# cbalint13/opencv-dlco

Measured on AMD Instinct MI355X. Metric: pj-learn patch-pairs/sec, higher is better.
Workload: dtype f32; 1 GPU; pj-learn configs[1] Liberty-shaped, rank ~64: 500000 pair-rows x PR-dim 8192, batch 200+200 per GPU (global 200+200), mu=0.0025 gamma=0.5, fp32, rank 48 after 3893 steps; device= (gfx950:sramecc+:xnack-), burn_in_steps=300

## Files before the change

### include/dlco.h

```cpp
#ifndef DLCO_H
#define DLCO_H

#include <stddef.h>
#include <stdint.h>

#ifdef __cplusplus
extern "C" {
#endif

#define DLCO_OK            0
#define DLCO_ERR_INVALID  -2
#define DLCO_ERR_HIP      -3
#define DLCO_ERR_NODEVICE -4
#define DLCO_ERR_NOCONV   -5
#define DLCO_ERR_COMM     -6

typedef struct dlco_ctx dlco_ctx;

typedef struct dlco_cfg {
    int32_t  F;
    int32_t  N;
    int32_t  B;
    float    mu;
    float    gamma;
    uint64_t seed;
    int32_t  device;
    int32_t  rank;
    int32_t  world;
    float    eig_tol;
    int32_t  eig_guard;
    int32_t  eig_max_iter;
    int32_t  shard;
    int32_t  strict_conv;
    int32_t  grad_bf16;
    int32_t  reserved[5];
} dlco_cfg;

void dlco_cfg_default(dlco_cfg *cfg);

const char *dlco_version(void);
const char *dlco_last_error(const dlco_ctx *ctx);

int dlco_ctx_create(dlco_ctx **out, const dlco_cfg *cfg);
void dlco_ctx_destroy(dlco_ctx *ctx);
int dlco_device_name(const dlco_ctx *ctx, char *buf, size_t cap, int *cc_major, int *cc_minor);

int dlco_set_data(dlco_ctx *ctx, const float *dists_host, const uint8_t *labels_host);
int dlco_set_data_device(dlco_ctx *ctx, const float *dists_dev, const uint8_t *labels_host);
int dlco_device_width(const dlco_ctx *ctx);
int dlco_set_data_shared(dlco_ctx *ctx, dlco_ctx *src);
int dlco_set_pairs(dlco_ctx *ctx, const float *desc_host, int32_t P, const int32_t *pairs_host);
int dlco_set_pairs_device(dlco_ctx *ctx, const float *desc_dev, int32_t P, const int32_t *pairs_host);
int dlco_synth_data(dlco_ctx *ctx, const float *U_host, int32_t k, uint64_t seed,
                    float sigma_pos, float sigma_neg, float noise, float scale_jitter);
int dlco_get_rows(dlco_ctx *ctx, int32_t row0, int32_t n, float *out_host);

int dlco_get_index(const dlco_ctx *ctx, int32_t *pos, int32_t *n_pos, int32_t *n_pos_trn,
                   int32_t *neg, int32_t *n_neg, int32_t *n_neg_trn);

int dlco_step(dlco_ctx *ctx);
int dlco_steps(dlco_ctx *ctx, int32_t n);

int dlco_step_begin(dlco_ctx *ctx);
int dlco_step_grad(dlco_ctx *ctx);
int dlco_step_finish(dlco_ctx *ctx);

#define DLCO_BUF_DIST   1
#define DLCO_BUF_GRAD   2
#define DLCO_BUF_DFAVG  3
#define DLCO_BUF_W      4
#define DLCO_BUF_GATHER 5
#define DLCO_BUF_DATA   6
int dlco_dev_buffer(dlco_ctx *ctx, int32_t which, void **dev_ptr, size_t *bytes);
int dlco_bind_buffer(dlco_ctx *ctx, int32_t which, void *dev_ptr, size_t bytes);

typedef int (*dlco_allgather_fn)(void *user, int32_t which, size_t bytes_per_rank);
int dlco_set_allgather(dlco_ctx *ctx, dlco_allgather_fn fn, void *user);
int dlco_comm_unique_id(void *out_id, size_t cap, const char *rccl_path);
int dlco_comm_init(dlco_ctx *ctx, const void *id, size_t id_bytes, const char *rccl_path);
int dlco_comm_init_host(dlco_ctx *ctx, const char *shm_name);
int dlco_comm_destroy(dlco_ctx *ctx);
int dlco_stream(dlco_ctx *ctx, void **stream);
int dlco_sync(dlco_ctx *ctx);

int dlco_get_batch(const dlco_ctx *ctx, int32_t *pos_rows, int32_t *neg_rows,
                   float *pos_dist, float *neg_dist, int32_t *rho, int32_t *kappa);

int dlco_get_t(const dlco_ctx *ctx, uint32_t *t);
int dlco_get_W(dlco_ctx *ctx, float *W_host , int32_t *r);
int dlco_get_A(dlco_ctx *ctx, float *A_host );
int dlco_get_dfavg(dlco_ctx *ctx, float *dfavg_host );
int dlco_set_state(dlco_ctx *ctx, uint32_t t, const float *dfavg_host, const float *W_host, int32_t r);

int dlco_validate(dlco_ctx *ctx, float *loss_val, float *regul, int32_t *rank);

int dlco_stats(dlco_ctx *ctx, const float *W_host, int32_t r, int32_t *dim, float *fpr95, double *auc);

int dlco_project_sqdist(dlco_ctx *ctx, const int32_t *row_ids_host, int32_t n,
                        const float *W_host, int32_t r, float *out_host);
int dlco_viol_counts(dlco_ctx *ctx, const float *pd_host, const float *nd_host, int32_t B,
                     int32_t *rho_host, int32_t *kappa_host);
int dlco_grad_rda(dlco_ctx *ctx, const int32_t *pos_rows_host, const int32_t *neg_rows_host,
                  const int32_t *rho_host, const int32_t *kappa_host, int32_t B,
                  float alpha, float beta, const float *dfavg_in_host, float *dfavg_out_host);
int dlco_psd_project(dlco_ctx *ctx, const float *dfavg_host, uint32_t t,
                     float *W_host, int32_t *r, float *A_host );
int dlco_sym_product(dlco_ctx *ctx, const float *X_host, int32_t rows, const float *G_host, int32_t mode,
                     float *out_host);
int dlco_hinge_sum(dlco_ctx *ctx, const float *pos_host, int32_t n_pos,
                   const float *neg_host, int32_t n_neg, double *out);
int dlco_roc_stats(dlco_ctx *ctx, const float *dist_host, const uint8_t *labels_host, int32_t n,
                   float *fpr95, double *auc);

typedef struct dlco_log_entry {
    uint32_t t;
    int32_t  is_best;
    int32_t  saved;
    float    loss_val, regul, obj, obj_best;
    int32_t  rank, rank_best;
    int32_t  dim;
    double   auc, auc_best;
    float    fpr95, fpr95_best;
    double   vtime;
    int32_t  nonconv;
    int32_t  reserved;
} dlco_log_entry;
int dlco_log_step(dlco_ctx *ctx, dlco_log_entry *out);
int dlco_get_saved(dlco_ctx *ctx, float *W_host, int32_t *r, float *A_host);

int dlco_profile_enable(dlco_ctx *ctx, int32_t on);
int dlco_profile_read(dlco_ctx *ctx, const char *kernel, int64_t *launches, double *total_ms);
int dlco_counters(const dlco_ctx *ctx, int64_t out[8]);
int dlco_eig_stats(const dlco_ctx *ctx, int64_t *iters, int64_t *product_rows, int64_t *jacobi_sweeps,
                   int32_t *block_rows);

typedef struct dlco_pr_ctx dlco_pr_ctx;
const char *dlco_pr_last_error(const dlco_pr_ctx *ctx);
int dlco_pr_create(dlco_pr_ctx **out, int32_t F, int32_t N, float mu, float gamma, uint64_t seed, int32_t device);
void dlco_pr_destroy(dlco_pr_ctx *ctx);
int dlco_pr_device_name(const dlco_pr_ctx *ctx, char *buf, size_t cap, int *cc_major, int *cc_minor);
int dlco_pr_set_data(dlco_pr_ctx *ctx, const float *dists_host, const uint8_t *labels_host);
int dlco_pr_get_index(const dlco_pr_ctx *ctx, int32_t *n_pos, int32_t *n_pos_trn, int32_t *n_neg, int32_t *n_neg_trn);
int dlco_pr_steps(dlco_pr_ctx *ctx, uint32_t n);
int dlco_pr_get_state(dlco_pr_ctx *ctx, uint32_t *t, float *w_host , float *dfavg_host );
int dlco_pr_set_state(dlco_pr_ctx *ctx, uint32_t t, const float *w_host, const float *dfavg_host);
int dlco_pr_validate(dlco_pr_ctx *ctx, float *loss_val, float *regul, int32_t *nnz);
int dlco_pr_stats(dlco_pr_ctx *ctx, const float *w_host, const float *prparams_host, int32_t pr_rows, int32_t pr_cols,
                  int32_t nchannels, int32_t max_dim, int32_t *nPR, int32_t *dim, int32_t *nzdim, float *fpr95, double *auc);

typedef struct dlco_pr_grid dlco_pr_grid;
int  dlco_pr_grid_create(dlco_pr_grid **out, dlco_pr_ctx *src, int32_t G, const float *mu, const float *gamma, uint64_t seed);
void dlco_pr_grid_destroy(dlco_pr_grid *grid);
const char *dlco_pr_grid_last_error(const dlco_pr_grid *grid);
int  dlco_pr_grid_steps(dlco_pr_grid *grid, uint32_t n);
int  dlco_pr_grid_get_state(dlco_pr_grid *grid, uint32_t *t, float *w_host , float *dfavg_host );
int  dlco_pr_grid_validate(dlco_pr_grid *grid, float *loss_val, float *regul, int32_t *nnz);
int  dlco_pr_grid_stats(dlco_pr_grid *grid, const int32_t *configs, int32_t n, const float *w_host, const float *prparams_host,
                        int32_t pr_rows, int32_t pr_cols, int32_t nchannels, int32_t max_dim,
                        int32_t *nPR, int32_t *dim, int32_t *nzdim, float *fpr95, double *auc);
int  dlco_pr_grid_set_group(dlco_pr_grid *grid, int32_t per_group);
int32_t dlco_pr_grid_group(const dlco_pr_grid *grid);

typedef struct dlco_desc_ctx dlco_desc_ctx;

int  dlco_desc_create(dlco_desc_ctx **out, float init_sigma, int32_t n_angle_bins, int32_t norm, int32_t device);
void dlco_desc_destroy(dlco_desc_ctx *ctx);
const char *dlco_desc_last_error(const dlco_desc_ctx *ctx);
int  dlco_desc_select_filters(const float *pr_filters, int32_t rows, int32_t cols, const float *w, int32_t wcols,
                              float *out, int32_t *nsel_out);
int  dlco_desc_set_filters(dlco_desc_ctx *ctx, const float *filters_host, int32_t nsel);
int32_t dlco_desc_size(const dlco_desc_ctx *ctx);
int  dlco_desc_transform(dlco_desc_ctx *ctx, const uint8_t *patch_host, float *patch_trans_host);
int  dlco_desc_compute(dlco_desc_ctx *ctx, const uint8_t *patches_host, int64_t n, float *desc_host);
int  dlco_desc_compute_device(dlco_desc_ctx *ctx, const uint8_t *patches_host, int64_t n, float *desc_dev, int64_t ld);
int  dlco_desc_pair_dists(dlco_desc_ctx *ctx, const uint8_t *patches_host, int64_t n_patches, const int32_t *pairs_host,
                          int64_t n_pairs, float *dist_host, uint8_t *label_host);
int  dlco_desc_full_dists(dlco_desc_ctx *ctx, const uint8_t *patches_host, int64_t n_patches, const int32_t *pairs_host,
                          int64_t n_pairs, float *dist_host, uint8_t *label_host);
typedef int (*dlco_desc_sink_fn)(void *user, int64_t row0, int64_t rows, const float *dist, const uint8_t *label);
int  dlco_desc_pair_dists_stream(dlco_desc_ctx *ctx, const uint8_t *patches_host, int64_t n_patches, const int32_t *pairs_host,
                                 int64_t n_pairs, int64_t chunk_rows, dlco_desc_sink_fn sink, void *user);
int  dlco_desc_full_dists_stream(dlco_desc_ctx *ctx, const uint8_t *patches_host, int64_t n_patches, const int32_t *pairs_host,
                                 int64_t n_pairs, int64_t chunk_rows, dlco_desc_sink_fn sink, void *user);
int  dlco_desc_set_projection(dlco_desc_ctx *ctx, const float *W_host, int32_t r, int32_t F);
int32_t dlco_desc_projected_size(const dlco_desc_ctx *ctx);
int  dlco_desc_describe(dlco_desc_ctx *ctx, const uint8_t *patches_host, int64_t n, float *out_host);
int  dlco_desc_describe_device(dlco_desc_ctx *ctx, const uint8_t *patches_host, int64_t n, float *out_dev, int64_t ld);
int  dlco_desc_pair_sqdists(dlco_desc_ctx *ctx, const uint8_t *patches_host, int64_t n_patches, const int32_t *pairs_host,
                            int64_t n_pairs, float *dist_host, uint8_t *label_host);
int  dlco_desc_pair_stats(dlco_desc_ctx *ctx, const uint8_t *patches_host, int64_t n_patches, const int32_t *pairs_host,
                          int64_t n_pairs, int32_t *dim, float *fpr95, double *auc);
int dlco_desc_match(dlco_desc_ctx *ctx, const float *query_host, int64_t nq, const float *train_host, int64_t nt,
                    int32_t r, int32_t *idx_host, float *sqdist_host);
int dlco_desc_match_device(dlco_desc_ctx *ctx, const float *query_dev, int64_t ldq, int64_t nq,
                           const float *train_dev, int64_t ldt, int64_t nt, int32_t r,
                           int32_t *idx_dev, float *sqdist_dev);
int dlco_desc_cross_sqdists(dlco_desc_ctx *ctx, const float *query_host, int64_t nq, const float *train_host, int64_t nt,
                            int32_t r, float *out_host);
double dlco_desc_last_kernel_ms(const dlco_desc_ctx *ctx);

#ifdef __cplusplus
}
#endif
#endif
```

### opencv-dlco_amd/__init__.py

```python
import ctypes as C
import os
import subprocess

import numpy as np

_HERE = os.path.dirname(os.path.abspath(__file__))
LIB_PATH = os.path.join(_HERE, "libdlco.so")
HEADER_PATH = os.path.join(os.path.dirname(_HERE), "include", "dlco.h")

OK, ERR_INVALID, ERR_HIP, ERR_NODEVICE, ERR_NOCONV, ERR_COMM = 0, -2, -3, -4, -5, -6
BUF_DIST, BUF_GRAD, BUF_DFAVG, BUF_W, BUF_GATHER, BUF_DATA = 1, 2, 3, 4, 5, 6
ALLGATHER_FN = C.CFUNCTYPE(C.c_int, C.c_void_p, C.c_int32, C.c_size_t)


class DlcoError(RuntimeError):
    def __init__(self, code, msg):
        super().__init__("libdlco error %d: %s" % (code, msg))
        self.code = code


class Cfg(C.Structure):
    _fields_ = [
        ("F", C.c_int32), ("N", C.c_int32), ("B", C.c_int32),
        ("mu", C.c_float), ("gamma", C.c_float),
        ("seed", C.c_uint64),
        ("device", C.c_int32), ("rank", C.c_int32), ("world", C.c_int32),
        ("eig_tol", C.c_float), ("eig_guard", C.c_int32), ("eig_max_iter", C.c_int32),
        ("shard", C.c_int32), ("strict_conv", C.c_int32), ("grad_bf16", C.c_int32),
        ("reserved", C.c_int32 * 5),
    ]


class LogEntry(C.Structure):
    _fields_ = [
        ("t", C.c_uint32), ("is_best", C.c_int32), ("saved", C.c_int32),
        ("loss_val", C.c_float), ("regul", C.c_float), ("obj", C.c_float), ("obj_best", C.c_float),
        ("rank", C.c_int32), ("rank_best", C.c_int32), ("dim", C.c_int32),
        ("auc", C.c_double), ("auc_best", C.c_double),
        ("fpr95", C.c_float), ("fpr95_best", C.c_float),
        ("vtime", C.c_double),
        ("nonconv", C.c_int32), ("reserved", C.c_int32),
    ]


def build(verbose=False):
    cmd = ["make", "-C", os.path.join(_HERE, "csrc"), "-j8"]
    if not verbose:
        cmd.insert(1, "-s")
    subprocess.check_call(cmd)


_lib = None
f32p, i32p, u8p = C.POINTER(C.c_float), C.POINTER(C.c_int32), C.POINTER(C.c_uint8)


def load():
    global _lib
    if _lib is not None:
        return _lib
    if not os.path.exists(LIB_PATH):
        raise DlcoError(ERR_NODEVICE, "%s is missing: run __graft_entry__.build() (no CPU fallback exists)" % LIB_PATH)
    L = C.CDLL(LIB_PATH)
    vp = C.c_void_p
    L.dlco_version.restype = C.c_char_p
    L.dlco_last_error.restype = C.c_char_p
    L.dlco_last_error.argtypes = [vp]
    L.dlco_cfg_default.argtypes = [C.POINTER(Cfg)]
    L.dlco_cfg_default.restype = None
    L.dlco_ctx_create.argtypes = [C.POINTER(vp), C.POINTER(Cfg)]
    L.dlco_ctx_destroy.argtypes = [vp]
    L.dlco_ctx_destroy.restype = None
    L.dlco_device_name.argtypes = [vp, C.c_char_p, C.c_size_t, C.POINTER(C.c_int), C.POINTER(C.c_int)]
    L.dlco_set_data.argtypes = [vp, f32p, u8p]
    L.dlco_set_data_device.argtypes = [vp, vp, u8p]
    L.dlco_set_data_shared.argtypes = [vp, vp]
    L.dlco_device_width.argtypes = [vp]
    L.dlco_set_pairs.argtypes = [vp, f32p, C.c_int32, i32p]
    L.dlco_synth_data.argtypes = [vp, f32p, C.c_int32, C.c_uint64, C.c_float, C.c_float, C.c_float, C.c_float]
    L.dlco_get_rows.argtypes = [vp, C.c_int32, C.c_int32, f32p]
    L.dlco_get_index.argtypes = [vp, i32p, i32p, i32p, i32p, i32p, i32p]
    for name in ("dlco_step", "dlco_step_begin", "dlco_step_grad", "dlco_step_finish", "dlco_sync"):
        getattr(L, name).argtypes = [vp]
    L.dlco_steps.argtypes = [vp, C.c_int32]
    L.dlco_dev_buffer.argtypes = [vp, C.c_int32, C.POINTER(vp), C.POINTER(C.c_size_t)]
    L.dlco_bind_buffer.argtypes = [vp, C.c_int32, vp, C.c_size_t]
    L.dlco_stream.argtypes = [vp, C.POINTER(vp)]
    L.dlco_set_allgather.argtypes = [vp, ALLGATHER_FN, vp]
    L.dlco_comm_unique_id.argtypes = [vp, C.c_size_t, C.c_char_p]
    L.dlco_comm_init.argtypes = [vp, vp, C.c_size_t, C.c_char_p]
    L.dlco_comm_destroy.argtypes = [vp]
    L.dlco_get_batch.argtypes = [vp, i32p, i32p, f32p, f32p, i32p, i32p]
    L.dlco_get_t.argtypes = [vp, C.POINTER(C.c_uint32)]
    L.dlco_get_W.argtypes = [vp, f32p, i32p]
    L.dlco_get_A.argtypes = [vp, f32p]
    L.dlco_get_dfavg.argtypes = [vp, f32p]
    L.dlco_set_state.argtypes = [vp, C.c_uint32, f32p, f32p, C.c_int32]
    L.dlco_validate.argtypes = [vp, f32p, f32p, i32p]
    L.dlco_stats.argtypes = [vp, f32p, C.c_int32, i32p, f32p, C.POINTER(C.c_double)]
    L.dlco_project_sqdist.argtypes = [vp, i32p, C.c_int32, f32p, C.c_int32, f32p]
    L.dlco_viol_counts.argtypes = [vp, f32p, f32p, C.c_int32, i32p, i32p]
    L.dlco_grad_rda.argtypes = [vp, i32p, i32p, i32p, i32p, C.c_int32, C.c_float, C.c_float, f32p, f32p]
    L.dlco_psd_project.argtypes = [vp, f32p, C.c_uint32, f32p, i32p, f32p]
    L.dlco_hinge_sum.argtypes = [vp, f32p, C.c_int32, f32p, C.c_int32, C.POINTER(C.c_double)]
    L.dlco_sym_product.argtypes = [vp, f32p, C.c_int32, f32p, C.c_int32, f32p]
    L.dlco_roc_stats.argtypes = [vp, f32p, u8p, C.c_int32, f32p, C.POINTER(C.c_double)]
    L.dlco_log_step.argtypes = [vp, C.POINTER(LogEntry)]
    L.dlco_get_saved.argtypes = [vp, f32p, i32p, f32p]
    L.dlco_profile_enable.argtypes = [vp, C.c_int32]
    L.dlco_profile_read.argtypes = [vp, C.c_char_p, C.POINTER(C.c_int64), C.POINTER(C.c_double)]
    L.dlco_eig_stats.argtypes = [vp, C.POINTER(C.c_int64), C.POINTER(C.c_int64), C.POINTER(C.c_int64), i32p]
    L.dlco_counters.argtypes = [vp, C.POINTER(C.c_int64)]
    i64 = C.c_int64
    L.dlco_set_pairs_device.argtypes = [vp, vp, C.c_int32, i32p]
    L.dlco_desc_last_error.restype = C.c_char_p
    L.dlco_desc_last_error.argtypes = [vp]
    L.dlco_desc_create.argtypes = [C.POINTER(vp), C.c_float, C.c_int32, C.c_int32, C.c_int32]
    L.dlco_desc_destroy.argtypes = [vp]
    L.dlco_desc_destroy.restype = None
    L.dlco_desc_select_filters.argtypes = [f32p, C.c_int32, C.c_int32, f32p, C.c_int32, f32p, C.POINTER(C.c_int32)]
    L.dlco_desc_set_filters.argtypes = [vp, f32p, C.c_int32]
    L.dlco_desc_size.argtypes = [vp]
    L.dlco_desc_size.restype = C.c_int32
    L.dlco_desc_transform.argtypes = [vp, u8p, f32p]
    L.dlco_desc_compute.argtypes = [vp, u8p, i64, f32p]
    L.dlco_desc_compute_device.argtypes = [vp, u8p, i64, vp, i64]
    L.dlco_desc_pair_dists.argtypes = [vp, u8p, i64, i32p, i64, f32p, u8p]
    L.dlco_desc_full_dists.argtypes = [vp, u8p, i64, i32p, i64, f32p, u8p]
    L.dlco_desc_set_projection.argtypes = [vp, f32p, C.c_int32, C.c_int32]
    L.dlco_desc_projected_size.argtypes = [vp]
    L.dlco_desc_projected_size.restype = C.c_int32
    L.dlco_desc_describe.argtypes = [vp, u8p, i64, f32p]
    L.dlco_desc_describe_device.argtypes = [vp, u8p, i64, vp, i64]
    L.dlco_desc_pair_sqdists.argtypes = [vp, u8p, i64, i32p, i64, f32p, u8p]
    L.dlco_desc_pair_stats.argtypes = [vp, u8p, i64, i32p, i64, C.POINTER(C.c_int32), C.POINTER(C.c_float), C.POINTER(C.c_double)]
    L.dlco_desc_match.argtypes = [vp, f32p, i64, f32p, i64, C.c_int32, i32p, f32p]
    L.dlco_desc_match_device.argtypes = [vp, vp, i64, i64, vp, i64, i64, C.c_int32, vp, vp]
    L.dlco_desc_cross_sqdists.argtypes = [vp, f32p, i64, f32p, i64, C.c_int32, f32p]
    L.dlco_desc_last_kernel_ms.argtypes = [vp]
    L.dlco_desc_last_kernel_ms.restype = C.c_double
    L.dlco_pr_last_error.restype = C.c_char_p
    L.dlco_pr_last_error.argtypes = [vp]
    L.dlco_pr_create.argtypes = [C.POINTER(vp), C.c_int32, C.c_int32, C.c_float, C.c_float, C.c_uint64, C.c_int32]
    L.dlco_pr_destroy.argtypes = [vp]
    L.dlco_pr_destroy.restype = None
    L.dlco_pr_device_name.argtypes = [vp, C.c_char_p, C.c_size_t, C.POINTER(C.c_int), C.POINTER(C.c_int)]
    L.dlco_pr_set_data.argtypes = [vp, f32p, u8p]
    L.dlco_pr_get_index.argtypes = [vp, i32p, i32p, i32p, i32p]
    L.dlco_pr_steps.argtypes = [vp, C.c_uint32]
    L.dlco_pr_get_state.argtypes = [vp, C.POINTER(C.c_uint32), f32p, f32p]
    L.dlco_pr_set_state.argtypes = [vp, C.c_uint32, f32p, f32p]
    L.dlco_pr_validate.argtypes = [vp, f32p, f32p, i32p]
    L.dlco_pr_stats.argtypes = [vp, f32p, f32p, C.c_int32, C.c_int32, C.c_int32, C.c_int32, i32p, i32p, i32p, f32p, C.POINTER(C.c_double)]
    L.dlco_pr_grid_last_error.restype = C.c_char_p
    L.dlco_pr_grid_last_error.argtypes = [vp]
    L.dlco_pr_grid_create.argtypes = [C.POINTER(vp), vp, C.c_int32, f32p, f32p, C.c_uint64]
    L.dlco_pr_grid_destroy.argtypes = [vp]
    L.dlco_pr_grid_destroy.restype = None
    L.dlco_pr_grid_steps.argtypes = [vp, C.c_uint32]
    L.dlco_pr_grid_get_state.argtypes = [vp, C.POINTER(C.c_uint32), f32p, f32p]
    L.dlco_pr_grid_validate.argtypes = [vp, f32p, f32p, i32p]
    L.dlco_pr_grid_stats.argtypes = [vp, i32p, C.c_int32, f32p, f32p, C.c_int32, C.c_int32, C.c_int32, C.c_int32, i32p, i32p, i32p, f32p,
                                     C.POINTER(C.c_double)]
    L.dlco_pr_grid_set_group.argtypes = [vp, C.c_int32]
    L.dlco_pr_grid_group.argtypes = [vp]
    L.dlco_pr_grid_group.restype = C.c_int32
    _lib = L
    return L


def comm_unique_id(rccl_path=None):
    L = load()
    buf = C.create_string_buffer(128)
    rc = L.dlco_comm_unique_id(buf, 128, rccl_path.encode() if rccl_path else None)
    if rc != OK:
        raise DlcoError(rc, L.dlco_last_error(None).decode())
    return buf.raw


def exported_symbols():
    import re
    text = open(HEADER_PATH).read()
    return sorted(set(re.findall(r"\b(dlco_[a-z0-9_]+)\s*\(", text)))


def _p(a, t):
    return None if a is None else a.ctypes.data_as(t)


def _f32(a):
    return np.ascontiguousarray(a, dtype=np.float32)


def _i32(a):
    return np.ascontiguousarray(a, dtype=np.int32)


class Context:

    def __init__(self, F, N, B=200, mu=0.001, gamma=0.5, seed=2215, device=0, rank=0, world=1,
                 eig_tol=None, eig_guard=None, eig_max_iter=None, shard=0, strict_conv=0, grad_bf16=0):
        self.L = load()
        cfg = Cfg()
        self.L.dlco_cfg_default(C.byref(cfg))
        cfg.F, cfg.N, cfg.B, cfg.mu, cfg.gamma, cfg.seed = F, N, B, mu, gamma, seed
        cfg.device, cfg.rank, cfg.world, cfg.shard = device, rank, world, shard
        cfg.strict_conv = strict_conv
        cfg.grad_bf16 = grad_bf16
        if eig_tol is not None:
            cfg.eig_tol = eig_tol
        if eig_guard is not None:
            cfg.eig_guard = eig_guard
        if eig_max_iter is not None:
            cfg.eig_max_iter = eig_max_iter
        self.F, self.N, self.B, self.world, self.rank = F, N, B, world, rank
        h = C.c_void_p()
        rc = self.L.dlco_ctx_create(C.byref(h), C.byref(cfg))
        if rc != OK:
            raise DlcoError(rc, self.L.dlco_last_error(None).decode())
        self.h = h

    def close(self):
        if getattr(self, "h", None):
            self.L.dlco_ctx_destroy(self.h)
            self.h = None

    def __del__(self):
        try:
            self.close()
        except Exception:
            pass

    def _ck(self, rc):
        if rc != OK:
            raise DlcoError(rc, self.L.dlco_last_error(self.h).decode())

    def device_name(self):
        buf = C.create_string_buffer(256)
        a, b = C.c_int(), C.c_int()
        self._ck(self.L.dlco_device_name(self.h, buf, 256, C.byref(a), C.byref(b)))
        return buf.value.decode(), a.value, b.value

    def set_data(self, dists, labels):
        d, l = _f32(dists), np.ascontiguousarray(labels, np.uint8).ravel()
        assert d.shape == (self.N, self.F) and l.size == self.N
        self._ck(self.L.dlco_set_data(self.h, _p(d, f32p), _p(l, u8p)))

    def set_data_device(self, dev_ptr, labels):
        l = np.ascontiguousarray(labels, np.uint8).ravel()
        self._ck(self.L.dlco_set_data_device(self.h, C.c_void_p(dev_ptr), _p(l, u8p)))

    def set_data_shared(self, other):
        self._ck(self.L.dlco_set_data_shared(self.h, other.h))

    def device_width(self):
        return int(self.L.dlco_device_width(self.h))

    def set_pairs(self, desc, pairs):
# ... 14 lines not shown
    def get_rows(self, row0, n):
        out = np.empty((n, self.F), np.float32)
        self._ck(self.L.dlco_get_rows(self.h, row0, n, _p(out, f32p)))
        return out

    def index(self):
        a, b, c_, d = C.c_int32(), C.c_int32(), C.c_int32(), C.c_int32()
        self._ck(self.L.dlco_get_index(self.h, None, C.byref(a), C.byref(b), None, C.byref(c_), C.byref(d)))
        pos, neg = np.empty(max(a.value, 1), np.int32), np.empty(max(c_.value, 1), np.int32)
        self._ck(self.L.dlco_get_index(self.h, _p(pos, i32p), None, None, _p(neg, i32p), None, None))
        return dict(pos=pos[:a.value], n_pos_trn=b.value, neg=neg[:c_.value], n_neg_trn=d.value)

    def step(self):
        self._ck(self.L.dlco_step(self.h))

    def steps(self, n):
        self._ck(self.L.dlco_steps(self.h, n))

    def step_begin(self):
        self._ck(self.L.dlco_step_begin(self.h))

    def step_grad(self):
        self._ck(self.L.dlco_step_grad(self.h))

    def step_finish(self):
        self._ck(self.L.dlco_step_finish(self.h))

    def sync(self):
        self._ck(self.L.dlco_sync(self.h))

    def dev_buffer(self, which):
        p, n = C.c_void_p(), C.c_size_t()
        self._ck(self.L.dlco_dev_buffer(self.h, which, C.byref(p), C.byref(n)))
        return p.value, n.value

    def bind_buffer(self, which, dev_ptr, nbytes):
        self._ck(self.L.dlco_bind_buffer(self.h, which, C.c_void_p(dev_ptr), nbytes))

    def stream(self):
        p = C.c_void_p()
        self._ck(self.L.dlco_stream(self.h, C.byref(p)))
        return p.value

    def comm_init(self, id_bytes, rccl_path=None):
        buf = C.create_string_buffer(bytes(id_bytes), 128)
        self._ck(self.L.dlco_comm_init(self.h, buf, 128, rccl_path.encode() if rccl_path else None))

    def comm_destroy(self):
        self._ck(self.L.dlco_comm_destroy(self.h))

    def set_allgather(self, fn):
        def tramp(_user, which, nbytes):
            try:
                return int(fn(int(which), int(nbytes)) or 0)
            except Exception:
                import traceback
                traceback.print_exc()
                return -1
        self._ag = ALLGATHER_FN(tramp)
        self._ck(self.L.dlco_set_allgather(self.h, self._ag, None))

    def batch(self):
        B = self.B
        pr, nr = np.empty(B, np.int32), np.empty(B, np.int32)
        pd, nd = np.empty(B, np.float32), np.empty(B, np.float32)
        rho, kap = np.empty(B, np.int32), np.empty(B, np.int32)
        self._ck(self.L.dlco_get_batch(self.h, _p(pr, i32p), _p(nr, i32p), _p(pd, f32p), _p(nd, f32p), _p(rho, i32p), _p(kap, i32p)))
        return dict(pos_rows=pr, neg_rows=nr, pd=pd, nd=nd, rho=rho, kappa=kap)

    def t(self):
        v = C.c_uint32()
        self._ck(self.L.dlco_get_t(self.h, C.byref(v)))
        return v.value

    def W(self):
        W = np.empty((self.F, self.F), np.float32)
        r = C.c_int32()
        self._ck(self.L.dlco_get_W(self.h, _p(W, f32p), C.byref(r)))
        return W[:r.value].copy()

    def A(self):
        A = np.empty((self.F, self.F), np.float32)
        self._ck(self.L.dlco_get_A(self.h, _p(A, f32p)))
        return A

    def dfavg(self):
        A = np.empty((self.F, self.F), np.float32)
        self._ck(self.L.dlco_get_dfavg(self.h, _p(A, f32p)))
        return A

    def set_state(self, t, dfavg=None, W=None):
        d = None if dfavg is None else _f32(dfavg)
        w = None if W is None or len(W) == 0 else _f32(W)
        self._ck(self.L.dlco_set_state(self.h, t, _p(d, f32p), _p(w, f32p), 0 if w is None else w.shape[0]))

    def validate(self):
        lo, rg, rk = C.c_float(), C.c_float(), C.c_int32()
        self._ck(self.L.dlco_validate(self.h, C.byref(lo), C.byref(rg), C.byref(rk)))
        return lo.value, rg.value, rk.value

    def stats(self, W=None):
        dim, f, a = C.c_int32(), C.c_float(), C.c_double()
        w = None if W is None else _f32(W)
        self._ck(self.L.dlco_stats(self.h, _p(w, f32p), 0 if w is None else w.shape[0], C.byref(dim), C.byref(f), C.byref(a)))
        return dim.value, f.value, a.value

    def log_step(self):
        e = LogEntry()
        self._ck(self.L.dlco_log_step(self.h, C.byref(e)))
        return e

    def saved(self):
        r = C.c_int32()
        self._ck(self.L.dlco_get_saved(self.h, None, C.byref(r), None))
        if r.value == 0:
            return None, None
        W, A = np.empty((r.value, self.F), np.float32), np.empty((self.F, self.F), np.float32)
        self._ck(self.L.dlco_get_saved(self.h, _p(W, f32p), C.byref(r), _p(A, f32p)))
        return W, A

    def project_sqdist(self, row_ids, W):
        ids, w = _i32(row_ids), _f32(W)
        out = np.empty(ids.size, np.float32)
        self._ck(self.L.dlco_project_sqdist(self.h, _p(ids, i32p), ids.size, _p(w, f32p), w.shape[0] if w.size else 0, _p(out, f32p)))
        return out

    def viol_counts(self, pd, nd):
        pd, nd = _f32(pd), _f32(nd)
        rho, kap = np.empty(pd.size, np.int32), np.empty(pd.size, np.int32)
        self._ck(self.L.dlco_viol_counts(self.h, _p(pd, f32p), _p(nd, f32p), pd.size, _p(rho, i32p), _p(kap, i32p)))
        return rho, kap

    def grad_rda(self, pos_rows, neg_rows, rho, kappa, alpha, beta, dfavg_in=None):
        pr, nr, rho, kap = _i32(pos_rows), _i32(neg_rows), _i32(rho), _i32(kappa)
        d = None if dfavg_in is None else _f32(dfavg_in)
        out = np.empty((self.F, self.F), np.float32)
        self._ck(self.L.dlco_grad_rda(self.h, _p(pr, i32p), _p(nr, i32p), _p(rho, i32p), _p(kap, i32p), pr.size, alpha, beta, _p(d, f32p), _p(out, f32p)))
        return out

    def psd_project(self, dfavg, t, want_A=True):
        d = _f32(dfavg)
        W = np.empty((self.F, self.F), np.float32)
        A = np.empty((self.F, self.F), np.float32) if want_A else None
        r = C.c_int32()
        self._ck(self.L.dlco_psd_project(self.h, _p(d, f32p), t, _p(W, f32p), C.byref(r), _p(A, f32p)))
        return W[:r.value].copy(), A

    def sym_product(self, X, G, mode=0):
        x, g = _f32(X), _f32(G)
        out = np.empty_like(x)
        self._ck(self.L.dlco_sym_product(self.h, _p(x, f32p), x.shape[0], _p(g, f32p), mode, _p(out, f32p)))
        return out

    def hinge_sum(self, pos, neg):
        p, n = _f32(pos), _f32(neg)
        out = C.c_double()
        self._ck(self.L.dlco_hinge_sum(self.h, _p(p, f32p), p.size, _p(n, f32p), n.size, C.byref(out)))
        return out.value

    def roc_stats(self, dist, labels):
        d, l = _f32(dist), np.ascontiguousarray(labels, np.uint8).ravel()
        f, a = C.c_float(), C.c_double()
        self._ck(self.L.dlco_roc_stats(self.h, _p(d, f32p), _p(l, u8p), d.size, C.byref(f), C.byref(a)))
        return f.value, a.value

    def profile_enable(self, on=True):
        self._ck(self.L.dlco_profile_enable(self.h, int(on)))

    def profile_read(self, kernel="grad_syrk"):
        n, ms = C.c_int64(), C.c_double()
        self._ck(self.L.dlco_profile_read(self.h, kernel.encode(), C.byref(n), C.byref(ms)))
        return n.value, ms.value

    def counters(self):
        out = (C.c_int64 * 8)()
        self._ck(self.L.dlco_counters(self.h, out))
        return dict(steps=out[0], active_rows=out[1], nonconverged=out[2], jacobi_barrier_timeouts=out[3],
                    rank_update_passes=out[4], rank_update_check=out[5] * 1e-9, locked_passes=out[6], locked_rows=out[7])

    def eig_stats(self):
        a, b, c_, d = C.c_int64(), C.c_int64(), C.c_int64(), C.c_int32()
        self._ck(self.L.dlco_eig_stats(self.h, C.byref(a), C.byref(b), C.byref(c_), C.byref(d)))
        return dict(iters=a.value, product_rows=b.value, jacobi_sweeps=c_.value, block_rows=d.value)


class PrContext:

    def __init__(self, F, N, mu=0.025, gamma=0.10, seed=2215, device=0):
        self.L = load()
        self.F, self.N = F, N
        h = C.c_void_p()
        rc = self.L.dlco_pr_create(C.byref(h), F, N, mu, gamma, seed, device)
        if rc != OK:
            raise DlcoError(rc, self.L.dlco_pr_last_error(None).decode())
        self.h = h

    def close(self):
        if getattr(self, "h", None):
            self.L.dlco_pr_destroy(self.h)
            self.h = None

    def __del__(self):
        try:
            self.close()
        except Exception:
            pass

    def _ck(self, rc):
        if rc != OK:
            raise DlcoError(rc, self.L.dlco_pr_last_error(self.h).decode())

    def set_data(self, dists, labels):
        d, l = _f32(dists), np.ascontiguousarray(labels, np.uint8).ravel()
        assert d.shape == (self.N, self.F) and l.size == self.N
        self._ck(self.L.dlco_pr_set_data(self.h, _p(d, f32p), _p(l, u8p)))

    def index(self):
        a, b, c_, d = C.c_int32(), C.c_int32(), C.c_int32(), C.c_int32()
        self._ck(self.L.dlco_pr_get_index(self.h, C.byref(a), C.byref(b), C.byref(c_), C.byref(d)))
        return dict(n_pos=a.value, n_pos_trn=b.value, n_neg=c_.value, n_neg_trn=d.value)

    def steps(self, n):
        self._ck(self.L.dlco_pr_steps(self.h, n))

    def state(self):
        t = C.c_uint32()
        w, df = np.empty(self.F, np.float32), np.empty(self.F, np.float32)
        self._ck(self.L.dlco_pr_get_state(self.h, C.byref(t), _p(w, f32p), _p(df, f32p)))
        return dict(t=t.value, w=w, dfavg=df)

    def set_state(self, t, w=None, dfavg=None):
        w = None if w is None else _f32(w)
        d = None if dfavg is None else _f32(dfavg)
        self._ck(self.L.dlco_pr_set_state(self.h, t, _p(w, f32p), _p(d, f32p)))

    def validate(self):
        lo, rg, nz = C.c_float(), C.c_float(), C.c_int32()
        self._ck(self.L.dlco_pr_validate(self.h, C.byref(lo), C.byref(rg), C.byref(nz)))
        return lo.value, rg.value, nz.value

    def stats(self, prparams, w=None, nchannels=8, max_dim=-1):
        p = _f32(prparams)
        wv = None if w is None else _f32(w)
        npr, dim, nz, f, a = C.c_int32(), C.c_int32(), C.c_int32(), C.c_float(-1.0), C.c_double(0.0)
        self._ck(self.L.dlco_pr_stats(self.h, _p(wv, f32p), _p(p, f32p), p.shape[0], p.shape[1], nchannels, max_dim,
                                      C.byref(npr), C.byref(dim), C.byref(nz), C.byref(f), C.byref(a)))
        return dict(nPR=npr.value, dim=dim.value, nzdim=nz.value, fpr95=f.value, auc=a.value)


class PrGrid:

    def __init__(self, src, mus, gammas, seed=2215):
        self.L = load()
        mu, ga = _f32(mus).ravel(), _f32(gammas).ravel()
        assert mu.size == ga.size
        self.src, self.F, self.N, self.G = src, src.F, src.N, int(mu.size)
        self.mus, self.gammas = mu.copy(), ga.copy()
        h = C.c_void_p()
        rc = self.L.dlco_pr_grid_create(C.byref(h), src.h, self.G, _p(mu, f32p), _p(ga, f32p), seed)
        if rc != OK:
            raise DlcoError(rc, self.L.dlco_pr_grid_last_error(None).decode())
        self.h = h

    def close(self):
        if getattr(self, "h", None):
            self.L.dlco_pr_grid_destroy(self.h)
            self.h = None

    def __del__(self):
        try:
            self.close()
        except Exception:
            pass

    def _ck(self, rc):
        if rc != OK:
            raise DlcoError(rc, self.L.dlco_pr_grid_last_error(self.h).decode())

    def set_group(self, per_group):
        self._ck(self.L.dlco_pr_grid_set_group(self.h, per_group))

    def group(self):
        return int(self.L.dlco_pr_grid_group(self.h))

    def steps(self, n):
        self._ck(self.L.dlco_pr_grid_steps(self.h, n))

    def state(self):
        t = C.c_uint32()
        w, df = np.empty((self.G, self.F), np.float32), np.empty((self.G, self.F), np.float32)
        self._ck(self.L.dlco_pr_grid_get_state(self.h, C.byref(t), _p(w, f32p), _p(df, f32p)))
        return dict(t=t.value, w=w, dfavg=df)

    def validate(self):
        lo, rg, nz = np.empty(self.G, np.float32), np.empty(self.G, np.float32), np.empty(self.G, np.int32)
        self._ck(self.L.dlco_pr_grid_validate(self.h, _p(lo, f32p), _p(rg, f32p), _p(nz, i32p)))
        return dict(loss=lo, regul=rg, nnz=nz)

    def stats(self, prparams, configs=None, w=None, nchannels=8, max_dim=-1):
        p = _f32(prparams)
        cf = _i32(np.arange(self.G) if configs is None else configs).ravel()
        n = cf.size
        wv = None if w is None else _f32(w).reshape(n, self.F)
        npr, dim, nz = np.zeros(n, np.int32), np.zeros(n, np.int32), np.zeros(n, np.int32)
        f, a = np.full(n, -1.0, np.float32), np.zeros(n, np.float64)
        self._ck(self.L.dlco_pr_grid_stats(self.h, _p(cf, i32p), n, _p(wv, f32p), _p(p, f32p), p.shape[0], p.shape[1], nchannels, max_dim,
# ... 146 lines not shown
```

### opencv-dlco_amd/csrc/dlco_api.cpp

```cpp
#include "../../include/dlco.h"

#include "dlco_internal.hpp"
#include "eig_tracker.hpp"
#include "pair_index.hpp"
#include "rccl_comm.hpp"
#include "host_comm.hpp"

#include <algorithm>
#include <cfloat>
#include <chrono>
#include <cmath>
#include <cstring>

using namespace dlco;

static thread_local std::string g_last_error;

namespace {
struct EnvSwitch { const char *name, *purpose; };
const EnvSwitch kEnvSwitches[] = {
    {"DLCO_SYRK_FP32", "gradient SYRK as the k-ordered fp32 MFMA chain (syrk_rda_kernel8) instead of split-bf16 planes"},
    {"DLCO_NO_PACKED", "full F x F dual average where the packed upper-tile form would apply"},
    {"DLCO_FORCE_SHARD", "column-sharded layout (cfg.shard) on a single rank: the multi-GPU path on one GPU"},
    {"DLCO_NO_RANK_UPDATE", "first filter term from a product with the dual average, not from the step's rank update"},
// ... 989 lines not shown
        if (r) h2d_rows(c, Wd.p, W_host, (size_t)r, true);
        if (n <= 4096) project_few(c, ids.p, n, Wd.p, r, out.p);
        else project_many(c, ids.p, 0, n, Wd.p, r, out.p);
        d2h(c, out_host, out.p, (size_t)n * sizeof(float));
    });
}

int dlco_viol_counts(dlco_ctx *c, const float *pd_host, const float *nd_host, int32_t B, int32_t *rho_host,
                     int32_t *kappa_host)
{
    if (!c || !pd_host || !nd_host || !rho_host || !kappa_host || B < 0) return DLCO_ERR_INVALID;
    return guarded(c, [&] {
        DLCO_HIP(hipSetDevice(c->cfg.device));
        if (B == 0) return;
        DevBuf<float> pd, nd; DevBuf<int32_t> rho, kap;
        pd.alloc(B); nd.alloc(B); rho.alloc(B); kap.alloc(B);
        h2d(c, pd.p, pd_host, (size_t)B * sizeof(float));
        h2d(c, nd.p, nd_host, (size_t)B * sizeof(float));
        viol_counts(pd.p, nd.p, B, rho.p, kap.p, c->stream);
        d2h(c, rho_host, rho.p, (size_t)B * sizeof(int32_t));
        d2h(c, kappa_host, kap.p, (size_t)B * sizeof(int32_t));
    });
}

int dlco_grad_rda(dlco_ctx *c, const int32_t *pos_rows_host, const int32_t *neg_rows_host, const int32_t *rho_host,
                  const int32_t *kappa_host, int32_t B, float alpha, float beta, const float *dfavg_in_host,
                  float *dfavg_out_host)
{
    if (!c || !pos_rows_host || !neg_rows_host || !rho_host || !kappa_host || !dfavg_out_host || B < 1) return DLCO_ERR_INVALID;
    return guarded(c, [&] {
        DLCO_HIP(hipSetDevice(c->cfg.device));
        DLCO_CHECK(c->have_data && c->phase == 0, DLCO_ERR_INVALID, "dlco_grad_rda: no data / step in flight");
        for (int i = 0; i < B; i++)
            DLCO_CHECK(pos_rows_host[i] >= 0 && pos_rows_host[i] < c->N && neg_rows_host[i] >= 0 && neg_rows_host[i] < c->N,
                       DLCO_ERR_INVALID, "dlco_grad_rda: row id out of range");
        DevBuf<int32_t> pr, nr, rho, kap, ids; DevBuf<float> w; DevBuf<int> k;
        pr.alloc(B); nr.alloc(B); rho.alloc(B); kap.alloc(B); ids.alloc((2 * B + 31) & ~31); w.alloc((2 * B + 31) & ~31); k.alloc(1);
        h2d(c, pr.p, pos_rows_host, (size_t)B * sizeof(int32_t));
        h2d(c, nr.p, neg_rows_host, (size_t)B * sizeof(int32_t));
        h2d(c, rho.p, rho_host, (size_t)B * sizeof(int32_t));
        h2d(c, kap.p, kappa_host, (size_t)B * sizeof(int32_t));
        const size_t FF = (size_t)c->F * c->F;
        if (dfavg_in_host) {
            h2d_square(c, c->grad.p, dfavg_in_host);
            if (!c->shard) syrk_mirror_upper(c->grad.p, c->F, c->F, c->stream);
        } else fill_f32(c->grad.p, 0.f, FF, c->stream);
        build_active_rows(pr.p, nr.p, rho.p, kap.p, B, 0, B, ids.p, w.p, k.p, c->stream);
        if (c->packed) {
            DevBuf<float> pk;
            pk.alloc(syrk_packed_floats(c->F));
            syrk_pack_upper(c->grad.p, c->F, c->F, pk.p, c->stream);
            grad_syrk(c, ids.p, w.p, k.p, 2 * B, alpha, beta, pk.p, true);
            syrk_unpack_upper(pk.p, c->F, c->grad.p, c->F, c->stream);
            d2h_square(c, dfavg_out_host, c->grad.p);
            return;
        }
        grad_syrk(c, ids.p, w.p, k.p, 2 * B, alpha, beta, c->grad.p);
        d2h_square(c, dfavg_out_host, c->grad.p);
    });
}

int dlco_psd_project(dlco_ctx *c, const float *dfavg_host, uint32_t t, float *W_host, int32_t *r, float *A_host)
{
    if (!c || !dfavg_host || !r) return DLCO_ERR_INVALID;
    return guarded(c, [&] {
        DLCO_HIP(hipSetDevice(c->cfg.device));
        DLCO_CHECK(c->phase == 0, DLCO_ERR_INVALID, "dlco_psd_project: step in flight");
        const size_t FF = (size_t)c->F * c->F;
        DevBuf<float> G, Gp;
        G.alloc(FF);
        h2d_square(c, G.p, dfavg_host);
        if (c->packed) {
            Gp.alloc(syrk_packed_floats(c->F));
            syrk_mirror_upper(G.p, c->F, c->F, c->stream);
            syrk_pack_upper(G.p, c->F, c->F, Gp.p, c->stream);
        }
        c->eig->reset();
        const float cscale = (float)(std::sqrt((double)t + 1.0) / (double)c->cfg.gamma);
        double tr = 0.0;
        bool conv = true;
        DevBuf<float> Wd;
        Wd.alloc((size_t)c->w_cap * c->F);
        const int rr = c->eig->update(c->packed ? Gp.p : G.p, c->cfg.mu, cscale, Wd.p, &tr, &conv);
        c->eig->reset();
        if (rr > 0) {
            if (W_host) d2h_rows(c, W_host, Wd.p, (size_t)rr);
            *r = rr;
        } else {
            if (W_host) std::memset(W_host, 0, (size_t)c->Fu * c->Fu * sizeof(float));
            *r = c->Fu;
        }
        if (A_host) {
            build_A(c, Wd.p, rr);
            d2h_square(c, A_host, c->grad.p);
        }
        if (!conv) throw Error(DLCO_ERR_NOCONV, "dlco_psd_project: tracker did not reach its tolerance");
    });
}

int dlco_sym_product(dlco_ctx *c, const float *X_host, int32_t rows, const float *G_host, int32_t mode, float *out_host)
{
    if (!c || !X_host || !G_host || !out_host || rows < 1 || rows > ((mode == 1 || mode == 3) ? 160 : 128)) return DLCO_ERR_INVALID;
    return guarded(c, [&] {
        DLCO_HIP(hipSetDevice(c->cfg.device));
        const int F = c->F, pad = ((rows + 31) / 32) * 32;
        DevBuf<float> X, G, out;
        X.alloc((size_t)pad * F); G.alloc((size_t)F * F); out.alloc((size_t)pad * F);
        X.zero(c->stream);
        h2d_rows(c, X.p, X_host, (size_t)rows);
        h2d_square(c, G.p, G_host);
        bool ok;
        if (mode == 3 || mode == 4) {
            DevBuf<char> hi, lo, lo2;
            hi.alloc(bf16x2_plane_bytes(rows, F)); lo.alloc(bf16x2_plane_bytes(rows, F));
            if (mode == 4) lo2.alloc(bf16x2_plane_bytes(rows, F));
            DevBuf<float> slab, Gp;
            slab.alloc((size_t)4 * pad * F);
            Gp.alloc(syrk_packed_floats(F));
            syrk_mirror_upper(G.p, F, F, c->stream);
            syrk_pack_upper(G.p, F, F, Gp.p, c->stream);
            ok = skinny_product_sym(X.p, F, rows, Gp.p, F, 1.0f, out.p, F, nullptr, 0.f, nullptr, 0.f, hi.p, lo.p, slab.p, c->stream,
                                    mode == 4 ? lo2.p : nullptr);
            sync(c);
        } else if (mode == 1 || mode == 2) {
            DevBuf<char> hi, lo, lo2;
            hi.alloc(bf16x2_plane_bytes(rows, F)); lo.alloc(bf16x2_plane_bytes(rows, F));
            if (mode == 2) lo2.alloc(bf16x2_plane_bytes(rows, F));
            DevBuf<float> slab;
            slab.alloc(bf16x2_slab_floats(rows, F));
            ok = skinny_product_bf16x2(X.p, F, rows, G.p, F, F, F, 1.0f, out.p, F, nullptr, 0.f, nullptr, 0.f, hi.p, lo.p, slab.p,
                                       c->stream, 0, mode == 2 ? lo2.p : nullptr);
            sync(c);
        } else {
            GemmArgs g;
            g.M = rows; g.N = F; g.K = F;
            g.A.p = X.p; g.A.ld = F; g.A.kmajor = false;
            g.B.p = G.p; g.B.ld = F; g.B.kmajor = true;
            g.C = out.p; g.ldc = F;
            const int bm = rows <= 64 ? 64 : 128;
            const long tiles = (long)((rows + bm - 1) / bm) * ((F + 127) / 128);
            g.split_k = split_k_slices(tiles, 1024, F, 256);
            DevBuf<float> slab;
            slab.alloc(gemm_slab_floats(rows, F, g.split_k));
            g.slab = slab.p;
            gemm_f32(g, c->stream);
            sync(c);
            ok = true;
        }
        DLCO_CHECK(ok, DLCO_ERR_INVALID, "dlco_sym_product: shape not supported by this mode");
        d2h_rows(c, out_host, out.p, (size_t)rows);
    });
}

int dlco_hinge_sum(dlco_ctx *c, const float *pos_host, int32_t n_pos, const float *neg_host, int32_t n_neg, double *out)
{
    if (!c || !out || n_pos < 0 || n_neg < 0) return DLCO_ERR_INVALID;
    return guarded(c, [&] {
        DLCO_HIP(hipSetDevice(c->cfg.device));
        *out = 0.0;
        if (n_pos == 0) return;
        DevBuf<float> p, n, rows;
        p.alloc(n_pos); n.alloc(std::max(n_neg, 1)); rows.alloc(n_pos);
        h2d(c, p.p, pos_host, (size_t)n_pos * sizeof(float));
        if (n_neg) h2d(c, n.p, neg_host, (size_t)n_neg * sizeof(float));
        hinge_rows(p.p, n_pos, n.p, n_neg, rows.p, c->stream);
        sum_f32_to_f64(rows.p, n_pos, c->dscal.p, c->stream);
        d2h(c, out, c->dscal.p, sizeof(double));
    });
}

int dlco_roc_stats(dlco_ctx *c, const float *dist_host, const uint8_t *labels_host, int32_t n, float *fpr95, double *auc)
{
    if (!c || !dist_host || !labels_host || !fpr95 || !auc || n < 1) return DLCO_ERR_INVALID;
    return guarded(c, [&] {
        DLCO_HIP(hipSetDevice(c->cfg.device));
        DevBuf<float> d; DevBuf<uint8_t> l;
        d.alloc(n); l.alloc(n);
        h2d(c, d.p, dist_host, (size_t)n * sizeof(float));
        h2d(c, l.p, labels_host, (size_t)n);
        RocWork *w = roc_work_create(n);
        try { roc_stats(w, d.p, l.p, n, fpr95, auc, c->stream); } catch (...) { roc_work_destroy(w); throw; }
        roc_work_destroy(w);
    });
}

int dlco_log_step(dlco_ctx *c, dlco_log_entry *out)
{
    if (!c || !out) return DLCO_ERR_INVALID;
    return guarded(c, [&] {
        DLCO_HIP(hipSetDevice(c->cfg.device));
        DLCO_CHECK(c->phase == 0, DLCO_ERR_INVALID, "dlco_log_step: step in flight");
        const auto t0 = std::chrono::steady_clock::now();
        std::memset(out, 0, sizeof(*out));
        out->t = c->t - 1;
        float loss = 0.f, regul = 0.f;
        int32_t rank = 0;
        validate(c, &loss, &regul, &rank);
        const auto t1 = std::chrono::steady_clock::now();
        out->loss_val = loss; out->regul = regul; out->obj = loss + regul; out->rank = rank;
        if ((loss + regul) < c->obj_best) {
            c->obj_best = loss + regul;
            c->r_best = rank;
            out->is_best = 1;
            int32_t dim = 0; float f95 = 0.f; double auc = 0.0;
            stats(c, c->W.p, c->r, &dim, &f95, &auc);
            out->dim = dim; out->auc = auc; out->fpr95 = f95;
            if (c->auc_best <= auc && c->fpr95_best >= f95) {
                c->auc_best = auc; c->fpr95_best = f95;
                c->r_save_dev = c->r;
                c->r_save = c->r > 0 ? c->r : c->Fu;
                if (c->r > 0) {
                    c->W_save_dev.alloc((size_t)c->w_cap * c->F);
                    DLCO_HIP(hipMemcpyAsync(c->W_save_dev.p, c->W.p, (size_t)c->r * c->F * sizeof(float), hipMemcpyDeviceToDevice, c->stream));
                }
                out->saved = 1;
            }
        }
        out->obj_best = c->obj_best; out->rank_best = c->r_best;
        out->auc_best = c->auc_best; out->fpr95_best = c->fpr95_best;
        out->vtime = std::chrono::duration<double>(t1 - t0).count();
        out->nonconv = c->nonconv_window;
        c->nonconv_window = 0;
    });
}

int dlco_get_saved(dlco_ctx *c, float *W_host, int32_t *r, float *A_host)
{
    if (!c || !r) return DLCO_ERR_INVALID;
    *r = c->r_save;
    if (c->r_save <= 0 || (!W_host && !A_host)) return DLCO_OK;
    return guarded(c, [&] {
        DLCO_HIP(hipSetDevice(c->cfg.device));
        DLCO_CHECK(c->phase == 0, DLCO_ERR_INVALID, "dlco_get_saved: step in flight");
        if (W_host) {
            if (c->r_save_dev > 0) d2h_rows(c, W_host, c->W_save_dev.p, (size_t)c->r_save_dev);
            else std::memset(W_host, 0, (size_t)c->Fu * c->Fu * sizeof(float));
        }
        if (A_host) {
            build_A(c, c->W_save_dev.p, c->r_save_dev);
            d2h_square(c, A_host, c->grad.p);
        }
    });
}

int dlco_profile_enable(dlco_ctx *c, int32_t on)
{
    if (!c) return DLCO_ERR_INVALID;
    return guarded(c, [&] {
        c->prof.reset();
        c->prof.on = on != 0;
        c->prof.mask = on == 2 ? (1u << PROF_GRAD_SYRK) : ~0u;
    });
}

int dlco_profile_read(dlco_ctx *c, const char *kernel, int64_t *launches, double *total_ms)
{
    if (!c || !launches || !total_ms) return DLCO_ERR_INVALID;
    return guarded(c, [&] {
        int slot = PROF_GRAD_SYRK;
        if (kernel && std::strcmp(kernel, "eig_product") == 0) slot = PROF_EIG_PRODUCT;
        else if (kernel && std::strcmp(kernel, "jacobi") == 0) slot = PROF_JACOBI;
        else if (kernel && std::strcmp(kernel, "project") == 0) slot = PROF_PROJECT;
        else if (kernel && std::strcmp(kernel, "rank_update") == 0) slot = PROF_RANK_UPDATE;
        else if (kernel && std::strcmp(kernel, "grad_syrk") != 0) throw Error(DLCO_ERR_INVALID, "dlco_profile_read: unknown kernel group");
        c->prof.drain(slot);
        *launches = c->prof.rec[slot].n;
        *total_ms = c->prof.rec[slot].ms;
    });
}

int dlco_counters(const dlco_ctx *c, int64_t out[8])
{
    if (!c || !out) return DLCO_ERR_INVALID;
    for (int i = 0; i < 8; i++) out[i] = 0;
    out[0] = c->steps_run; out[1] = c->active_rows_sum; out[2] = c->nonconv_steps;
    out[3] = c->eig->stats().jacobi_barrier_timeouts;
    out[4] = c->eig->stats().rank_update_passes;
    out[5] = (int64_t)(c->eig->stats().rank_update_check * 1e9);
    out[6] = c->eig->stats().locked_passes;
    out[7] = c->eig->stats().locked_rows;
    return DLCO_OK;
}

int dlco_eig_stats(const dlco_ctx *c, int64_t *iters, int64_t *product_rows, int64_t *jacobi_sweeps, int32_t *block_rows)
{
    if (!c) return DLCO_ERR_INVALID;
    const EigStats &s = c->eig->stats();
    if (iters) *iters = s.iters;
    if (product_rows) *product_rows = s.product_rows;
    if (jacobi_sweeps) *jacobi_sweeps = s.jacobi_sweeps;
    if (block_rows) *block_rows = c->eig->block_rows();
    return DLCO_OK;
}

}
```

### opencv-dlco_amd/csrc/dlco_internal.hpp

```cpp
#pragma once

#include "../../include/dlco.h"

#include <hip/hip_runtime.h>

#include <algorithm>
#include <climits>
#include <cstdint>
#include <cstdio>
#include <cstdlib>
#include <cstring>
#include <functional>
#include <mutex>
#include <utility>
#include <stdexcept>
#include <string>
#include <type_traits>
#include <vector>

namespace dlco {

struct Error : std::runtime_error {
    int code;
    Error(int c, const std::string &m) : std::runtime_error(m), code(c) {}
};

#define DLCO_HIP(expr)                                                             \
    do {                                                                           \
        hipError_t e__ = (expr);                                                   \
        if (e__ != hipSuccess)                                                     \
            throw ::dlco::Error(-3, std::string(#expr) + ": " + hipGetErrorString(e__)); \
    } while (0)

#define DLCO_CHECK(cond, code, msg)                                                \
    do {                                                                           \
        if (!(cond)) throw ::dlco::Error((code), std::string(msg));                \
    } while (0)

template <typename Fn>
int guarded_call(std::string &thread_err, std::string *ctx_err, Fn &&fn)
{
    try {
        fn();
        return DLCO_OK;
    } catch (const Error &e) {
        thread_err = e.what();
        if (ctx_err) *ctx_err = e.what();
        return e.code;
    } catch (const std::exception &e) {
        thread_err = e.what();
        if (ctx_err) *ctx_err = e.what();
        return DLCO_ERR_INVALID;
    }
}

inline hipDeviceProp_t use_gfx950_device(int device)
{
    int ndev = 0;
    if (hipGetDeviceCount(&ndev) != hipSuccess || ndev <= 0 || device >= ndev)
        throw Error(DLCO_ERR_NODEVICE, "no usable HIP device (this library has no CPU fallback)");
    DLCO_HIP(hipSetDevice(device));
    hipDeviceProp_t prop;
    DLCO_HIP(hipGetDeviceProperties(&prop, device));
    if (std::strncmp(prop.gcnArchName, "gfx950", 6) != 0)
        throw Error(DLCO_ERR_NODEVICE, std::string("device is ") + prop.gcnArchName + ", this build targets gfx950 only");
    return prop;
}

template <int MAX, typename F>
void dispatch_mt(int mt, F &&f)
{
    if constexpr (MAX > 1) {
        if (mt < MAX) return dispatch_mt<MAX - 1>(mt, f);
    }
    f(std::integral_constant<int, MAX>{});
}

const char *env_switch(const char *name);

inline void ensure_dynamic_lds(const void *func, int bytes)
{
    static std::mutex mu;
    static std::vector<std::pair<const void *, int>> done;
    int dev = 0;
    DLCO_HIP(hipGetDevice(&dev));
    std::lock_guard<std::mutex> lock(mu);
    for (const auto &d : done)
        if (d.first == func && d.second == dev) return;
    DLCO_HIP(hipFuncSetAttribute(func, hipFuncAttributeMaxDynamicSharedMemorySize, bytes));
    done.emplace_back(func, dev);
}

template <typename T>
struct DevBuf {
    T *p = nullptr;
    size_t n = 0;
    DevBuf() = default;
    DevBuf(const DevBuf &) = delete;
    DevBuf &operator=(const DevBuf &) = delete;
    ~DevBuf() { release(); }
    void release() {
        if (p) (void)hipFree(p);
        p = nullptr;
        n = 0;
    }
    void alloc(size_t count) {
        if (count <= n && p) return;
        release();
        if (count == 0) count = 1;
        DLCO_HIP(hipMalloc((void **)&p, count * sizeof(T)));
        n = count;
    }
    void zero(hipStream_t s) { if (p) DLCO_HIP(hipMemsetAsync(p, 0, n * sizeof(T), s)); }
};

enum ProfSlot { PROF_GRAD_SYRK = 0, PROF_EIG_PRODUCT = 1, PROF_JACOBI = 2, PROF_PROJECT = 3, PROF_RANK_UPDATE = 4, PROF_SLOTS = 5 };

struct Profiler {
    bool on = false;
    unsigned mask = ~0u;
    hipStream_t s = nullptr;
    struct Rec { std::vector<hipEvent_t> ev; size_t used = 0; double ms = 0.0; int64_t n = 0; };
    Rec rec[PROF_SLOTS];
    ~Profiler() { for (auto &r : rec) for (hipEvent_t e : r.ev) (void)hipEventDestroy(e); }
    void mark(int slot) {
        if (!on || !((mask >> slot) & 1u)) return;
        Rec &r = rec[slot];
        if (r.used == r.ev.size()) { hipEvent_t e; DLCO_HIP(hipEventCreateWithFlags(&e, hipEventDisableSystemFence)); r.ev.push_back(e); }
        DLCO_HIP(hipEventRecord(r.ev[r.used++], s));
        if (r.used >= 8192 && (r.used % 2) == 0) drain(slot);
    }
    void begin(int slot) { mark(slot); }
    void end(int slot) { mark(slot); }
    void drain(int slot) {
        Rec &r = rec[slot];
        if (r.used == 0) return;
        DLCO_HIP(hipStreamSynchronize(s));
        for (size_t i = 0; i + 1 < r.used; i += 2) {
            float ms = 0.f;
            DLCO_HIP(hipEventElapsedTime(&ms, r.ev[i], r.ev[i + 1]));
            r.ms += ms; r.n++;
        }
        r.used = 0;
    }
    void drain_all() { for (int i = 0; i < PROF_SLOTS; i++) drain(i); }
    void reset() { drain_all(); for (auto &r : rec) { r.ms = 0.0; r.n = 0; } }
};

struct GemmOperand {
    const float *p = nullptr;
    long ld = 0;
    bool kmajor = false;
    const int32_t *row_ids = nullptr;
    const int32_t *row_ids2 = nullptr;
    const float *row_scale = nullptr;
};

struct GemmArgs {
    int M = 0, N = 0, K = 0;
    GemmOperand A, B;
    float *C = nullptr;
    long ldc = 0;
    float alpha = 1.0f, beta = 0.0f;
    const float *E1 = nullptr;
    float b1 = 0.0f;
    const float *E2 = nullptr;
    float b2 = 0.0f;
    const int *k_dev = nullptr;
    int split_k = 1;
    float *slab = nullptr;
    bool upper_only = false;
    const float *B2 = nullptr;
    float *C2 = nullptr;
    bool small_m_tiles = false;
    bool small_n_tiles = false;
};

void gemm_f32(const GemmArgs &a, hipStream_t s);
size_t bf16x2_plane_bytes(int M, int K);
size_t bf16x2_slab_floats(int M, int N, int ksplit = 0);
void split_planes_bf16(const float *X, long ldx, int M, int K, void *hi, void *lo, void *lo2, hipStream_t s);
bool skinny_product_bf16x2(const float *X, long ldx, int M, const float *G, long ldg, int N, int K, float alpha, float *C,
                           long ldc, const float *E1, float b1, const float *E2, float b2, void *plane_hi, void *plane_lo,
                           float *slab, hipStream_t s, int ksplit = 0, void *plane_lo2 = nullptr, bool g_tiled = false);
size_t project_rows_plane_bytes(int K);
bool project_rows_sqdist(const float *W, long ldw, int r, const float *D, long ldd, int F, const int32_t *ids, const int32_t *ids2,
                         long row0, int nrows, float *dist, void *plane_hi, void *plane_lo, void *plane_lo2, bool bf16, hipStream_t s);
bool project_rows_slab(const float *W, long ldw, int r, const float *D, long ldd, int F, const int32_t *ids, const int32_t *ids2,
                       int nrows, int ksplit, float *slab, long ldn, void *plane_hi, void *plane_lo, void *plane_lo2, bool bf16,
                       hipStream_t s);
struct RankCoeffJob {
    const float *proj = nullptr;
    long ldp = 0;
    int nw = 0, m = 0, MT = 0;
    const float *wscale = nullptr;
    const int32_t *slot = nullptr;
    void *frag = nullptr;
};
void syrk_mirror_upper(float *C, long ldc, int F, hipStream_t s);
size_t syrk_planes_bytes(int kmax, int F);
bool syrk_rda_f32(const float *D, long ldd, const int32_t *ids, const int32_t *ids2, const float *w, const int *k_dev,
                  int kmax, int F, float alpha, float beta, float *C, long ldc, hipStream_t s, int slab_col0 = 0,
                  int slab_cols = 0, bool bf16 = false, bool packed = false, void *planes_ws = nullptr,
                  const RankCoeffJob *coeff_job = nullptr);
int syrk_planes_mode(bool bf16);
size_t rank_coeff_bytes(int m, int kmax);
bool rank_first_term(const float *Y, const float *Q, long ld, int m, int F, float ay, float aq, float ac, float *out,
                     const float *proj, long ldp, int nw, const float *wscale, const int32_t *slot, const float *w,
                     const int *k_dev, int kmax, const void *planes, void *coeff_ws, void *plane_hi, void *plane_lo, hipStream_t s,
                     bool coeff_ready = false, int planes_mode = 3);
size_t syrk_packed_floats(int F);
void syrk_pack_upper(const float *C, long ldc, int F, float *packed, hipStream_t s);
void syrk_unpack_upper(const float *packed, int F, float *C, long ldc, hipStream_t s);
bool skinny_product_sym(const float *X, long ldx, int M, const float *Gpacked, int F, float alpha, float *C, long ldc,
                        const float *E1, float b1, const float *E2, float b2, void *plane_hi, void *plane_lo, float *slab,
                        hipStream_t s, void *plane_lo2 = nullptr, bool planes_ready = false, bool emit_planes = false);
size_t gemm_slab_floats(int M, int N, int split_k);
inline int split_k_slices(long tiles, long target, long K, long kmin, long slab_cap = LONG_MAX)
{
    const long split = std::min(std::min((target + tiles - 1) / tiles, K / kmin), slab_cap);
    return (int)std::max(1L, split);
}
void splitk_reduce_f32(const float *slab, int split, int M, int N, float *C, long ldc, float alpha, float beta,
                       const float *E1, float b1, const float *E2, float b2, hipStream_t s);

void sqdist_from_proj(const float *proj, int split, int r, int n, long ld, float *dist, hipStream_t s, int r_all = 0,
                      float *reduced = nullptr);
void viol_counts(const float *pd, const float *nd, int B, int32_t *rho, int32_t *kappa, hipStream_t s);
void viol_counts_active_rows(const float *pd, const float *nd, int B, int32_t *rho, int32_t *kappa, const int32_t *pos_rows,
                             const int32_t *neg_rows, int slot_lo, int slot_hi, int32_t *ids, float *w, int *k_active, hipStream_t s,
                             int32_t *slots = nullptr);
void build_active_rows(const int32_t *pos_rows, const int32_t *neg_rows, const int32_t *rho, const int32_t *kappa,
                       int B, int slot_lo, int slot_hi, int32_t *ids, float *w, int *k_active, hipStream_t s);
void hinge_rows(const float *pos, int n_pos, const float *neg, int n_neg, float *row_sums, hipStream_t s);
void sum_f32_to_f64(const float *x, int n, double *out, hipStream_t s);
void hinge_rows_batched(const float *pos, int n_pos, const float *neg, int n_neg, long ld_in, float *row_sums, long ld_out, int count,
                        hipStream_t s);
void sum_f32_to_f64_batched(const float *x, int n, long ldx, double *out, int count, hipStream_t s);
void axpby_inplace(float *y, const float *x, float a, float b, size_t n, hipStream_t s);
void scale_rows(float *dst, long ldd, const float *src, long lds, const float *scale, const int32_t *src_rows,
                int rows, int cols, hipStream_t s, const int32_t *src_rows2 = nullptr);
void emit_w_rows(float *W, long ldw, const float *Q, long ldq, const float *theta, int nw, float mu, float cscale, int F,
                 hipStream_t s, int m_ext = 0, float *wscale = nullptr);
void translate_ids(const int32_t *ids, int base, int n, const int32_t *pa, const int32_t *pb, int32_t *out_a, int32_t *out_b,
                   hipStream_t s);
void fill_f32(float *p, float v, size_t n, hipStream_t s);

struct ShardComm {
    int world = 1, rank = 0;
    int c0 = 0, cw = 0;
    float *gather = nullptr;
    size_t gather_floats = 0;
    std::function<void(size_t bytes_per_rank)> allgather;
};
void pack_cols(float *dst, const float *src, long ld, int c0, int cw, int rows, hipStream_t s);
void unpack_cols(float *dst, long ld, const float *src, int cw, int rows, int world, hipStream_t s);

void synth_rows(float *D, int N, int F, long ld, const float *U, int k, uint64_t seed, float sig_pos, float sig_neg,
                float noise, float jitter, hipStream_t s);

void jacobi_eigh(const float *T, long ldt, int n, float *evals, float *V, long ldv, float *work, int *sweeps_out,
                 hipStream_t s, float lam_cut = -3.0e38f, bool single_workgroup = false);
size_t jacobi_work_floats(int n);
constexpr int CHOL_INV_MAX_N = 160;
void chol_inverse128(const float *M, long ldm, int n, float rel_thresh, float *Linv, long ldl, int *dead, hipStream_t s);
struct ResidualEmit {
    float *W = nullptr;
    long ldw = 0;
    float mu = 0.f, cscale = 0.f;
    float *wscale = nullptr;
    bool guards = false;
};
void residual_norms_publish(const float *X, const float *Y, long ld, const float *theta, int m, int F, float *res, unsigned *ticket,
                            const float *src, float *dst_host, int n, unsigned *flag_host, unsigned seq, hipStream_t s,
                            const int *extra_dev = nullptr, int *extra_host = nullptr, const ResidualEmit *emit = nullptr,
                            bool *emitted = nullptr);
void residual_norms(const float *X, const float *Y, long ld, const float *theta, int m, int F, float *res,
                    hipStream_t s);
void row_normalize(float *X, long ld, int m, int F, hipStream_t s, float min_norm = 0.f);
void symv(const float *H, long ld, int F, const float *x, float *y, hipStream_t s);

struct RocWork;
RocWork *roc_work_create(int n_max);
void roc_work_destroy(RocWork *w);
void roc_stats(RocWork *w, const float *dist_dev, const uint8_t *labels_dev, int n, float *fpr95, double *auc,
               hipStream_t s);

bool pr_steps(const float *D, long ld, const int32_t *pos_rows, const int32_t *neg_rows, unsigned n, unsigned t0, float mu, float gamma,
              int F, float *w_io, float *df_io, float *last_f, hipStream_t s);
void pr_gemv(const float *D, long ld, const int32_t *ids, int n, const float *w, int F, float *out, bool in_double, hipStream_t s);
int pr_grid_group(int G, int F, int cus);
bool pr_grid_steps(const float *D, long ld, const int32_t *pos_rows, const int32_t *neg_rows, unsigned n, unsigned t0, const float *mu,
                   const float *gamma, int G, int group, int F, long ldw, float *w_io, float *df_io, hipStream_t s);
void pr_gemv_multi(const float *D, long ld, const int32_t *ids, int n, const float *W, long ldw, const int32_t *sel, int nsel, int F,
                   float *out, long ldo, bool in_double, hipStream_t s);

void desc_permute_filters(const float *src, int nsel, float *dst, hipStream_t s);
void desc_transform(const uint8_t *patches, int n_patches, const float *cf, int ks, float inv_step, bool norm, int qk, float qgamma,
                    float *PT, hipStream_t s);
void desc_pool(const float *PT, int n_patches, const float *Fl, int nsel, int nsel_pad, float *desc, long desc_ld, hipStream_t s);
void desc_pair_diff(const float *desc, long ld, int F, const int32_t *pairs, long n_pairs, float *dist, uint8_t *label, hipStream_t s);
void desc_full_dist(const float *desc, long ld, int n_groups, int n_pairs, float *dist, hipStream_t s);
void desc_project(const float *desc, long desc_ld, int n, const float *W, int r, int F, float *Y, long y_ld, hipStream_t s);
void desc_pair_sqdist(const float *Y, long ld, int r, const int32_t *pairs, long n_pairs, float *dist, uint8_t *label, hipStream_t s);
void match_norms(const float *x, long ld, long n, int r, double *norm, hipStream_t s);
int match_tiles_per_slice(long nq, long nt, int n_cu);
int match_slices(long nt, int tiles_per_slice);
void match_top2(const float *query, long ldq, int nq, const float *train, long ldt, int nt, int r, const double *qnorm, const double *tnorm,
                int tiles_per_slice, int32_t *idx, float *sqdist, void *part, float *out, hipStream_t s);

}
```

### opencv-dlco_amd/csrc/eig_tracker.cpp

```cpp
#include "eig_tracker.hpp"

#include <algorithm>
#include <chrono>
#include <cmath>
#include <cstring>
#include <initializer_list>

namespace dlco {

namespace {
inline int ceil_div(long a, long b) { return (int)((a + b - 1) / b); }
}

struct EigTracker::PlaneChain {
    const float *planes_of = nullptr;
    int rows = 0;
    bool next = false;
};

EigTracker::EigTracker(int F, int max_rows, int guard, float tol, int max_iter, hipStream_t stream, int live_cols)
    : F_(F), live_(live_cols > 0 ? std::min(live_cols, F) : F), guard_(guard), max_iter_(max_iter), tol_(tol), s_(stream)
{
    cap_ = std::min(live_, std::max(max_rows, 2 * guard + 32));
    if (guard_ > cap_ / 2) guard_ = std::max(1, cap_ / 2);
    for (int i = 0; i < 6; i++) { buf_[i].alloc((size_t)cap_ * F_); all_[i] = buf_[i].p; }
    Q_ = all_[0]; Y_ = all_[1];
    Tm_.alloc((size_t)cap_ * cap_);
    Vm_.alloc((size_t)cap_ * cap_);
    Cw_.alloc((size_t)cap_ * cap_);
    ritz_block_.alloc((size_t)2 * (cap_ + 8) + 8);
    evals_.p = ritz_block_.p;
    res_.p = ritz_block_.p + (cap_ + 8);
    sweeps_dev_ = reinterpret_cast<int *>(ritz_block_.p + 2 * (cap_ + 8));
    DLCO_HIP(hipMemsetAsync(sweeps_dev_, 0, 8 * sizeof(int), s_));
    scale_.alloc(cap_ + 8);
    wscale_.alloc(cap_ + 8);
    srcrow_.alloc(cap_ + 8);
    jwork_.alloc(jacobi_work_floats(cap_));
    dead_.alloc(CHOL_INV_MAX_N);
    {
        const int nt = F_ / 128;
        ks_ = 1;
        for (int d : {4, 2, 8, 7, 6, 5, 3})
            if (nt > 0 && nt % d == 0) { ks_ = d; break; }
    }
    plane_hi_.alloc(bf16x2_plane_bytes(std::min(cap_, 160), F_));
    plane_lo_.alloc(bf16x2_plane_bytes(std::min(cap_, 160), F_));
    plane_lo2_.alloc(bf16x2_plane_bytes(std::min(cap_, 128), F_));
    pv_.alloc(F_);
    pw_.alloc(F_);
    slab_floats_ = std::max((size_t)4 * cap_ * F_, (size_t)8 << 20);
    slab_floats_ = std::min(slab_floats_, (size_t)64 << 20);
    slab_floats_ = std::max(slab_floats_, (size_t)cap_ * F_);
    slab_.alloc(slab_floats_);
    pin_floats_ = (size_t)3 * cap_ + 64;
    DLCO_HIP(hipHostMalloc((void **)&pin_, pin_floats_ * sizeof(float), hipHostMallocCoherent));
    std::memset(pin_, 0, pin_floats_ * sizeof(float));
    h_theta_.assign(cap_, 0.f);
    h_res_.assign(cap_, 0.f);
}

EigTracker::~EigTracker()
{
    if (pin_) (void)hipHostFree(pin_);
}

float *EigTracker::pick(std::initializer_list<const float *> busy) const
{
    for (int i = 0; i < 6; i++) {
        bool used = false;
        for (const float *b : busy) used = used || (b == all_[i]);
        if (!used) return all_[i];
    }
    throw Error(-2, "eig tracker: no free work buffer");
}

void EigTracker::reset()
{
    m_ = 0;
    have_theta_ = false;
    have_lo_ = false;
    steps_since_lo_ = 0;
    cold_ = true;
    wext_rows_ = 0;
    ru_offered_ = false;
}

void EigTracker::seed_rows(const float *src, long ld, const int32_t *ids_dev, int n, const int32_t *ids2_dev)
{
    const int k = std::min(n, cap_);
    have_theta_ = false;
    wext_rows_ = 0;
    ru_offered_ = false;
    if (k <= 0) { m_ = 0; return; }
    scale_rows(Q_, F_, src, ld, nullptr, ids_dev, k, F_, s_, ids2_dev);
    m_ = k;
}

bool EigTracker::rank_coeff_job(RankCoeffJob *job, int kmax)
{
    if (wext_rows_ <= 0 || wext_rows_ != m_ || m_ > 160 || !packed_ || shard_ || kmax % 32 != 0) return false;
    coeff_.alloc(rank_coeff_bytes(cap_ < 160 ? cap_ : 160, kmax));
    job->nw = wext_nw_; job->m = m_; job->MT = (m_ + 31) / 32;
    job->wscale = wscale_.p; job->frag = coeff_.p;
    return true;
}

float EigTracker::next_uniform()
{
    rng_ ^= rng_ << 13; rng_ ^= rng_ >> 7; rng_ ^= rng_ << 17;
    return (float)((double)(rng_ >> 11) * (2.0 / 9007199254740992.0) - 1.0);
}

void EigTracker::append_random(float *Q, int have, int add)
{
    if (add <= 0) return;
    y_ok_ = false;
    h_tmp_.assign((size_t)add * F_, 0.f);
    for (int i = 0; i < add; i++)
        for (int j = 0; j < live_; j++) h_tmp_[(size_t)i * F_ + j] = next_uniform();
    DLCO_HIP(hipMemcpyAsync(Q + (size_t)have * F_, h_tmp_.data(), h_tmp_.size() * sizeof(float), hipMemcpyHostToDevice, s_));
    DLCO_HIP(hipStreamSynchronize(s_));
}

void EigTracker::product(const float *X, int rows, const float *G, float alpha, float *out, const float *E1, float b1,
                         const float *E2, float b2, bool approx, PlaneChain *chain)
{
    const int one_pass = (approx && !shard_) ? 160 : (packed_ ? 96 : 128);
    if (rows > one_pass && (packed_ || F_ >= 256)) {
        if (chain) chain->next = false;
        const int step = approx ? (rows <= 2 * one_pass ? (rows / 2 + 31) / 32 * 32 : one_pass) : 96;
        for (int r0 = 0; r0 < rows; r0 += step) {
            const int nr = std::min(step, rows - r0);
            const size_t o = (size_t)r0 * F_;
            product(X + o, nr, G, alpha, out + o, E1 ? E1 + o : nullptr, b1, E2 ? E2 + o : nullptr, b2, approx, chain);
        }
        return;
    }
    st_.product_rows += rows;
    if (packed_) {
        if (prof_) prof_->begin(PROF_EIG_PRODUCT);
        const bool ready = approx && chain && chain->planes_of == X && chain->rows == rows;
        const bool emit = approx && chain && chain->next;
        const bool ok = skinny_product_sym(X, F_, rows, G, F_, alpha, out, F_, E1, b1, E2, b2, plane_hi_.p, plane_lo_.p, slab_.p, s_,
                                           approx ? nullptr : plane_lo2_.p, ready, emit);
        if (chain) { chain->planes_of = emit ? out : nullptr; chain->rows = rows; }
        if (prof_) prof_->end(PROF_EIG_PRODUCT);
        DLCO_CHECK(ok, -2, "eig tracker: the symmetric product rejected a shape of the packed layout");
        return;
    }
    if (shard_) {
        const int c0 = shard_->c0, cw = shard_->cw, world = shard_->world;
        DLCO_CHECK((size_t)world * rows * cw <= shard_->gather_floats, -2, "eig tracker: exchange buffer too small");
        const float *E1s = E1 ? E1 + c0 : nullptr, *E2s = E2 ? E2 + c0 : nullptr;
        if (prof_) prof_->begin(PROF_EIG_PRODUCT);
        bool done = false;
        if (rows <= 128) {
            int ks = ks_;
            while (ks < 4 * world && F_ % (128 * ks * 2) == 0 && bf16x2_slab_floats(rows, cw, ks * 2) <= slab_floats_) ks *= 2;
            done = skinny_product_bf16x2(X, F_, rows, G + c0, F_, cw, F_, alpha, out + c0, F_, E1s, b1, E2s, b2, plane_hi_.p,
                                         plane_lo_.p, slab_.p, s_, ks, approx ? nullptr : plane_lo2_.p);
        }
        if (!done) {
            GemmArgs g;
            g.M = rows; g.N = cw; g.K = F_;
            g.A.p = X; g.A.ld = F_; g.A.kmajor = false;
            g.B.p = G + c0; g.B.ld = F_; g.B.kmajor = true;
            g.C = out + c0; g.ldc = F_;
            g.alpha = alpha; g.E1 = E1s; g.b1 = b1; g.E2 = E2s; g.b2 = b2;
            const long tiles = (long)ceil_div(rows, rows <= 64 ? 64 : 128) * ceil_div(cw, 128);
            g.split_k = split_k_slices(tiles, 512, F_, 256, (long)(slab_floats_ / ((size_t)rows * cw)));
            g.slab = slab_.p;
            gemm_f32(g, s_);
        }
        if (prof_) prof_->end(PROF_EIG_PRODUCT);
        pack_cols(shard_->gather + (size_t)shard_->rank * rows * cw, out, F_, c0, cw, rows, s_);
        shard_->allgather((size_t)rows * cw * sizeof(float));
        unpack_cols(out, F_, shard_->gather, cw, rows, world, s_);
        return;
    }
    if (rows <= one_pass && F_ >= 256) {
        if (prof_) prof_->begin(PROF_EIG_PRODUCT);
        const bool ok = skinny_product_bf16x2(X, F_, rows, G, F_, F_, F_, alpha, out, F_, E1, b1, E2, b2, plane_hi_.p,
                                              plane_lo_.p, slab_.p, s_, ks_, approx ? nullptr : plane_lo2_.p);
        if (prof_) prof_->end(PROF_EIG_PRODUCT);
        if (ok) return;
    }
    GemmArgs g;
    g.M = rows; g.N = F_; g.K = F_;
    g.A.p = X; g.A.ld = F_; g.A.kmajor = false;
    g.B.p = G; g.B.ld = F_; g.B.kmajor = true;
    g.C = out; g.ldc = F_;
    g.alpha = alpha; g.E1 = E1; g.b1 = b1; g.E2 = E2; g.b2 = b2;
    const int bm = rows <= 64 ? 64 : 128;
    const long tiles = (long)ceil_div(rows, bm) * ceil_div(F_, 128);
    g.split_k = split_k_slices(tiles, 1024, F_, 256, (long)(slab_floats_ / ((size_t)rows * F_)));
    g.slab = slab_.p;
    if (prof_) prof_->begin(PROF_EIG_PRODUCT);
    gemm_f32(g, s_);
    if (prof_) prof_->end(PROF_EIG_PRODUCT);
}

void EigTracker::rotate(const float *C, long ldc, int k_in, int k_out, const float *X, float *out, const float *X2, float *out2)
{
    GemmArgs g;
    g.M = k_out; g.N = F_; g.K = k_in;
    g.A.p = C; g.A.ld = ldc; g.A.kmajor = false;
    g.B.p = X; g.B.ld = F_; g.B.kmajor = true;
    g.C = out; g.ldc = F_;
    g.B2 = X2; g.C2 = out2;
    gemm_f32(g, s_);
}

void EigTracker::gram_rect(const float *X, int xrows, const float *Y, int yrows, float *T)
{
    GemmArgs g;
    g.M = xrows; g.N = yrows; g.K = F_;
    g.A.p = X; g.A.ld = F_; g.A.kmajor = false;
    g.B.p = Y; g.B.ld = F_; g.B.kmajor = false;
    g.C = T; g.ldc = cap_;
    const long tiles = (long)ceil_div(xrows, xrows <= 64 ? 64 : 128) * ceil_div(yrows, yrows <= 64 ? 64 : 128);
    const long kslice = std::max(64L, (long)F_ / 64 / 64 * 64);
    g.split_k = split_k_slices(tiles, 512, F_, kslice, (long)(slab_floats_ / ((size_t)xrows * yrows)));
    g.slab = slab_.p;
    gemm_f32(g, s_);
}

void EigTracker::project_out(float *Wp, int np, const float *Q, int kept)
{
    gram_rect(Wp, np, Q, kept, Cw_.p);
    GemmArgs g;
    g.M = np; g.N = F_; g.K = kept;
    g.A.p = Cw_.p; g.A.ld = cap_; g.A.kmajor = false;
    g.B.p = Q; g.B.ld = F_; g.B.kmajor = true;
    g.C = Wp; g.ldc = F_;
    g.alpha = -1.0f; g.beta = 1.0f;
    gemm_f32(g, s_);
}

int EigTracker::orthonormalize(float *Z, int rows, float *scratch, const std::vector<int> &panel_ends, int skip)
{
    const bool one_panel = skip == 0 && rows <= CHOL_INV_MAX_N && (panel_ends.empty() || panel_ends[0] >= rows);
    if (!one_panel) row_normalize(Z + (size_t)skip * F_, F_, rows - skip, F_, s_);
    size_t pi = 0;
    for (int p0 = skip; p0 < rows;) {
        while (pi < panel_ends.size() && panel_ends[pi] <= p0) pi++;
        int pend = pi < panel_ends.size() ? std::min(rows, panel_ends[pi]) : rows;
        if (pend - p0 > CHOL_INV_MAX_N) pend = p0 + CHOL_INV_MAX_N;
        const int np = pend - p0;
        float *Wp = Z + (size_t)p0 * F_, *Sp = scratch + (size_t)p0 * F_;
        if (p0 > 0) {
            for (int pass = 0; pass < 2; pass++) {
                project_out(Wp, np, Z, p0);
                row_normalize(Wp, F_, np, F_, s_, pass == 0 ? 2e-5f : 0.f);
            }
        }
        for (int pass = 0; pass < 2; pass++) {
            const float *src = pass == 0 ? Wp : Sp;
            float *dst = pass == 0 ? Sp : Wp;
            gram_rect(src, np, src, np, Tm_.p);
            chol_inverse128(Tm_.p, cap_, np, 1e-5f, Vm_.p, cap_, dead_.p, s_);
            GemmArgs g;
            g.M = np; g.N = F_; g.K = np;
            g.A.p = Vm_.p; g.A.ld = cap_; g.A.kmajor = false;
            g.B.p = src; g.B.ld = F_; g.B.kmajor = true;
            g.C = dst; g.ldc = F_;
            gemm_f32(g, s_);
        }
        p0 = pend;
    }
    return rows;
}

int EigTracker::drop_dead_rows()
{
    std::vector<int32_t> live;
    for (int i = 0; i < m_; i++)
        if (!(h_theta_[i] == 0.f && h_res_[i] == 0.f)) live.push_back(i);
    const int k = (int)live.size();
    if (k == m_ || k == 0) return m_;
    DLCO_HIP(hipMemcpyAsync(srcrow_.p, live.data(), (size_t)k * sizeof(int32_t), hipMemcpyHostToDevice, s_));
    DLCO_HIP(hipStreamSynchronize(s_));
    float *Qn = pick({Q_, Y_});
    scale_rows(Qn, F_, Q_, F_, nullptr, srcrow_.p, k, F_, s_);
    float *Yn = pick({Q_, Y_, Qn});
    scale_rows(Yn, F_, Y_, F_, nullptr, srcrow_.p, k, F_, s_);
    Q_ = Qn; Y_ = Yn;
    for (int j = 0; j < k; j++) { h_theta_[j] = h_theta_[live[j]]; h_res_[j] = h_res_[live[j]]; }
    m_ = k;
    return k;
}

void EigTracker::refresh_lower_bound(const float *G, int iters, float theta_top)
{
    static const float kZero = 0.f;
    const bool cold = !have_lo_;
    if (cold) {
        std::vector<float> v(F_, 0.f);
        for (int i = 0; i < live_; i++) v[i] = next_uniform();
        DLCO_HIP(hipMemcpyAsync(pv_.p, v.data(), F_ * sizeof(float), hipMemcpyHostToDevice, s_));
        DLCO_HIP(hipStreamSynchronize(s_));
        row_normalize(pv_.p, F_, 1, F_, s_);
    }
    DLCO_HIP(hipMemcpyAsync(scale_.p, &kZero, sizeof(float), hipMemcpyHostToDevice, s_));
    auto run = [&](float shift, int n) -> float {
        float *v = pv_.p, *w = pw_.p;
        for (int i = 0; i < n; i++) {
            if (shard_ || packed_) product(v, 1, G, 1.0f, w, nullptr, 0.f, nullptr, 0.f, false);
            else symv(G, F_, F_, v, w, s_);
            if (shift != 0.f) axpby_inplace(w, v, 1.0f, shift, F_, s_);
            if (i == n - 1) residual_norms(v, w, F_, scale_.p, 1, F_, res_.p, s_);
            row_normalize(w, F_, 1, F_, s_);
            std::swap(v, w);
        }
        if (v != pv_.p) DLCO_HIP(hipMemcpyAsync(pv_.p, v, F_ * sizeof(float), hipMemcpyDeviceToDevice, s_));
        DLCO_HIP(hipMemcpyAsync(pin_, res_.p, sizeof(float), hipMemcpyDeviceToHost, s_));
        DLCO_HIP(hipStreamSynchronize(s_));
        return pin_[0];
    };
    const float rho = run(0.f, cold ? 12 : 2);
    const float shift = std::max(cold ? 2.0f * rho : 1.05f * rho, 1.1f * std::max(theta_top, 0.f)) + 1e-30f;
    const float top = run(shift, iters) - shift;
    const float lam_max = std::max(top, 0.f);
    lo_bound_ = -(1.3f * lam_max + 0.05f * std::max(rho, theta_top)) - 1e-12f;
    have_lo_ = true;
    steps_since_lo_ = 0;
}

struct EigTracker::UpdateState {
    const float *G = nullptr;
    float mu = 0.f, cscale = 0.f;
    float *W = nullptr;
    float tol = 0.f;
    bool ru_ok = false;
    int ru_nw = 0;
    int it = 0;
    int nw = 0;
    int n_ritz = 0;
    float theta_top = 0.f, block_min = 0.f;
    bool conv = false, cheap_done = false;
    bool w_emitted = false;
    eig_rules::FilterPlan plan;
    std::vector<int> panel_ends;
};

eig_rules::Block EigTracker::block_of(const UpdateState &u) const
{
    eig_rules::Block b;
    b.theta = h_theta_.data(); b.res = h_res_.data();
    b.m = m_; b.live = live_; b.guard = guard_;
    b.mu = u.mu; b.cscale = u.cscale; b.tol = u.tol;
    return b;
}

int EigTracker::update(const float *G, float mu, float cscale, float *W, double *trace, bool *converged)
{
    st_.updates++;
    UpdateState u;
    u.G = G; u.mu = mu; u.cscale = cscale; u.W = W;
    open_update(u);
    for (; u.it < max_iter_; u.it++) {
        u.plan = eig_rules::plan_filter(block_of(u), u.n_ritz, u.nw, u.it, deg0_, lo_bound_, u.block_min, u.theta_top, lock_,
                                        !u.cheap_done && y_ok_, last_crit_);
        float *Z = Q_;
        if (u.plan.cheap) { u.cheap_done = true; Z = filter_cheap(u); }
        else if (u.plan.n_lock > 0) Z = filter_locked(u);
        else if (u.plan.filtered) Z = filter_plain(u);
        if (u.plan.filtered) last_deg_ = u.plan.d;
        eig_rules::cut_panels(block_of(u), u.n_ritz, u.plan, CHOL_INV_MAX_N, u.panel_ends);
        orthonormalize(Z, m_, pick({Z}), u.panel_ends, u.plan.n_lock);
        rayleigh_ritz(u, Z);
        judge(u);
        const bool crowded = m_ < live_ && eig_rules::reaches_guards(u.nw, m_, guard_);
        if (crowded) u.conv = false;
        if (crowded && m_ < cap_) { grow(u); continue; }
        if (crowded || u.conv) { u.it++; break; }
    }
    const double tr = trim_and_emit(u);
    if (converged) *converged = u.conv;
    if (trace) *trace = tr;
    return u.nw;
}

void EigTracker::open_update(UpdateState &u)
{
    u.ru_ok = ru_offered_ && y_ok_ && have_theta_ && packed_ && !shard_ && wext_rows_ == m_ &&
              ru_.rows == m_ && m_ >= 1 && m_ <= 160 && m_ < live_ && ru_.proj && ru_.planes;
    ru_offered_ = false;
    u.ru_nw = wext_nw_;
    wext_rows_ = 0;
    y_ok_ = false;
    if (m_ == 0) {
        m_ = std::min(cap_, 2 * guard_ + 32);
        append_random(Q_, 0, m_);
        have_theta_ = false;
    }
    u.theta_top = have_theta_ ? h_theta_[0] : 0.f;
    u.block_min = have_theta_ ? std::min(h_theta_[m_ - 1], u.mu) : u.mu;
    u.n_ritz = have_theta_ ? m_ : 0;
    steps_since_lo_++;
    if (!have_lo_) refresh_lower_bound(u.G, 30, u.theta_top);
    else if (steps_since_lo_ >= eig_rules::lower_bound_period(st_.updates)) refresh_lower_bound(u.G, 6, u.theta_top);

    u.tol = cold_ ? 0.25f * tol_ : tol_;
    cold_ = false;
}

float *EigTracker::filter_cheap(const UpdateState &u)
{
    const float c0 = u.plan.c0, e0 = u.plan.e0;
    axpby_inplace(Y_, Q_, 1.0f / e0, -c0 / e0, (size_t)m_ * F_, s_);
    y_ok_ = false;
    st_.cheap_passes++;
    return Y_;
}

float *EigTracker::filter_locked(const UpdateState &u)
{
    const float c0 = u.plan.c0, e0 = u.plan.e0;
    const int n_lock = u.plan.n_lock, na = m_ - n_lock;
    const size_t off = (size_t)n_lock * F_;
    y_ok_ = false;
    const float *prev = Q_;
    float *cur = pick({Q_, Y_});
    product(Q_ + off, na, u.G, -1.0f / e0, cur + off, Q_ + off, -c0 / e0, nullptr, 0.f, true);
    project_out(cur + off, na, Q_, n_lock);
    for (int k = 2; k <= u.plan.d; k++) {
        float *nxt = pick({Q_, prev, cur});
        product(cur + off, na, u.G, -2.0f / e0, nxt + off, cur + off, -2.0f * c0 / e0, prev + off, -1.0f, true);
        project_out(nxt + off, na, Q_, n_lock);
        prev = cur; cur = nxt;
    }
    DLCO_HIP(hipMemcpyAsync(cur, Q_, off * sizeof(float), hipMemcpyDeviceToDevice, s_));
    st_.locked_passes++;
    st_.locked_rows += n_lock;
    return cur;
}

float *EigTracker::filter_plain(const UpdateState &u)
{
    const float c0 = u.plan.c0, e0 = u.plan.e0;
    const int d = u.plan.d;
    const float *prev = Q_;
    float *cur = pick({Q_, Y_});
    PlaneChain chain;
    chain.next = d >= 2;
    bool first_done = false;
    if (u.it == 0 && u.ru_ok && u.n_ritz == m_) {
        coeff_.alloc(rank_coeff_bytes(cap_ < 160 ? cap_ : 160, ru_.kmax));
        if (prof_) prof_->begin(PROF_RANK_UPDATE);
        first_done = rank_first_term(Y_, Q_, F_, m_, F_, ru_.beta / e0, -c0 / e0, -ru_.alpha / e0, cur, ru_.proj, ru_.ldp,
                                     u.ru_nw, wscale_.p, ru_.slot, ru_.w, ru_.k_dev, ru_.kmax, ru_.planes, coeff_.p,
                                     chain.next ? plane_hi_.p : nullptr, plane_lo_.p, s_, ru_.coeff_ready, ru_.planes_mode);
        if (prof_) prof_->end(PROF_RANK_UPDATE);
        if (first_done) {
            st_.rank_update_passes++;
            chain.planes_of = chain.next ? cur : nullptr;
            chain.rows = m_;
            if (ru_check_) check_first_term(u, cur);
        }
    }
    if (!first_done) product(Q_, m_, u.G, -1.0f / e0, cur, Q_, -c0 / e0, nullptr, 0.f, true, &chain);
    for (int k = 2; k <= d; k++) {
        float *nxt = pick({prev, cur});
        chain.next = k < d;
        product(cur, m_, u.G, -2.0f / e0, nxt, cur, -2.0f * c0 / e0, prev, -1.0f, true, &chain);
        prev = cur; cur = nxt;
    }
    return cur;
}

void EigTracker::check_first_term(const UpdateState &u, const float *cur)
{
    const float c0 = u.plan.c0, e0 = u.plan.e0;
    float *ref = pick({Q_, Y_, cur});
    std::vector<char> ph(bf16x2_plane_bytes(m_, F_)), pl(ph.size());
    DLCO_HIP(hipMemcpyAsync(ph.data(), plane_hi_.p, ph.size(), hipMemcpyDeviceToHost, s_));
    DLCO_HIP(hipMemcpyAsync(pl.data(), plane_lo_.p, pl.size(), hipMemcpyDeviceToHost, s_));
    product(Q_, m_, u.G, -1.0f / e0, ref, Q_, -c0 / e0, nullptr, 0.f, true);
    std::vector<float> a((size_t)m_ * F_), b(a.size());
    DLCO_HIP(hipMemcpyAsync(a.data(), cur, a.size() * sizeof(float), hipMemcpyDeviceToHost, s_));
    DLCO_HIP(hipMemcpyAsync(b.data(), ref, b.size() * sizeof(float), hipMemcpyDeviceToHost, s_));
    DLCO_HIP(hipMemcpyAsync(plane_hi_.p, ph.data(), ph.size(), hipMemcpyHostToDevice, s_));
    DLCO_HIP(hipMemcpyAsync(plane_lo_.p, pl.data(), pl.size(), hipMemcpyHostToDevice, s_));
    DLCO_HIP(hipStreamSynchronize(s_));
    double dmax = 0.0, rmax = 0.0;
    for (size_t e = 0; e < a.size(); e++) { dmax = std::max(dmax, (double)std::fabs(a[e] - b[e])); rmax = std::max(rmax, (double)std::fabs(b[e])); }
    st_.rank_update_check = std::max(st_.rank_update_check, rmax > 0.0 ? dmax / rmax : 0.0);
    st_.product_rows -= m_;
}

void EigTracker::rayleigh_ritz(UpdateState &u, float *Qo)
{
    float *Yb = pick({Qo});
    product(Qo, m_, u.G, -1.0f, Yb, nullptr, 0.f, nullptr, 0.f, false);
    gram_rect(Yb, m_, Qo, m_, Tm_.p);
    if (prof_) prof_->begin(PROF_JACOBI);
    const float lam_cut = eig_rules::jacobi_lam_cut(block_of(u), have_theta_ && u.n_ritz == m_);
    float *Qn = pick({Qo, Yb});
    float *Yn = pick({Qo, Yb, Qn});
    u.w_emitted = false;
    const size_t blk = (size_t)2 * (cap_ + 8) + 1;
    for (int attempt = 0;; attempt++) {
        jacobi_eigh(Tm_.p, cap_, m_, evals_.p, Vm_.p, cap_, jwork_.p, sweeps_dev_, s_, lam_cut, attempt > 0);
        if (prof_) prof_->end(PROF_JACOBI);
        rotate(Vm_.p, cap_, m_, m_, Qo, Qn, Yb, Yn);
        Q_ = Qn; Y_ = Yn;
        y_ok_ = true;
        unsigned *flag = reinterpret_cast<unsigned *>(pin_ + pin_floats_ - 16);
        const unsigned seq = ++publish_seq_;
        int *extra_host = reinterpret_cast<int *>(pin_ + pin_floats_ - 32);
        ResidualEmit em;
        em.W = u.W; em.ldw = F_; em.mu = u.mu; em.cscale = u.cscale; em.wscale = wscale_.p; em.guards = emit_guards_;
        residual_norms_publish(Q_, Y_, F_, evals_.p, m_, F_, res_.p, reinterpret_cast<unsigned *>(sweeps_dev_ + 4), ritz_block_.p, pin_,
                               (int)blk, flag, seq, s_, extra_dev_, extra_host, &em, &u.w_emitted);
        const auto t0 = std::chrono::steady_clock::now();
        bool seen = false;
        for (long spins = 0;; spins++) {
            if (__atomic_load_n(flag, __ATOMIC_ACQUIRE) == seq) { seen = true; break; }
            if ((spins & 1023) == 1023 && std::chrono::steady_clock::now() - t0 > std::chrono::milliseconds(200)) break;
        }
        if (!seen) {
            DLCO_HIP(hipStreamSynchronize(s_));
            DLCO_CHECK(__atomic_load_n(flag, __ATOMIC_ACQUIRE) == seq, -3, "eig tracker: read-back did not arrive");
        }
        if (extra_dev_) extra_val_ = *reinterpret_cast<int *>(pin_ + pin_floats_ - 32);
        const int sweeps = *reinterpret_cast<int *>(pin_ + 2 * (cap_ + 8));
        if (sweeps >= 0) { st_.jacobi_sweeps += sweeps; break; }
        st_.jacobi_barrier_timeouts++;
        DLCO_CHECK(attempt == 0, -3, "eig tracker: the Jacobi kernel reported a failure twice (grid barrier of jacobi_mw_kernel, then the single-workgroup kernel)");
        if (prof_) prof_->begin(PROF_JACOBI);
    }
    std::memcpy(h_theta_.data(), pin_, (size_t)m_ * sizeof(float));
    std::memcpy(h_res_.data(), pin_ + (cap_ + 8), (size_t)m_ * sizeof(float));
    have_theta_ = true;
    const int before = m_;
    theta_dev_valid_ = (drop_dead_rows() == before);
    u.theta_top = h_theta_[0];
    u.block_min = std::min(h_theta_[m_ - 1], u.mu);
    u.n_ritz = m_;
}

void EigTracker::judge(UpdateState &u)
{
    const eig_rules::Verdict v = eig_rules::judge(block_of(u), u.it);
    u.nw = v.nw;
    u.conv = v.conv;
    last_crit_ = v.crit;
    if (debug_)
        std::fprintf(stderr, "[eig] upd %ld it %d deg %d lock %d m %d nw %d theta[%.5g .. %.5g] mu %.5g lo %.5g crit/emax %.3g guards_ok %d conv %d\n",
                     (long)st_.updates, u.it, last_deg_, u.plan.n_lock, m_, u.nw, h_theta_[0], h_theta_[m_ - 1], u.mu, lo_bound_, last_crit_,
                     (int)v.guards_ok, (int)u.conv);
    lo_bound_ = eig_rules::lowered_bound(lo_bound_, h_theta_[m_ - 1]);
}

void EigTracker::grow(UpdateState &u)
{
    const int add = eig_rules::growth_rows(m_, cap_, guard_, u.nw);
    int got = 0;
    if (grow_cb_) got = std::max(0, std::min(add / 2, grow_cb_(Q_ + (size_t)m_ * F_, add / 2)));
    append_random(Q_, m_ + got, add - got);
    for (int i = m_; i < m_ + add; i++) { h_theta_[i] = u.block_min; h_res_[i] = 0.f; }
    m_ += add;
}

double EigTracker::trim_and_emit(UpdateState &u)
{
    st_.iters += u.it;
    deg0_ = eig_rules::next_deg0(deg0_, u.it, u.conv, last_crit_, tol_);
    if (!u.conv) st_.nonconverged++;
    m_ = eig_rules::trimmed_rows(m_, u.nw, guard_);
    const int nw = u.nw;
    double tr = 0.0;
    if (nw > 0) {
        for (int i = 0; i < nw; i++) tr += (double)(u.cscale * (h_theta_[i] - u.mu));
        if (theta_dev_valid_) {
            const bool ext = emit_guards_ && y_ok_ && m_ > nw;
            if (!u.w_emitted) emit_w_rows(u.W, F_, Q_, F_, evals_.p, nw, u.mu, u.cscale, F_, s_, ext ? m_ : 0, ext ? wscale_.p : nullptr);
            if (ext) { wext_rows_ = m_; wext_nw_ = nw; }
        } else {
            h_sc_.resize(nw);
            h_sr_.resize(nw);
            for (int j = 0; j < nw; j++) {
                const int i = nw - 1 - j;
                h_sc_[j] = std::sqrt(u.cscale * (h_theta_[i] - u.mu));
                h_sr_[j] = i;
            }
            DLCO_HIP(hipMemcpyAsync(scale_.p, h_sc_.data(), nw * sizeof(float), hipMemcpyHostToDevice, s_));
            DLCO_HIP(hipMemcpyAsync(srcrow_.p, h_sr_.data(), nw * sizeof(int32_t), hipMemcpyHostToDevice, s_));
            DLCO_HIP(hipStreamSynchronize(s_));
            scale_rows(u.W, F_, Q_, F_, scale_.p, srcrow_.p, nw, F_, s_);
        }
    }
    return tr;
}

}
```

### opencv-dlco_amd/csrc/eig_tracker.hpp

```cpp
#pragma once

#include "dlco_internal.hpp"
#include "eig_rules.hpp"

#include <functional>
#include <initializer_list>

namespace dlco {

struct EigStats {
    int64_t iters = 0, product_rows = 0, jacobi_sweeps = 0, updates = 0, nonconverged = 0, cheap_passes = 0;
    int64_t jacobi_barrier_timeouts = 0;
    int64_t locked_passes = 0, locked_rows = 0;
    int64_t rank_update_passes = 0;
    double rank_update_check = 0.0;
};

struct RankUpdate {
    const float *proj = nullptr;
    long ldp = 0;
    int rows = 0;
    const int32_t *slot = nullptr;
    const float *w = nullptr;
    const int *k_dev = nullptr;
    int kmax = 0;
    const void *planes = nullptr;
    float alpha = 0.f, beta = 1.f;
    int planes_mode = 3;
    bool coeff_ready = false;
};

class EigTracker {
public:
    EigTracker(int F, int max_rows, int guard, float tol, int max_iter, hipStream_t stream, int live_cols = 0);
    ~EigTracker();

    void reset();
    void seed_rows(const float *src, long ld, const int32_t *ids_dev, int n, const int32_t *ids2_dev = nullptr);

    int update(const float *G, float mu, float cscale, float *W, double *trace, bool *converged);

    int block_rows() const { return m_; }
    void set_profiler(Profiler *p) { prof_ = p; }
    void set_shard(const ShardComm *sc) { shard_ = sc; }
    void set_readback_extra(const int *dev) { extra_dev_ = dev; }
    void set_growth_rows(std::function<int(float *dst, int want)> cb) { grow_cb_ = std::move(cb); }
    int readback_extra() const { return extra_val_; }
    void set_emit_guards(bool on) { emit_guards_ = on; }
    int ext_rows() const { return wext_rows_; }
    void offer_rank_update(const RankUpdate &ru) { ru_ = ru; ru_offered_ = true; }
    bool rank_coeff_job(RankCoeffJob *job, int kmax);
    void set_packed(bool on) { packed_ = on; }
    bool packed() const { return packed_; }
    static bool packed_supported(int F) { return F % 128 == 0 && F / 128 <= 64 && env_switch("DLCO_NO_PACKED") == nullptr; }
    const EigStats &stats() const { return st_; }
    float last_crit() const { return last_crit_; }

private:
    struct UpdateState;
    struct PlaneChain;
    void open_update(UpdateState &u);
    eig_rules::Block block_of(const UpdateState &u) const;
    float *filter_cheap(const UpdateState &u);
    float *filter_locked(const UpdateState &u);
    float *filter_plain(const UpdateState &u);
    void check_first_term(const UpdateState &u, const float *cur);
    void rayleigh_ritz(UpdateState &u, float *Qo);
    void judge(UpdateState &u);
    void grow(UpdateState &u);
    double trim_and_emit(UpdateState &u);

    void product(const float *X, int rows, const float *G, float alpha, float *out, const float *E1, float b1,
                 const float *E2, float b2, bool approx, PlaneChain *chain = nullptr);
    void gram_rect(const float *X, int xrows, const float *Y, int yrows, float *T);
    void project_out(float *Wp, int np, const float *Q, int kept);
    void rotate(const float *C, long ldc, int k_in, int k_out, const float *X, float *out, const float *X2 = nullptr, float *out2 = nullptr);
    int orthonormalize(float *Z, int rows, float *scratch, const std::vector<int> &panel_ends, int skip = 0);
    int drop_dead_rows();
    void refresh_lower_bound(const float *G, int iters, float theta_top);
    void append_random(float *Q, int have, int add);
    float next_uniform();
    float *pick(std::initializer_list<const float *> busy) const;

    int F_, live_, cap_, guard_, max_iter_;
    float tol_;
    std::function<int(float *, int)> grow_cb_;
    const int *extra_dev_ = nullptr;
    int extra_val_ = 0;
    bool packed_ = false;
    bool emit_guards_ = false;
    int wext_rows_ = 0, wext_nw_ = 0;
    RankUpdate ru_;
    bool ru_offered_ = false;
    bool ru_check_ = env_switch("DLCO_RANK_UPDATE_CHECK") != nullptr;
    DevBuf<float> wscale_;
    DevBuf<char> coeff_;
    bool cold_ = true;
    hipStream_t s_;
    int m_ = 0;
    bool have_theta_ = false;
    bool theta_dev_valid_ = false;
    float lo_bound_ = 0.f;
    bool have_lo_ = false;
    int steps_since_lo_ = 0;
    uint64_t rng_ = 0x243F6A8885A308D3ULL;
    float last_crit_ = 0.f;
    int deg0_ = 4;
    int last_deg_ = 0;
    bool y_ok_ = false;
    bool lock_ = env_switch("DLCO_NO_LOCKING") == nullptr;
    bool debug_ = env_switch("DLCO_EIG_DEBUG") != nullptr;

    DevBuf<float> buf_[6];
    float *all_[6] = {nullptr, nullptr, nullptr, nullptr, nullptr, nullptr};
    float *Q_ = nullptr, *Y_ = nullptr;
    DevBuf<float> Tm_, Vm_, Cw_, jwork_, slab_, pv_, pw_, scale_;
    struct FView { float *p = nullptr; };
    DevBuf<float> ritz_block_;
    FView evals_, res_;
    int *sweeps_dev_ = nullptr;
    DevBuf<int32_t> srcrow_;
    int ks_ = 4;
    DevBuf<char> plane_hi_, plane_lo_, plane_lo2_;
    DevBuf<int> dead_;
    size_t slab_floats_ = 0;
    std::vector<float> h_theta_, h_res_, h_tmp_, h_sc_;
    std::vector<int32_t> h_sr_;
    float *pin_ = nullptr;
    unsigned publish_seq_ = 0;
    size_t pin_floats_ = 0;
    EigStats st_;
    Profiler *prof_ = nullptr;
    const ShardComm *shard_ = nullptr;
};

}
```

### opencv-dlco_amd/csrc/kernels_bf16x2.hip

```cpp
#include "dlco_internal.hpp"
#include "split_bf16_dev.hpp"

#include <algorithm>

namespace dlco {

namespace {

constexpr int W8 = 8;
constexpr int T8 = 64 * W8;
constexpr int KS = 4;

__global__ __launch_bounds__(256) void split_x_kernel(const float *X, long ldx, int M, int MT, int K, bf16x8 *hi, bf16x8 *lo,
                                                      bf16x8 *lo2)
{
    const long t = (long)blockIdx.x * blockDim.x + threadIdx.x;
    const long total = (long)(K / 16) * MT * 64;
    if (t >= total) return;
    const int lane = (int)(t & 63);
    const long q = t >> 6;
    const int tile = (int)(q % MT);
    const int k16 = (int)(q / MT);
    const int row = tile * 32 + (lane & 31), k = k16 * 16 + 8 * (lane >> 5);
    bf16x8 h, l, l2;
// ... 323 lines not shown
        struct Stage { f32x4 gq[8]; bf16x8 aq[NA]; };
        Stage s0, s1;
        auto gload = [&](int cc, Stage &st) {
            const int J = __builtin_amdgcn_readfirstlane(partner(cc)), half = cc & 1;
            const bool direct = I <= J;
            const int voff = direct ? voff_d : voff_t;
            const int soff = tile_bytes(J) + (direct ? half * 64 : half * 64 * 128) * (int)sizeof(float);
            const int ustep = (direct ? 16 : 8) * 128 * (int)sizeof(float);
            const int a0 = slice_bytes<MT>(J * 8 + half * 4);
            __builtin_amdgcn_sched_barrier(0);
#pragma unroll
            for (int u = 0; u < 8; u++) {
                st.gq[u] = __builtin_bit_cast(f32x4, __builtin_amdgcn_raw_buffer_load_b128(rsrc, voff, soff + u * ustep, 0));
                __builtin_amdgcn_sched_barrier(0);
            }
#pragma unroll
            for (int v = 0; v < NA; v++) {
                st.aq[v] = load_slice_entry<MT>(rs, a0, lt, v);
                __builtin_amdgcn_sched_barrier(0);
            }
        };
        auto gstore = [&](int cc, const Stage &st) {
            float *gb = (cc & 1) ? gb1 : gb0;
            bf16x8 *ab = (cc & 1) ? ab1 : ab0;
            const bool direct = I <= partner(cc);
            const int loff = direct ? loff_d : loff_t, lstep = direct ? 16 * SB_RS : 8 * SYM_TS;
#pragma unroll
            for (int u = 0; u < 8; u++) *reinterpret_cast<f32x4 *>(gb + loff + u * lstep) = st.gq[u];
#pragma unroll
            for (int v = 0; v < NA; v++) ab[lt + 256 * v] = st.aq[v];
        };
        gload(0, s0);
        gload(1, s1);
        gstore(0, s0);
        gload(min(2, nchunks - 1), s0);
        __syncthreads();
        int cc = 0;
        for (; cc + 4 < nchunks; cc += 2) {
            gstore(cc + 1, s1); gload(cc + 3, s1); __syncthreads();
            gstore(cc + 2, s0); gload(cc + 4, s0); __syncthreads();
        }
        for (; cc < nchunks; cc += 2) {
            if (cc + 1 < nchunks) gstore(cc + 1, s1);
            if (cc + 3 < nchunks) gload(cc + 3, s1);
            __syncthreads();
            if (cc + 2 < nchunks) gstore(cc + 2, s0);
            if (cc + 4 < nchunks) gload(cc + 4, s0);
            __syncthreads();
        }
        __syncthreads();
        return;
    }

    const int lc = lane & 31, lh = lane >> 5;
    const int nt = wave & 3, kh = wave >> 2;
    f32x16 acc[MT];
#pragma unroll
    for (int a = 0; a < MT; a++)
#pragma unroll
        for (int r = 0; r < 16; r++) acc[a][r] = 0.f;

    auto fetch = [&](const float *gb, const bf16x8 *ab, bool direct, int q, Frag<MT, NS> &f) {
        if (direct) {
            const float *pp = gb + (nt * 32 + lc) * SB_RS + 16 * q + 8 * lh;
            f.g0 = *reinterpret_cast<const f32x4 *>(pp);
            f.g1 = *reinterpret_cast<const f32x4 *>(pp + 4);
        } else {
            const float *pp = gb + (16 * q + 8 * lh) * SYM_TS + nt * 32 + lc;
#pragma unroll
            for (int j = 0; j < 4; j++) { f.g0[j] = pp[j * SYM_TS]; f.g1[j] = pp[(4 + j) * SYM_TS]; }
        }
#pragma unroll
        for (int n = 0; n < NS; n++)
#pragma unroll
            for (int t = 0; t < MT; t++) f.a[n][t] = ab[n * APLANE + plane_entry(q, MT, t, lane)];
    };
    auto multiply = [&](const Frag<MT, NS> &f) {
        bf16x8 bh, bl, bl2;
        split_frag<NS>(f.g0, f.g1, bh, bl, bl2);
        mfma_split_terms<MT, NS>(f.a[0], f.a[NS >= 2 ? 1 : 0], f.a[NS - 1], bh, bl, bl2, acc);
    };
    Frag<MT, NS> fa;
    __syncthreads();
    for (int cc = 0; cc < nchunks; cc++) {
        const float *gb = (cc & 1) ? gb1 : gb0;
        const bf16x8 *ab = (cc & 1) ? ab1 : ab0;
        const bool direct = I <= partner(cc);
        fetch(gb, ab, direct, 2 * kh, fa);
        multiply(fa);
        fetch(gb, ab, direct, 2 * kh + 1, fa);
        multiply(fa);
        __syncthreads();
    }

    float *red = reinterpret_cast<float *>(lds_raw);
    if (kh == 1) {
#pragma unroll
        for (int a = 0; a < MT; a++)
#pragma unroll
            for (int r = 0; r < 16; r++) red[((nt * MT + a) * 16 + r) * 64 + lane] = acc[a][r];
    }
    __syncthreads();
    if (kh == 0) {
        float *slab = g.slab + (long)p * g.M * g.K;
        const int col = I * 128 + nt * 32 + lc;
#pragma unroll
        for (int a = 0; a < MT; a++)
#pragma unroll
            for (int r = 0; r < 16; r++) {
                const float sum = acc[a][r] + red[((nt * MT + a) * 16 + r) * 64 + lane];
                const int i = a * 32 + (r & 3) + 8 * (r >> 2) + 4 * lh;
                if (i < g.M) slab[(long)i * g.K + col] = sum;
            }
    }
}

template <int MT, int NS>
void launch_sym(const SymDev &g, hipStream_t s)
{
    const size_t lds = sb_lds_bytes(MT, NS);
    if (g.nt == (1 << g.lb)) {
        ensure_dynamic_lds(reinterpret_cast<const void *>(skinny_sym_kernel<MT, NS, true>), (int)lds);
        hipLaunchKernelGGL((skinny_sym_kernel<MT, NS, true>), dim3(4u << g.lb), dim3(SB_T), lds, s, g);
    } else {
        ensure_dynamic_lds(reinterpret_cast<const void *>(skinny_sym_kernel<MT, NS, false>), (int)lds);
        hipLaunchKernelGGL((skinny_sym_kernel<MT, NS, false>), dim3(4u << g.lb), dim3(SB_T), lds, s, g);
    }
}

template <int MT, int NS>
void launch_rows(const Bf2Dev &g, dim3 grid, hipStream_t s)
{
    const size_t lds = sb_lds_bytes(MT, NS);
    ensure_dynamic_lds(reinterpret_cast<const void *>(skinny_rows_kernel<MT, NS>), (int)lds);
    hipLaunchKernelGGL((skinny_rows_kernel<MT, NS>), grid, dim3(SB_T), lds, s, g);
}

}

void split_planes_bf16(const float *X, long ldx, int M, int K, void *hi, void *lo, void *lo2, hipStream_t s)
{
    const int mt = (M + 31) / 32;
    const long total = (long)(K / 16) * mt * 64;
    hipLaunchKernelGGL(split_x_kernel, dim3((unsigned)((total + 255) / 256)), dim3(256), 0, s, X, ldx, M, mt, K,
                       static_cast<bf16x8 *>(hi), static_cast<bf16x8 *>(lo), static_cast<bf16x8 *>(lo2));
    DLCO_HIP(hipGetLastError());
}

size_t bf16x2_plane_bytes(int M, int K) { return (size_t)((M + 31) / 32) * 32 * K * sizeof(__bf16); }
size_t bf16x2_slab_floats(int M, int N, int ksplit) { return (size_t)(ksplit > 0 ? ksplit : KS) * M * N; }

bool skinny_product_bf16x2(const float *X, long ldx, int M, const float *G, long ldg, int N, int K, float alpha, float *C,
                           long ldc, const float *E1, float b1, const float *E2, float b2, void *plane_hi, void *plane_lo,
                           float *slab, hipStream_t s, int ksplit, void *plane_lo2, bool g_tiled)
{
    const int mt = (M + 31) / 32;
    const int ks = ksplit > 0 ? ksplit : KS;
    if (M < 1 || mt > 5 || N % 128 != 0 || K % (16 * ks * 2 * 4) != 0) return false;
    if (ldx % 4 != 0 || (reinterpret_cast<uintptr_t>(X) & 15) != 0) return false;
    split_planes_bf16(X, ldx, M, K, plane_hi, plane_lo, plane_lo2, s);
    Bf2Dev g;
    g.M = M; g.N = N; g.K = K;
    g.xhi = static_cast<const bf16x8 *>(plane_hi); g.xlo = static_cast<const bf16x8 *>(plane_lo);
    g.xlo2 = static_cast<const bf16x8 *>(plane_lo2);
    g.G = G; g.ldg = ldg; g.slab = slab; g.tiled = g_tiled ? 1 : 0;
    const dim3 grid(N / 128, ks), block(T8);
    if (N == K && K % (128 * ks) == 0 && ldg % 4 == 0 && (reinterpret_cast<uintptr_t>(G) & 15) == 0 &&
        (long)K * ldg * 4 < (1L << 31) && !(mt >= 4 && plane_lo2)) {
        if (plane_lo2) dispatch_mt<4>(mt, [&](auto MT) { launch_rows<MT(), 3>(g, grid, s); });
        else dispatch_mt<5>(mt, [&](auto MT) { launch_rows<MT(), 2>(g, grid, s); });
        DLCO_HIP(hipGetLastError());
        splitk_reduce_f32(slab, ks, M, N, C, ldc, alpha, 0.f, E1, b1, E2, b2, s);
        return true;
    }
    if (g_tiled || mt > 4) return false;
    if (plane_lo2) dispatch_mt<4>(mt, [&](auto MT) { hipLaunchKernelGGL((skinny_bf16x2_kernel<MT(), 3>), grid, block, 0, s, g); });
    else dispatch_mt<4>(mt, [&](auto MT) { hipLaunchKernelGGL((skinny_bf16x2_kernel<MT(), 2>), grid, block, 0, s, g); });
    DLCO_HIP(hipGetLastError());
    splitk_reduce_f32(slab, ks, M, N, C, ldc, alpha, 0.f, E1, b1, E2, b2, s);
    return true;
}

bool skinny_product_sym(const float *X, long ldx, int M, const float *Gpacked, int F, float alpha, float *C, long ldc,
                        const float *E1, float b1, const float *E2, float b2, void *plane_hi, void *plane_lo, float *slab,
                        hipStream_t s, void *plane_lo2, bool planes_ready, bool emit_planes)
{
    const int mt = (M + 31) / 32;
    const int nt = F / 128;
    if (F % 128 != 0 || nt < 1 || nt > 64 || M < 1 || mt > 5 || (mt >= 4 && plane_lo2)) return false;
    if (ldx % 4 != 0 || (reinterpret_cast<uintptr_t>(X) & 15) != 0 || (reinterpret_cast<uintptr_t>(Gpacked) & 15) != 0) return false;
    if ((planes_ready || emit_planes) && plane_lo2) return false;
    if (!planes_ready) split_planes_bf16(X, ldx, M, F, plane_hi, plane_lo, plane_lo2, s);
    SymDev g;
    g.M = M; g.K = F;
    g.nt = nt; g.lb = 2;
    while ((1 << g.lb) < nt) g.lb++;
    g.xhi = static_cast<const bf16x8 *>(plane_hi); g.xlo = static_cast<const bf16x8 *>(plane_lo); g.xlo2 = static_cast<const bf16x8 *>(plane_lo2);
    g.G = Gpacked; g.slab = slab;
    if (plane_lo2) dispatch_mt<3>(mt, [&](auto MT) { launch_sym<MT(), 3>(g, s); });
    else dispatch_mt<5>(mt, [&](auto MT) { launch_sym<MT(), 2>(g, s); });
    DLCO_HIP(hipGetLastError());
    if (emit_planes && ldc % 4 == 0 && (reinterpret_cast<uintptr_t>(C) & 15) == 0) {
        const long work = (long)M * (F / 8);
        hipLaunchKernelGGL(reduce_split_kernel, dim3((unsigned)std::min<long>((work + 255) / 256, 4096)), dim3(256), 0, s, slab, 4, M, mt, F, C, ldc,
                           alpha, E1, b1, E2, b2, static_cast<bf16x8 *>(plane_hi), static_cast<bf16x8 *>(plane_lo));
        DLCO_HIP(hipGetLastError());
    } else {
        splitk_reduce_f32(slab, 4, M, F, C, ldc, alpha, 0.f, E1, b1, E2, b2, s);
    }
    return true;
}

}
```

### opencv-dlco_amd/csrc/kernels_eig.hip

```cpp
#include "dlco_internal.hpp"

#include <type_traits>

namespace dlco {

namespace {

typedef float f32x4 __attribute__((ext_vector_type(4)));

__device__ __forceinline__ float wsum(float v)
{
#pragma unroll
    for (int o = 32; o > 0; o >>= 1) v += __shfl_xor(v, o, 64);
    return v;
}

__global__ __launch_bounds__(256) void residual_kernel(const float *X, const float *Y, long ld, const float *theta,
                                                       int m, int F, float *res)
{
    __shared__ float part[4];
    const int i = blockIdx.x;
    if (i >= m) return;
    const float th = theta[i];
    float s = 0.f;
    if ((F & 3) == 0 && (ld & 3) == 0) {
        const f32x4 *y4 = reinterpret_cast<const f32x4 *>(Y + (long)i * ld), *x4 = reinterpret_cast<const f32x4 *>(X + (long)i * ld);
        for (int f = threadIdx.x; f < F / 4; f += blockDim.x) {
            const f32x4 d = y4[f] - th * x4[f];
            s += d[0] * d[0] + d[1] * d[1] + d[2] * d[2] + d[3] * d[3];
        }
    } else {
        for (int f = threadIdx.x; f < F; f += blockDim.x) {
            const float d = Y[(long)i * ld + f] - th * X[(long)i * ld + f];
            s += d * d;
        }
    }
    s = wsum(s);
    if ((threadIdx.x & 63) == 0) part[threadIdx.x >> 6] = s;
    __syncthreads();
    if (threadIdx.x == 0) res[i] = sqrtf(part[0] + part[1] + part[2] + part[3]);
}

__global__ __launch_bounds__(256) void row_normalize_kernel(float *X, long ld, int m, int F, float min_norm)
{
    __shared__ float part[4];
    __shared__ float inv;
    const int i = blockIdx.x;
    if (i >= m) return;
    float s = 0.f;
    const bool vec = (F & 3) == 0 && (ld & 3) == 0;
    f32x4 *x4 = reinterpret_cast<f32x4 *>(X + (long)i * ld);
    if (vec) {
        for (int f = threadIdx.x; f < F / 4; f += blockDim.x) { const f32x4 v = x4[f]; s += v[0] * v[0] + v[1] * v[1] + v[2] * v[2] + v[3] * v[3]; }
    } else {
        for (int f = threadIdx.x; f < F; f += blockDim.x) { const float v = X[(long)i * ld + f]; s += v * v; }
    }
    s = wsum(s);
    if ((threadIdx.x & 63) == 0) part[threadIdx.x >> 6] = s;
    __syncthreads();
    if (threadIdx.x == 0) { const float n2 = part[0] + part[1] + part[2] + part[3]; inv = (n2 > 0.f && n2 >= min_norm * min_norm) ? 1.f / sqrtf(n2) : 0.f; }
    __syncthreads();
    const float sc = inv;
    if (vec) {
        for (int f = threadIdx.x; f < F / 4; f += blockDim.x) x4[f] = x4[f] * sc;
    } else {
        for (int f = threadIdx.x; f < F; f += blockDim.x) X[(long)i * ld + f] *= sc;
    }
}

__global__ __launch_bounds__(256) void symv_kernel(const float *H, long ld, int F, const float *x, float *y)
{
    const int row = blockIdx.x * 4 + (threadIdx.x >> 6), lane = threadIdx.x & 63;
    if (row >= F) return;
    float s = 0.f;
    for (int f = lane; f < F; f += 64) s += H[(long)row * ld + f] * x[f];
    s = wsum(s);
    if (lane == 0) y[row] = s;
}

constexpr int C2_T = 1024;
__host__ __device__ constexpr int c2_pld(int nbm) { return 64 * nbm + 4; }
__host__ __device__ constexpr size_t c2_lds_floats(int nbm)
{
    return (size_t)2 * 32 * 33 + 2 * 32 * c2_pld(nbm) + 2 * 32 * nbm * 33 + 32 * nbm * 3 + 64 + 2 * nbm * nbm * 64;
}

__device__ __forceinline__ float readlane_f(float v, int l) { return __int_as_float(__builtin_amdgcn_readlane(__float_as_int(v), l)); }

template <int NBM>
__global__ __launch_bounds__(C2_T) void chol_inv2_kernel(const float *M, long ldm, int n, float rel_thresh, float *Linv, long ldl,
                                                         int *dead)
{
    extern __shared__ __attribute__((aligned(16))) float c2[];
    float (*Dblk)[33] = reinterpret_cast<float (*)[33]>(c2);
    float (*Tblk)[33] = reinterpret_cast<float (*)[33]>(c2 + 32 * 33);
    constexpr int C2_PLD = c2_pld(NBM), NR = 32 * NBM;
    float (*Praw)[C2_PLD] = reinterpret_cast<float (*)[C2_PLD]>(c2 + 2 * 32 * 33);
    float (*Pbuf)[C2_PLD] = reinterpret_cast<float (*)[C2_PLD]>(c2 + 2 * 32 * 33 + 32 * C2_PLD);
    float (*Acol)[33] = reinterpret_cast<float (*)[33]>(c2 + 2 * 32 * 33 + 2 * 32 * C2_PLD);
    float (*Fbuf)[33] = reinterpret_cast<float (*)[33]>(c2 + 2 * 32 * 33 + 2 * 32 * C2_PLD + NR * 33);
    float *diag0 = c2 + 2 * 32 * 33 + 2 * 32 * C2_PLD + 2 * NR * 33;
    float *dpiv = diag0 + NR;
    int *deadf = reinterpret_cast<int *>(dpiv + NR);
    float *dinv = dpiv + 2 * NR;
    float *stash = dinv + 64;
    const int t = threadIdx.x, tx = t & 31, ty = t >> 5;
    const int nb = (n + 31) >> 5;

    float reg[NBM][2 * NBM];
#pragma unroll
    for (int r = 0; r < NBM; r++)
#pragma unroll
        for (int c = 0; c < NBM; c++) {
            const int i = 32 * r + ty, k = 32 * c + tx;
            reg[r][c] = (i < n && k < n) ? M[(long)max(i, k) * ldm + min(i, k)] : ((i == k) ? 1.f : 0.f);
            reg[r][NBM + c] = (i == k) ? 1.f : 0.f;
        }
    if (t < NR) { diag0[t] = t < n ? M[(long)t * ldm + t] : 1.f; deadf[t] = 0; dpiv[t] = 1.f; }
    {
        float e2 = 0.f;
#pragma unroll
        for (int r = 0; r < NBM; r++)
#pragma unroll
            for (int c = 0; c < NBM; c++) { const float e = reg[r][c] - ((32 * r + ty == 32 * c + tx) ? 1.f : 0.f); e2 += e * e; }
        e2 = wsum(e2);
        if ((t & 63) == 0) dinv[32 + (t >> 6)] = e2;
    }
    __syncthreads();
    {
        float tot = 0.f;
        for (int w = 0; w < C2_T / 64; w++) tot += dinv[32 + w];
        if (tot <= 1e-6f) {
#pragma unroll
            for (int r = 0; r < NBM; r++)
#pragma unroll
                for (int c = 0; c < NBM; c++) {
                    const int i = 32 * r + ty, k = 32 * c + tx;
                    if (i < n && k < n) Linv[(long)i * ldl + k] = ((i == k) ? 1.5f : 0.f) - 0.5f * reg[r][c];
                }
            if (t < n) dead[t] = 0;
            return;
        }
    }

    auto block = [&](auto KBc) {
        constexpr int kb = decltype(KBc)::value;
        if (kb < nb) {
            Dblk[ty][tx] = reg[kb][kb];
            __syncthreads();
            if (t < 64) {
#pragma unroll
                for (int r = 0; r < NBM; r++)
#pragma unroll
                    for (int c = 0; c < 2 * NBM; c++) stash[(r * 2 * NBM + c) * 64 + t] = reg[r][c];
                const int i = t & 31;
                float a[32], x[32];
#pragma unroll
                for (int k = 0; k < 32; k++) { a[k] = Dblk[i][k]; x[k] = (i == k) ? 1.f : 0.f; }
                const float d0_mine = diag0[32 * kb + i];
#pragma unroll
                for (int j = 0; j < 32; j++) {
                    const float piv = readlane_f(a[j], j);
                    const float d0 = readlane_f(d0_mine, j);
                    const bool dd = !(piv > rel_thresh * d0) || !(d0 > 0.f);
                    const float rinv = dd ? 0.f : __builtin_amdgcn_rcpf(piv);
                    if (t == 0) { dpiv[32 * kb + j] = piv; deadf[32 * kb + j] = dd ? 1 : 0; dinv[j] = rinv; }
                    const float f = (i > j) ? a[j] * rinv : 0.f;
#pragma unroll
                    for (int k = j + 1; k < 32; k++) a[k] -= f * readlane_f(a[k], j);
#pragma unroll
                    for (int k = 0; k <= j; k++) x[k] -= f * readlane_f(x[k], j);
                }
                if (t < 32) {
#pragma unroll
                    for (int k = 0; k < 32; k++) Tblk[i][k] = x[k];
                }
#pragma unroll
                for (int r = 0; r < NBM; r++)
#pragma unroll
                    for (int c = 0; c < 2 * NBM; c++) reg[r][c] = stash[(r * 2 * NBM + c) * 64 + t];
            }
#pragma unroll
            for (int c = 0; c < NBM; c++) {
                if (c > kb && c < nb) Praw[ty][32 * c + tx] = reg[kb][c];
                if (c <= kb) Praw[ty][NR + 32 * c + tx] = reg[kb][NBM + c];
            }
#pragma unroll
            for (int r = 0; r < NBM; r++)
                if (r > kb && r < nb) Acol[32 * r + ty][tx] = reg[r][kb];
            __syncthreads();
            {
                float pacc[2 * NBM];
#pragma unroll
                for (int c = 0; c < 2 * NBM; c++) pacc[c] = 0.f;
#pragma unroll 2
                for (int j = 0; j < 32; j++) {
                    const float tj = Tblk[ty][j];
#pragma unroll
                    for (int c = 0; c < NBM; c++) {
                        if (c > kb && c < nb) pacc[c] += tj * Praw[j][32 * c + tx];
                        if (c <= kb) pacc[NBM + c] += tj * Praw[j][NR + 32 * c + tx];
                    }
                }
#pragma unroll
                for (int c = 0; c < NBM; c++) {
                    if (c > kb && c < nb) { reg[kb][c] = pacc[c]; Pbuf[ty][32 * c + tx] = pacc[c]; }
                    if (c <= kb) { reg[kb][NBM + c] = pacc[NBM + c]; Pbuf[ty][NR + 32 * c + tx] = pacc[NBM + c]; }
                }
                const float di = dinv[tx];
#pragma unroll
                for (int r = 0; r < NBM; r++) {
                    if (r > kb && r < nb) {
                        float facc = 0.f;
#pragma unroll 4
                        for (int l = 0; l < 32; l++) facc += Tblk[tx][l] * Acol[32 * r + ty][l];
                        Fbuf[32 * r + ty][tx] = facc * di;
                    }
                }
            }
            __syncthreads();
            if (kb + 1 < nb) {
#pragma unroll 2
                for (int j = 0; j < 32; j++) {
                    float fr[NBM], pc[2 * NBM];
#pragma unroll
                    for (int r = 0; r < NBM; r++) fr[r] = (r > kb && r < nb) ? Fbuf[32 * r + ty][j] : 0.f;
#pragma unroll
                    for (int c = 0; c < NBM; c++) {
                        pc[c] = (c > kb && c < nb) ? Pbuf[j][32 * c + tx] : 0.f;
                        pc[NBM + c] = (c <= kb) ? Pbuf[j][NR + 32 * c + tx] : 0.f;
                    }
#pragma unroll
                    for (int r = 0; r < NBM; r++) {
                        if (r > kb) {
#pragma unroll
                            for (int c = 0; c < NBM; c++) {
                                if (c > kb) reg[r][c] -= fr[r] * pc[c];
                                if (c <= kb) reg[r][NBM + c] -= fr[r] * pc[NBM + c];
                            }
                        }
                    }
                }
            }
        }
    };
    block(std::integral_constant<int, 0>{});
    block(std::integral_constant<int, 1>{});
    block(std::integral_constant<int, 2>{});
    if constexpr (NBM > 3) block(std::integral_constant<int, 3>{});
    if constexpr (NBM > 4) block(std::integral_constant<int, NBM - 1>{});
    __syncthreads();
#pragma unroll
    for (int r = 0; r < NBM; r++) {
        const int i = 32 * r + ty;
        if (i < n) {
            const float sc = deadf[i] ? 0.f : rsqrtf(dpiv[i]);
#pragma unroll
            for (int c = 0; c < NBM; c++) {
                const int k = 32 * c + tx;
                if (k < n) Linv[(long)i * ldl + k] = (k <= i) ? reg[r][NBM + c] * sc : 0.f;
            }
        }
    }
    if (t < n) dead[t] = deadf[t];
}

}

template <int NBM>
static void launch_chol_inv2(const float *M, long ldm, int n, float rel_thresh, float *Linv, long ldl, int *dead, hipStream_t s)
{
    ensure_dynamic_lds(reinterpret_cast<const void *>(chol_inv2_kernel<NBM>), (int)(c2_lds_floats(NBM) * sizeof(float)));
    hipLaunchKernelGGL(chol_inv2_kernel<NBM>, dim3(1), dim3(C2_T), c2_lds_floats(NBM) * sizeof(float), s, M, ldm, n, rel_thresh, Linv, ldl, dead);
}

void chol_inverse128(const float *M, long ldm, int n, float rel_thresh, float *Linv, long ldl, int *dead, hipStream_t s)
{
    DLCO_CHECK(n >= 1 && n <= CHOL_INV_MAX_N, -2, "chol_inverse128: n out of range");
    if (n <= 96) launch_chol_inv2<3>(M, ldm, n, rel_thresh, Linv, ldl, dead, s);
    else if (n <= 128) launch_chol_inv2<4>(M, ldm, n, rel_thresh, Linv, ldl, dead, s);
    else launch_chol_inv2<5>(M, ldm, n, rel_thresh, Linv, ldl, dead, s);
    DLCO_HIP(hipGetLastError());
}

__global__ __launch_bounds__(256) void residual_publish_kernel(const float *X, const float *Y, long ld, const float *theta, int m, int F,
                                                               float *res, unsigned *ticket, const float *src, float *dst_host, int n,
                                                               unsigned *flag_host, unsigned seq, const int *extra_dev, int *extra_host,
                                                               ResidualEmit em)
{
    __shared__ float part[4];
    __shared__ int last;
    __shared__ int cnt[4];
    const int i = blockIdx.x;
    const float th = theta[i];
    float s = 0.f;
    if (em.W && (F & 3) == 0 && (ld & 3) == 0 && (em.ldw & 3) == 0) {
        int c = 0;
        for (int k = threadIdx.x; k < m; k += blockDim.x) c += theta[k] > em.mu ? 1 : 0;
        c = (int)wsum((float)c);
        if ((threadIdx.x & 63) == 0) cnt[threadIdx.x >> 6] = c;
        __syncthreads();
        const int nw = cnt[0] + cnt[1] + cnt[2] + cnt[3];
        const bool mine = i < nw || em.guards;
        const float sc = i < nw ? sqrtf(em.cscale * (th - em.mu)) : 1.0f;
        f32x4 *w4 = reinterpret_cast<f32x4 *>(em.W + (long)(i < nw ? nw - 1 - i : i) * em.ldw);
        if (em.wscale && threadIdx.x == 0) em.wscale[i] = sc;
        const f32x4 *y4 = reinterpret_cast<const f32x4 *>(Y + (long)i * ld), *x4 = reinterpret_cast<const f32x4 *>(X + (long)i * ld);
        for (int f = threadIdx.x; f < F / 4; f += blockDim.x) {
            const f32x4 x = x4[f];
            const f32x4 d = y4[f] - th * x;
            s += d[0] * d[0] + d[1] * d[1] + d[2] * d[2] + d[3] * d[3];
            if (mine) { f32x4 v = x; v[0] *= sc; v[1] *= sc; v[2] *= sc; v[3] *= sc; w4[f] = v; }
        }
    } else if ((F & 3) == 0 && (ld & 3) == 0) {
        const f32x4 *y4 = reinterpret_cast<const f32x4 *>(Y + (long)i * ld), *x4 = reinterpret_cast<const f32x4 *>(X + (long)i * ld);
        for (int f = threadIdx.x; f < F / 4; f += blockDim.x) {
            const f32x4 d = y4[f] - th * x4[f];
            s += d[0] * d[0] + d[1] * d[1] + d[2] * d[2] + d[3] * d[3];
        }
    } else {
        for (int f = threadIdx.x; f < F; f += blockDim.x) {
            const float d = Y[(long)i * ld + f] - th * X[(long)i * ld + f];
            s += d * d;
        }
    }
    s = wsum(s);
    if ((threadIdx.x & 63) == 0) part[threadIdx.x >> 6] = s;
    __syncthreads();
    if (threadIdx.x == 0) {
        __hip_atomic_store(res + i, sqrtf(part[0] + part[1] + part[2] + part[3]), __ATOMIC_RELAXED, __HIP_MEMORY_SCOPE_AGENT);
        const unsigned t = __hip_atomic_fetch_add(ticket, 1u, __ATOMIC_ACQ_REL, __HIP_MEMORY_SCOPE_AGENT);
        last = t == gridDim.x - 1 ? 1 : 0;
        if (last) __hip_atomic_store(ticket, 0u, __ATOMIC_RELAXED, __HIP_MEMORY_SCOPE_AGENT);
    }
    __syncthreads();
    if (!last) return;
    __builtin_amdgcn_fence(__ATOMIC_ACQUIRE, "agent");
    for (int k = threadIdx.x; k < n; k += 256) dst_host[k] = __hip_atomic_load(src + k, __ATOMIC_RELAXED, __HIP_MEMORY_SCOPE_AGENT);
    if (extra_dev && threadIdx.x == 0) *extra_host = __hip_atomic_load(extra_dev, __ATOMIC_RELAXED, __HIP_MEMORY_SCOPE_AGENT);
    __threadfence_system();
    __syncthreads();
    if (threadIdx.x == 0) __hip_atomic_store(flag_host, seq, __ATOMIC_RELEASE, __HIP_MEMORY_SCOPE_SYSTEM);
}

void residual_norms_publish(const float *X, const float *Y, long ld, const float *theta, int m, int F, float *res, unsigned *ticket,
                            const float *src, float *dst_host, int n, unsigned *flag_host, unsigned seq, hipStream_t s,
                            const int *extra_dev, int *extra_host, const ResidualEmit *emit, bool *emitted)
{
    DLCO_CHECK(m > 0, -2, "residual_norms_publish: empty block");
    ResidualEmit em;
    if (emit && emit->W && (F & 3) == 0 && (ld & 3) == 0 && (emit->ldw & 3) == 0 && (reinterpret_cast<uintptr_t>(emit->W) & 15) == 0) em = *emit;
    if (emitted) *emitted = em.W != nullptr;
    hipLaunchKernelGGL(residual_publish_kernel, dim3(m), dim3(256), 0, s, X, Y, ld, theta, m, F, res, ticket, src, dst_host, n, flag_host,
                       seq, extra_dev, extra_host, em);
    DLCO_HIP(hipGetLastError());
}

void residual_norms(const float *X, const float *Y, long ld, const float *theta, int m, int F, float *res,
                    hipStream_t s)
{
    if (m <= 0) return;
    hipLaunchKernelGGL(residual_kernel, dim3(m), dim3(256), 0, s, X, Y, ld, theta, m, F, res);
    DLCO_HIP(hipGetLastError());
}

void row_normalize(float *X, long ld, int m, int F, hipStream_t s, float min_norm)
{
    if (m <= 0) return;
    hipLaunchKernelGGL(row_normalize_kernel, dim3(m), dim3(256), 0, s, X, ld, m, F, min_norm);
    DLCO_HIP(hipGetLastError());
}

void symv(const float *H, long ld, int F, const float *x, float *y, hipStream_t s)
{
    hipLaunchKernelGGL(symv_kernel, dim3((F + 3) / 4), dim3(256), 0, s, H, ld, F, x, y);
    DLCO_HIP(hipGetLastError());
}

}
```

### opencv-dlco_amd/csrc/kernels_gemm.hip

```cpp
#include "dlco_internal.hpp"

namespace dlco {

typedef float f32x16 __attribute__((ext_vector_type(16)));
typedef float f32x4 __attribute__((ext_vector_type(4)));

namespace {

constexpr int BK = 16;
constexpr int PAD = 4;
constexpr int NT = 256;

struct OperandDev {
    const float *p;
    long ld;
    const int32_t *row_ids;
    const float *row_scale;
    int vec_ok;
    const int32_t *row_ids2;
};

__device__ __forceinline__ f32x4 load4(const float *src, int pos, int limit, int vec_ok)
{
    f32x4 v = {0.f, 0.f, 0.f, 0.f};
    if (vec_ok && pos + 3 < limit) {
        v = *reinterpret_cast<const f32x4 *>(src);
    } else {
        v[0] = src[0];
        if (pos + 1 < limit) v[1] = src[1];
        if (pos + 2 < limit) v[2] = src[2];
        if (pos + 3 < limit) v[3] = src[3];
    }
    return v;
}

struct GemmDev {
    int M, N, K;
    OperandDev A, B;
    float *C;
    long ldc;
    float alpha, beta, b1, b2;
    const float *E1, *E2;
    const int *k_dev;
    int k_chunk;
    float *slab;
    int upper_only;
    const float *B2;
    float *C2;
};

template <int BT, bool KM>
__device__ __forceinline__ void load_tile(const OperandDev &op, int t0, int tmax, int k0, int kend,
                                          f32x4 (&regs)[BT / 64])
{
    const int tid = threadIdx.x;
#pragma unroll
    for (int u = 0; u < BT / 64; u++) {
        const int f = tid + NT * u;
        f32x4 v = {0.f, 0.f, 0.f, 0.f};
        if (KM) {
            const int row = f / (BT / 4), c4 = f % (BT / 4);
            const int k = k0 + row, col = t0 + c4 * 4;
            if (k < kend && col < tmax) {
                const long mr = op.row_ids ? (long)op.row_ids[k] : (long)k;
                v = load4(op.p + mr * op.ld + col, col, tmax, op.vec_ok);
                if (op.row_ids2) v -= load4(op.p + (long)op.row_ids2[k] * op.ld + col, col, tmax, op.vec_ok);
                if (op.row_scale) {
                    const float sc = op.row_scale[k];
                    v *= sc;
                }
            }
        } else {
            const int row = f / (BK / 4), kq = f % (BK / 4);
            const int t = t0 + row, k = k0 + kq * 4;
            if (t < tmax && k < kend) {
                const long mr = op.row_ids ? (long)op.row_ids[t] : (long)t;
                v = load4(op.p + mr * op.ld + k, k, kend, op.vec_ok);
                if (op.row_ids2) v -= load4(op.p + (long)op.row_ids2[t] * op.ld + k, k, kend, op.vec_ok);
            }
        }
        regs[u] = v;
    }
}

template <int BT, bool KM>
__device__ __forceinline__ void store_tile(float (*lds)[BT + PAD], const f32x4 (&regs)[BT / 64])
{
    const int tid = threadIdx.x;
#pragma unroll
    for (int u = 0; u < BT / 64; u++) {
        const int f = tid + NT * u;
        if (KM) {
            const int row = f / (BT / 4), c4 = f % (BT / 4);
            *reinterpret_cast<f32x4 *>(&lds[row][c4 * 4]) = regs[u];
        } else {
            const int row = f / (BK / 4), kq = f % (BK / 4);
            lds[kq * 4 + 0][row] = regs[u][0];
            lds[kq * 4 + 1][row] = regs[u][1];
            lds[kq * 4 + 2][row] = regs[u][2];
            lds[kq * 4 + 3][row] = regs[u][3];
        }
    }
}

template <int WM, int WN, bool A_KM, bool B_KM>
__global__ __launch_bounds__(NT) void gemm_kernel(GemmDev g)
{
    constexpr int BM = 64 * WM, BN = 64 * WN;
    __shared__ __attribute__((aligned(16))) float As[2][BK][BM + PAD];
    __shared__ __attribute__((aligned(16))) float Bs[2][BK][BN + PAD];

    const int bi = blockIdx.y, bj = blockIdx.x;
    if (g.upper_only && bj * BN + BN <= bi * BM) return;
    const int i0 = bi * BM, j0 = bj * BN;
    const int lane = threadIdx.x & 63, wave = threadIdx.x >> 6;
    const int wm = wave >> 1, wn = wave & 1;

    int kz = blockIdx.z;
    if (g.B2) {
        if (kz == 1) { g.B.p = g.B2; g.C = g.C2; }
        kz = 0;
    }
    int kbeg = kz * g.k_chunk;
    int kend = min(g.K, kbeg + g.k_chunk);
    if (g.k_dev) kend = min(kend, *g.k_dev);

    f32x16 acc[WM][WN];
#pragma unroll
    for (int a = 0; a < WM; a++)
#pragma unroll
        for (int b = 0; b < WN; b++)
#pragma unroll
            for (int r = 0; r < 16; r++) acc[a][b][r] = 0.f;

    const int nk = kend > kbeg ? (kend - kbeg + BK - 1) / BK : 0;
    f32x4 ra[BM / 64], rb[BN / 64];
    if (nk > 0) {
        load_tile<BM, A_KM>(g.A, i0, g.M, kbeg, kend, ra);
        load_tile<BN, B_KM>(g.B, j0, g.N, kbeg, kend, rb);
        store_tile<BM, A_KM>(As[0], ra);
        store_tile<BN, B_KM>(Bs[0], rb);
    }
    __syncthreads();
    for (int kt = 0; kt < nk; kt++) {
        const int buf = kt & 1;
        if (kt + 1 < nk) {
            load_tile<BM, A_KM>(g.A, i0, g.M, kbeg + (kt + 1) * BK, kend, ra);
            load_tile<BN, B_KM>(g.B, j0, g.N, kbeg + (kt + 1) * BK, kend, rb);
        }
        const int lr = lane & 31, lk = lane >> 5;
#pragma unroll
        for (int kk = 0; kk < BK / 2; kk++) {
            float af[WM], bf[WN];
#pragma unroll
            for (int a = 0; a < WM; a++) af[a] = As[buf][2 * kk + lk][wm * 32 * WM + a * 32 + lr];
#pragma unroll
            for (int b = 0; b < WN; b++) bf[b] = Bs[buf][2 * kk + lk][wn * 32 * WN + b * 32 + lr];
#pragma unroll
            for (int a = 0; a < WM; a++)
#pragma unroll
                for (int b = 0; b < WN; b++)
                    acc[a][b] = __builtin_amdgcn_mfma_f32_32x32x2f32(af[a], bf[b], acc[a][b], 0, 0, 0);
        }
        if (kt + 1 < nk) {
            store_tile<BM, A_KM>(As[buf ^ 1], ra);
            store_tile<BN, B_KM>(Bs[buf ^ 1], rb);
        }
        __syncthreads();
    }

    const int lc = lane & 31, lh = lane >> 5;
#pragma unroll
    for (int a = 0; a < WM; a++)
#pragma unroll
        for (int b = 0; b < WN; b++)
#pragma unroll
            for (int r = 0; r < 16; r++) {
                const int i = i0 + wm * 32 * WM + a * 32 + (r & 3) + 8 * (r >> 2) + 4 * lh;
                const int j = j0 + wn * 32 * WN + b * 32 + lc;
                if (i >= g.M || j >= g.N) continue;
                if (g.slab) {
                    g.slab[((long)blockIdx.z * g.M + i) * g.N + j] = acc[a][b][r];
                    continue;
                }
                if (g.upper_only && j < i) continue;
                const long idx = (long)i * g.ldc + j;
                float o = g.alpha * acc[a][b][r];
                if (g.beta != 0.f) o += g.beta * g.C[idx];
                if (g.E1) o += g.b1 * g.E1[idx];
                if (g.E2) o += g.b2 * g.E2[idx];
                g.C[idx] = o;
                if (g.upper_only && j > i) g.C[(long)j * g.ldc + i] = o;
            }
}

__global__ void splitk_reduce_kernel(const float *slab, int split, int M, int N, float *C, long ldc, float alpha,
                                     float beta, const float *E1, float b1, const float *E2, float b2)
{
    const long total = (long)M * N;
    const int zl = threadIdx.x & 15;
    for (long e = ((long)blockIdx.x * blockDim.x + threadIdx.x) >> 4; e < total; e += ((long)gridDim.x * blockDim.x) >> 4) {
        const int i = (int)(e / N), j = (int)(e % N);
        float s = 0.f;
        for (int z = zl; z < split; z += 16) s += slab[(long)z * total + e];
        s += __int_as_float(__builtin_amdgcn_update_dpp(0, __float_as_int(s), 0xB1, 0xF, 0xF, true));
        s += __int_as_float(__builtin_amdgcn_update_dpp(0, __float_as_int(s), 0x4E, 0xF, 0xF, true));
        s += __int_as_float(__builtin_amdgcn_update_dpp(0, __float_as_int(s), 0x141, 0xF, 0xF, true));
        s += __int_as_float(__builtin_amdgcn_update_dpp(0, __float_as_int(s), 0x140, 0xF, 0xF, true));
        if (zl != 0) continue;
        const long idx = (long)i * ldc + j;
        float o = alpha * s;
        if (beta != 0.f) o += beta * C[idx];
        if (E1) o += b1 * E1[idx];
        if (E2) o += b2 * E2[idx];
        C[idx] = o;
    }
}

__global__ __launch_bounds__(256) void splitk_reduce_wide_kernel(const float *slab, int split, int M, int N, float *C,
                                                                 long ldc, float alpha, float beta, const float *E1,
                                                                 float b1, const float *E2, float b2)
{
    const long total = (long)M * N, q = N >> 2;
    for (long e = (long)blockIdx.x * blockDim.x + threadIdx.x; e < (long)M * q; e += (long)gridDim.x * blockDim.x) {
        const int i = (int)(e / q), j = (int)(e % q) * 4;
        const float *p = slab + (long)i * N + j;
        f32x4 s = *reinterpret_cast<const f32x4 *>(p);
        for (int z = 1; z < split; z++) s += *reinterpret_cast<const f32x4 *>(p + (long)z * total);
        const long idx = (long)i * ldc + j;
        f32x4 o = alpha * s;
        if (beta != 0.f) o += beta * *reinterpret_cast<const f32x4 *>(C + idx);
        if (E1) o += b1 * *reinterpret_cast<const f32x4 *>(E1 + idx);
        if (E2) o += b2 * *reinterpret_cast<const f32x4 *>(E2 + idx);
        *reinterpret_cast<f32x4 *>(C + idx) = o;
    }
}

template <int WM, int WN>
void launch(const GemmDev &g, bool akm, bool bkm, dim3 grid, hipStream_t s)
{
    if (akm && bkm) hipLaunchKernelGGL((gemm_kernel<WM, WN, true, true>), grid, dim3(NT), 0, s, g);
    else if (akm && !bkm) hipLaunchKernelGGL((gemm_kernel<WM, WN, true, false>), grid, dim3(NT), 0, s, g);
    else if (!akm && bkm) hipLaunchKernelGGL((gemm_kernel<WM, WN, false, true>), grid, dim3(NT), 0, s, g);
    else hipLaunchKernelGGL((gemm_kernel<WM, WN, false, false>), grid, dim3(NT), 0, s, g);
}

inline int vec_ok(const GemmOperand &o) { return (o.ld % 4 == 0) && ((reinterpret_cast<uintptr_t>(o.p) & 15) == 0); }

}

size_t gemm_slab_floats(int M, int N, int split_k) { return split_k > 1 ? (size_t)split_k * M * N : 0; }

void splitk_reduce_f32(const float *slab, int split, int M, int N, float *C, long ldc, float alpha, float beta,
                       const float *E1, float b1, const float *E2, float b2, hipStream_t s)
{
    const long total = (long)M * N;
    auto al16 = [](const void *p) { return (reinterpret_cast<uintptr_t>(p) & 15) == 0; };
    if (split <= 32 && total >= 65536 && N % 4 == 0 && ldc % 4 == 0 && al16(slab) && al16(C) && (!E1 || al16(E1)) &&
        (!E2 || al16(E2))) {
        long blocks = (total / 4 + 255) / 256;
        if (blocks > 4096) blocks = 4096;
        hipLaunchKernelGGL(splitk_reduce_wide_kernel, dim3((unsigned)blocks), dim3(256), 0, s, slab, split, M, N, C, ldc, alpha,
                           beta, E1, b1, E2, b2);
        DLCO_HIP(hipGetLastError());
        return;
    }
    long blocks = (total * 16 + 255) / 256;
    if (blocks > 8192) blocks = 8192;
    hipLaunchKernelGGL(splitk_reduce_kernel, dim3((unsigned)blocks), dim3(256), 0, s, slab, split, M, N, C, ldc, alpha, beta,
                       E1, b1, E2, b2);
    DLCO_HIP(hipGetLastError());
}

void gemm_f32(const GemmArgs &a, hipStream_t s)
{
    if (a.M <= 0 || a.N <= 0) return;
    DLCO_CHECK(a.A.p && a.B.p && a.C, -2, "gemm_f32: null operand");
    DLCO_CHECK(!(a.upper_only && (a.M != a.N || a.split_k > 1)), -2, "gemm_f32: upper_only needs M==N, split_k==1");
    GemmDev g;
    g.M = a.M; g.N = a.N; g.K = a.K;
    g.A = {a.A.p, a.A.ld, a.A.row_ids, a.A.kmajor ? a.A.row_scale : nullptr, vec_ok(a.A), a.A.row_ids2};
    g.B = {a.B.p, a.B.ld, a.B.row_ids, a.B.kmajor ? a.B.row_scale : nullptr, vec_ok(a.B), a.B.row_ids2};
    g.C = a.C; g.ldc = a.ldc;
    g.alpha = a.alpha; g.beta = a.beta; g.E1 = a.E1; g.b1 = a.b1; g.E2 = a.E2; g.b2 = a.b2;
    g.k_dev = a.k_dev;
    g.upper_only = a.upper_only ? 1 : 0;
    int split = a.split_k < 1 ? 1 : a.split_k;
    int chunk = (a.K + split - 1) / split;
    chunk = ((chunk + BK - 1) / BK) * BK;
    if (chunk < BK) chunk = BK;
    split = a.K > 0 ? (a.K + chunk - 1) / chunk : 1;
    g.k_chunk = chunk;
    g.slab = nullptr;
    if (split > 1) {
        DLCO_CHECK(a.slab != nullptr, -2, "gemm_f32: split_k > 1 needs a slab workspace");
        g.slab = a.slab;
    }
    g.B2 = a.B2; g.C2 = a.C2;
    if (a.B2) {
        DLCO_CHECK(a.C2 && split == 1 && !a.upper_only, -2, "gemm_f32: a twin product needs C2 and no K split");
        split = 2;
    }
    bool small_m = a.M <= 64 || a.small_m_tiles, small_n = a.N <= 64 || a.small_n_tiles;
    auto n_wg = [&](bool sm, bool sn) {
        return (long)((a.M + (sm ? 63 : 127)) / (sm ? 64 : 128)) * ((a.N + (sn ? 63 : 127)) / (sn ? 64 : 128)) * split;
    };
    if (!a.upper_only) {
        if (!small_m && n_wg(small_m, small_n) < 256) small_m = true;
        if (!small_n && n_wg(small_m, small_n) < 256) small_n = true;
    }
    if (small_m && small_n) {
        dim3 grid((a.N + 63) / 64, (a.M + 63) / 64, split);
        launch<1, 1>(g, a.A.kmajor, a.B.kmajor, grid, s);
    } else if (small_m) {
        dim3 grid((a.N + 127) / 128, (a.M + 63) / 64, split);
        launch<1, 2>(g, a.A.kmajor, a.B.kmajor, grid, s);
    } else if (small_n) {
        dim3 grid((a.N + 63) / 64, (a.M + 127) / 128, split);
        launch<2, 1>(g, a.A.kmajor, a.B.kmajor, grid, s);
    } else {
        dim3 grid((a.N + 127) / 128, (a.M + 127) / 128, split);
        launch<2, 2>(g, a.A.kmajor, a.B.kmajor, grid, s);
    }
    DLCO_HIP(hipGetLastError());
    if (split > 1 && !a.B2)
        splitk_reduce_f32(a.slab, split, a.M, a.N, a.C, a.ldc, a.alpha, a.beta, a.E1, a.b1, a.E2, a.b2, s);
}

}
```

Baseline: 710,500 pair-rows/s.

## Fold Cholesky orthonormalization into Rayleigh-Ritz and emit bf16 planes from GEMM epilogue

For single-panel blocks, orthonormalization now uses a Gram matrix, an inverse Cholesky factor and a GEMM instead of row normalization plus panel passes. The GEMM epilogue writes the split bf16 hi/lo/lo2 planes directly, so the next product can skip re-splitting. Rayleigh-Ritz computes both Gram products in one twin-A split-K GEMM, and a fused single-block kernel does the Cholesky inverse plus the small projected-matrix products. This is meant to cut kernel launches and redundant passes over the F-wide block in the eigen-tracker. The cost is more code paths, and the Cholesky-based orthonormalization may be less numerically robust.

Result: slower. 693,200 pair-rows/s (-2.4%).

```diff
diff --git a/include/dlco.h b/include/dlco.h
--- a/include/dlco.h
+++ b/include/dlco.h
@@ -107,6 +107,11 @@
                      float *W_host, int32_t *r, float *A_host );
 int dlco_sym_product(dlco_ctx *ctx, const float *X_host, int32_t rows, const float *G_host, int32_t mode,
                      float *out_host);
+int dlco_ritz_prepare(dlco_ctx *ctx, const float *Z1_host, const float *Y1_host, int32_t rows, int32_t mode,
+                      float *S_host, float *T_host, int32_t *dead_host);
+int dlco_apply_planes(dlco_ctx *ctx, const float *L_host, const float *Z_host, int32_t rows, int32_t mode,
+                      float *out_host, uint16_t *hi_host, uint16_t *lo_host, uint16_t *lo2_host);
+int dlco_eig_block(dlco_ctx *ctx, float *Q_host, float *Y_host, int32_t *rows);
 int dlco_hinge_sum(dlco_ctx *ctx, const float *pos_host, int32_t n_pos,
                    const float *neg_host, int32_t n_neg, double *out);
 int dlco_roc_stats(dlco_ctx *ctx, const float *dist_host, const uint8_t *labels_host, int32_t n,
diff --git a/opencv-dlco_amd/__init__.py b/opencv-dlco_amd/__init__.py
--- a/opencv-dlco_amd/__init__.py
+++ b/opencv-dlco_amd/__init__.py
@@ -103,6 +103,10 @@
     L.dlco_psd_project.argtypes = [vp, f32p, C.c_uint32, f32p, i32p, f32p]
     L.dlco_hinge_sum.argtypes = [vp, f32p, C.c_int32, f32p, C.c_int32, C.POINTER(C.c_double)]
     L.dlco_sym_product.argtypes = [vp, f32p, C.c_int32, f32p, C.c_int32, f32p]
+    L.dlco_ritz_prepare.argtypes = [vp, f32p, f32p, C.c_int32, C.c_int32, f32p, f32p, i32p]
+    L.dlco_apply_planes.argtypes = [vp, f32p, f32p, C.c_int32, C.c_int32, f32p, C.POINTER(C.c_uint16), C.POINTER(C.c_uint16),
+                                    C.POINTER(C.c_uint16)]
+    L.dlco_eig_block.argtypes = [vp, f32p, f32p, i32p]
     L.dlco_roc_stats.argtypes = [vp, f32p, u8p, C.c_int32, f32p, C.POINTER(C.c_double)]
     L.dlco_log_step.argtypes = [vp, C.POINTER(LogEntry)]
     L.dlco_get_saved.argtypes = [vp, f32p, i32p, f32p]
@@ -423,6 +427,29 @@
         self._ck(self.L.dlco_sym_product(self.h, _p(x, f32p), x.shape[0], _p(g, f32p), mode, _p(out, f32p)))
         return out
 
+    def ritz_prepare(self, Z1, Y1, mode=0):
+        z, y = _f32(Z1), _f32(Y1)
+        n = z.shape[0]
+        S, T, dead = np.empty((n, n), np.float32), np.empty((n, n), np.float32), np.empty(n, np.int32)
+        self._ck(self.L.dlco_ritz_prepare(self.h, _p(z, f32p), _p(y, f32p), n, mode, _p(S, f32p), _p(T, f32p), _p(dead, i32p)))
+        return S, T, dead
+
+    def apply_planes(self, Lm, Z, mode=0):
+        l, z = _f32(Lm), _f32(Z)
+        n, F = z.shape
+        out = np.empty_like(z)
+        u16p = C.POINTER(C.c_uint16)
+        planes = [np.empty(((n + 31) // 32) * 32 * F, np.uint16) for _ in range(3)]
+        self._ck(self.L.dlco_apply_planes(self.h, _p(l, f32p), _p(z, f32p), n, mode, _p(out, f32p), *[_p(p, u16p) for p in planes]))
+        return out, planes
+
+    def eig_block(self):
+        rows = C.c_int32()
+        self._ck(self.L.dlco_eig_block(self.h, None, None, C.byref(rows)))
+        Q, Y = np.empty((rows.value, self.F), np.float32), np.empty((rows.value, self.F), np.float32)
+        self._ck(self.L.dlco_eig_block(self.h, _p(Q, f32p), _p(Y, f32p), C.byref(rows)))
+        return Q, Y
+
     def hinge_sum(self, pos, neg):
         p, n = _f32(pos), _f32(neg)
         out = C.c_double()
diff --git a/opencv-dlco_amd/csrc/dlco_api.cpp b/opencv-dlco_amd/csrc/dlco_api.cpp
--- a/opencv-dlco_amd/csrc/dlco_api.cpp
+++ b/opencv-dlco_amd/csrc/dlco_api.cpp
@@ -1165,6 +1165,102 @@
     });
 }
 
+int dlco_ritz_prepare(dlco_ctx *c, const float *Z1_host, const float *Y1_host, int32_t rows, int32_t mode, float *S_host, float *T_host,
+                      int32_t *dead_host)
+{
+    if (!c || !Z1_host || !Y1_host || !S_host || !T_host || !dead_host || rows < 1 || rows > CHOL_INV_MAX_N || mode < 0 || mode > 1)
+        return DLCO_ERR_INVALID;
+    return guarded(c, [&] {
+        DLCO_HIP(hipSetDevice(c->cfg.device));
+        DLCO_CHECK(c->Fu == c->F, DLCO_ERR_INVALID, "dlco_ritz_prepare: the context's width must need no padding");
+        const int F = c->F, n = rows;
+        DevBuf<float> Z, Y, Q2, Y2, MT, S, T, U, slab;
+        DevBuf<int> dead;
+        Z.alloc((size_t)n * F); Y.alloc((size_t)n * F); MT.alloc((size_t)2 * n * n); S.alloc((size_t)n * n); T.alloc((size_t)n * n);
+        U.alloc((size_t)n * n); dead.alloc(n);
+        h2d(c, Z.p, Z1_host, (size_t)n * F * sizeof(float));
+        h2d(c, Y.p, Y1_host, (size_t)n * F * sizeof(float));
+        const long kslice = std::max(64L, (long)F / 64 / 64 * 64);
+        const int split = split_k_slices(n <= 64 ? 1 : 4, 512, F, kslice);
+        slab.alloc((size_t)2 * split * n * n);
+        auto gram = [&](const float *A, const float *A2, const float *B, float *C) {
+            GemmArgs g;
+            g.M = n; g.N = n; g.K = F;
+            g.A.p = A; g.A.ld = F; g.A2 = A2;
+            g.B.p = B; g.B.ld = F;
+            g.C = C; g.ldc = n;
+            g.split_k = split; g.slab = slab.p;
+            gemm_f32(g, c->stream);
+        };
+        if (mode == 0) {
+            gram(Z.p, Y.p, Z.p, MT.p);
+            ritz_prepare(MT.p, n, n, 1e-5f, S.p, n, T.p, n, U.p, n, dead.p, c->stream);
+        } else {
+            Q2.alloc((size_t)n * F); Y2.alloc((size_t)n * F);
+            gram(Z.p, nullptr, Z.p, MT.p);
+            chol_inverse128(MT.p, n, n, 1e-5f, S.p, n, dead.p, c->stream);
+            GemmArgs g;
+            g.M = n; g.N = F; g.K = n;
+            g.A.p = S.p; g.A.ld = n;
+            g.B.p = Z.p; g.B.ld = F; g.B.kmajor = true;
+            g.C = Q2.p; g.ldc = F;
+            g.B2 = Y.p; g.C2 = Y2.p;
+            gemm_f32(g, c->stream);
+            gram(Y2.p, nullptr, Q2.p, T.p);
+        }
+        d2h(c, S_host, S.p, (size_t)n * n * sizeof(float));
+        d2h(c, T_host, T.p, (size_t)n * n * sizeof(float));
+        d2h(c, dead_host, dead.p, (size_t)n * sizeof(int));
+    });
+}
+
+int dlco_apply_planes(dlco_ctx *c, const float *L_host, const float *Z_host, int32_t rows, int32_t mode, float *out_host, uint16_t *hi_host,
+                      uint16_t *lo_host, uint16_t *lo2_host)
+{
+    if (!c || !L_host || !Z_host || !out_host || !hi_host || !lo_host || !lo2_host || rows < 1 || rows > 160 || mode < 0 || mode > 1)
+        return DLCO_ERR_INVALID;
+    return guarded(c, [&] {
+        DLCO_HIP(hipSetDevice(c->cfg.device));
+        DLCO_CHECK(c->Fu == c->F && c->F % 64 == 0, DLCO_ERR_INVALID, "dlco_apply_planes: the width must be whole 64-column tiles");
+        const int F = c->F, n = rows;
+        const size_t pb = bf16x2_plane_bytes(n, F);
+        DevBuf<float> L, Z, out;
+        DevBuf<char> hi, lo, lo2;
+        L.alloc((size_t)n * n); Z.alloc((size_t)n * F); out.alloc((size_t)n * F);
+        hi.alloc(pb); lo.alloc(pb); lo2.alloc(pb);
+        h2d(c, L.p, L_host, (size_t)n * n * sizeof(float));
+        h2d(c, Z.p, Z_host, (size_t)n * F * sizeof(float));
+        DLCO_HIP(hipMemsetAsync(hi.p, 0xFF, pb, c->stream));
+        DLCO_HIP(hipMemsetAsync(lo.p, 0xFF, pb, c->stream));
+        DLCO_HIP(hipMemsetAsync(lo2.p, 0xFF, pb, c->stream));
+        GemmArgs g;
+        g.M = n; g.N = F; g.K = n;
+        g.A.p = L.p; g.A.ld = n;
+        g.B.p = Z.p; g.B.ld = F; g.B.kmajor = true;
+        g.C = out.p; g.ldc = F;
+        if (mode == 0) { g.plane_hi = hi.p; g.plane_lo = lo.p; g.plane_lo2 = lo2.p; }
+        gemm_f32(g, c->stream);
+        if (mode == 1) split_planes_bf16(out.p, F, n, F, hi.p, lo.p, lo2.p, c->stream);
+        d2h(c, out_host, out.p, (size_t)n * F * sizeof(float));
+        d2h(c, hi_host, hi.p, pb);
+        d2h(c, lo_host, lo.p, pb);
+        d2h(c, lo2_host, lo2.p, pb);
+    });
+}
+
+int dlco_eig_block(dlco_ctx *c, float *Q_host, float *Y_host, int32_t *rows)
+{
+    if (!c || !rows) return DLCO_ERR_INVALID;
+    return guarded(c, [&] {
+        DLCO_HIP(hipSetDevice(c->cfg.device));
+        DLCO_CHECK(c->phase == 0, DLCO_ERR_INVALID, "dlco_eig_block: step in flight");
+        sync(c);
+        *rows = c->eig->block_rows();
+        if (Q_host) d2h_rows(c, Q_host, c->eig->block_q(), (size_t)*rows);
+        if (Y_host) d2h_rows(c, Y_host, c->eig->block_y(), (size_t)*rows);
+    });
+}
+
 int dlco_hinge_sum(dlco_ctx *c, const float *pos_host, int32_t n_pos, const float *neg_host, int32_t n_neg, double *out)
 {
     if (!c || !out || n_pos < 0 || n_neg < 0) return DLCO_ERR_INVALID;
diff --git a/opencv-dlco_amd/csrc/dlco_internal.hpp b/opencv-dlco_amd/csrc/dlco_internal.hpp
--- a/opencv-dlco_amd/csrc/dlco_internal.hpp
+++ b/opencv-dlco_amd/csrc/dlco_internal.hpp
@@ -172,6 +172,10 @@
     bool upper_only = false;
     const float *B2 = nullptr;
     float *C2 = nullptr;
+    const float *A2 = nullptr;
+    void *plane_hi = nullptr;
+    void *plane_lo = nullptr;
+    void *plane_lo2 = nullptr;
     bool small_m_tiles = false;
     bool small_n_tiles = false;
 };
@@ -182,7 +186,8 @@
 void split_planes_bf16(const float *X, long ldx, int M, int K, void *hi, void *lo, void *lo2, hipStream_t s);
 bool skinny_product_bf16x2(const float *X, long ldx, int M, const float *G, long ldg, int N, int K, float alpha, float *C,
                            long ldc, const float *E1, float b1, const float *E2, float b2, void *plane_hi, void *plane_lo,
-                           float *slab, hipStream_t s, int ksplit = 0, void *plane_lo2 = nullptr, bool g_tiled = false);
+                           float *slab, hipStream_t s, int ksplit = 0, void *plane_lo2 = nullptr, bool g_tiled = false,
+                           bool planes_ready = false);
 size_t project_rows_plane_bytes(int K);
 bool project_rows_sqdist(const float *W, long ldw, int r, const float *D, long ldd, int F, const int32_t *ids, const int32_t *ids2,
                          long row0, int nrows, float *dist, void *plane_hi, void *plane_lo, void *plane_lo2, bool bf16, hipStream_t s);
@@ -264,6 +269,9 @@
 size_t jacobi_work_floats(int n);
 constexpr int CHOL_INV_MAX_N = 160;
 void chol_inverse128(const float *M, long ldm, int n, float rel_thresh, float *Linv, long ldl, int *dead, hipStream_t s);
+void ritz_prepare(const float *MT, long ldm, int n, float rel_thresh, float *S, long lds, float *T, long ldt, float *U, long ldu, int *dead,
+                  hipStream_t s);
+void ritz_compose(const float *V, long ldv, const float *S, long lds, int n, float *C, long ldc, hipStream_t s);
 struct ResidualEmit {
     float *W = nullptr;
     long ldw = 0;
diff --git a/opencv-dlco_amd/csrc/eig_tracker.cpp b/opencv-dlco_amd/csrc/eig_tracker.cpp
--- a/opencv-dlco_amd/csrc/eig_tracker.cpp
+++ b/opencv-dlco_amd/csrc/eig_tracker.cpp
@@ -28,6 +28,8 @@
     Tm_.alloc((size_t)cap_ * cap_);
     Vm_.alloc((size_t)cap_ * cap_);
     Cw_.alloc((size_t)cap_ * cap_);
+    Mt_.alloc((size_t)2 * cap_ * cap_);
+    Sm_.alloc((size_t)cap_ * cap_);
     ritz_block_.alloc((size_t)2 * (cap_ + 8) + 8);
     evals_.p = ritz_block_.p;
     res_.p = ritz_block_.p + (cap_ + 8);
@@ -138,9 +140,11 @@
         return;
     }
     st_.product_rows += rows;
+    const bool x3_ready = !approx && x3_of_ == X && x3_rows_ == rows;
+    x3_of_ = nullptr;
     if (packed_) {
         if (prof_) prof_->begin(PROF_EIG_PRODUCT);
-        const bool ready = approx && chain && chain->planes_of == X && chain->rows == rows;
+        const bool ready = approx ? (chain && chain->planes_of == X && chain->rows == rows) : x3_ready;
         const bool emit = approx && chain && chain->next;
         const bool ok = skinny_product_sym(X, F_, rows, G, F_, alpha, out, F_, E1, b1, E2, b2, plane_hi_.p, plane_lo_.p, slab_.p, s_,
                                            approx ? nullptr : plane_lo2_.p, ready, emit);
@@ -159,7 +163,7 @@
             int ks = ks_;
             while (ks < 4 * world && F_ % (128 * ks * 2) == 0 && bf16x2_slab_floats(rows, cw, ks * 2) <= slab_floats_) ks *= 2;
             done = skinny_product_bf16x2(X, F_, rows, G + c0, F_, cw, F_, alpha, out + c0, F_, E1s, b1, E2s, b2, plane_hi_.p,
-                                         plane_lo_.p, slab_.p, s_, ks, approx ? nullptr : plane_lo2_.p);
+                                         plane_lo_.p, slab_.p, s_, ks, approx ? nullptr : plane_lo2_.p, false, x3_ready);
         }
         if (!done) {
             GemmArgs g;
@@ -182,7 +186,7 @@
     if (rows <= one_pass && F_ >= 256) {
         if (prof_) prof_->begin(PROF_EIG_PRODUCT);
         const bool ok = skinny_product_bf16x2(X, F_, rows, G, F_, F_, F_, alpha, out, F_, E1, b1, E2, b2, plane_hi_.p,
-                                              plane_lo_.p, slab_.p, s_, ks_, approx ? nullptr : plane_lo2_.p);
+                                              plane_lo_.p, slab_.p, s_, ks_, approx ? nullptr : plane_lo2_.p, false, x3_ready);
         if (prof_) prof_->end(PROF_EIG_PRODUCT);
         if (ok) return;
     }
@@ -212,6 +216,13 @@
     gemm_f32(g, s_);
 }
 
+int EigTracker::gram_slices(int xrows, int yrows, int products) const
+{
+    const long tiles = (long)ceil_div(xrows, xrows <= 64 ? 64 : 128) * ceil_div(yrows, yrows <= 64 ? 64 : 128);
+    const long kslice = std::max(64L, (long)F_ / 64 / 64 * 64);
+    return split_k_slices(tiles, 512, F_, kslice, (long)(slab_floats_ / ((size_t)products * xrows * yrows)));
+}
+
 void EigTracker::gram_rect(const float *X, int xrows, const float *Y, int yrows, float *T)
 {
     GemmArgs g;
@@ -219,9 +230,20 @@
     g.A.p = X; g.A.ld = F_; g.A.kmajor = false;
     g.B.p = Y; g.B.ld = F_; g.B.kmajor = false;
     g.C = T; g.ldc = cap_;
-    const long tiles = (long)ceil_div(xrows, xrows <= 64 ? 64 : 128) * ceil_div(yrows, yrows <= 64 ? 64 : 128);
-    const long kslice = std::max(64L, (long)F_ / 64 / 64 * 64);
-    g.split_k = split_k_slices(tiles, 512, F_, kslice, (long)(slab_floats_ / ((size_t)xrows * yrows)));
+    g.split_k = gram_slices(xrows, yrows, 1);
+    g.slab = slab_.p;
+    gemm_f32(g, s_);
+}
+
+void EigTracker::gram_pair(const float *X, const float *Y, int rows, float *MT)
+{
+    GemmArgs g;
+    g.M = rows; g.N = rows; g.K = F_;
+    g.A.p = X; g.A.ld = F_; g.A.kmajor = false;
+    g.A2 = Y;
+    g.B.p = X; g.B.ld = F_; g.B.kmajor = false;
+    g.C = MT; g.ldc = cap_;
+    g.split_k = gram_slices(rows, rows, 2);
     g.slab = slab_.p;
     gemm_f32(g, s_);
 }
@@ -238,10 +260,27 @@
     gemm_f32(g, s_);
 }
 
-int EigTracker::orthonormalize(float *Z, int rows, float *scratch, const std::vector<int> &panel_ends, int skip)
+float *EigTracker::orthonormalize(float *Z, int rows, float *scratch, const std::vector<int> &panel_ends, int skip, bool *fold)
 {
     const bool one_panel = skip == 0 && rows <= CHOL_INV_MAX_N && (panel_ends.empty() || panel_ends[0] >= rows);
-    if (!one_panel) row_normalize(Z + (size_t)skip * F_, F_, rows - skip, F_, s_);
+    *fold = one_panel;
+    x3_of_ = nullptr;
+    if (one_panel) {
+        gram_rect(Z, rows, Z, rows, Tm_.p);
+        chol_inverse128(Tm_.p, cap_, rows, 1e-5f, Vm_.p, cap_, dead_.p, s_);
+        GemmArgs g;
+        g.M = rows; g.N = F_; g.K = rows;
+        g.A.p = Vm_.p; g.A.ld = cap_; g.A.kmajor = false;
+        g.B.p = Z; g.B.ld = F_; g.B.kmajor = true;
+        g.C = scratch; g.ldc = F_;
+        if (exact_planes_fit(rows)) {
+            g.plane_hi = plane_hi_.p; g.plane_lo = plane_lo_.p; g.plane_lo2 = plane_lo2_.p;
+            x3_of_ = scratch; x3_rows_ = rows;
+        }
+        gemm_f32(g, s_);
+        return scratch;
+    }
+    row_normalize(Z + (size_t)skip * F_, F_, rows - skip, F_, s_);
     size_t pi = 0;
     for (int p0 = skip; p0 < rows;) {
         while (pi < panel_ends.size() && panel_ends[pi] <= p0) pi++;
@@ -269,7 +308,13 @@
         }
         p0 = pend;
     }
-    return rows;
+    return Z;
+}
+
+bool EigTracker::exact_planes_fit(int rows) const
+{
+    if (F_ % 128 != 0) return false;
+    return packed_ ? rows <= 96 : (F_ >= 256 && rows <= 128);
 }
 
 int EigTracker::drop_dead_rows()
@@ -368,8 +413,9 @@
         else if (u.plan.filtered) Z = filter_plain(u);
         if (u.plan.filtered) last_deg_ = u.plan.d;
         eig_rules::cut_panels(block_of(u), u.n_ritz, u.plan, CHOL_INV_MAX_N, u.panel_ends);
-        orthonormalize(Z, m_, pick({Z}), u.panel_ends, u.plan.n_lock);
-        rayleigh_ritz(u, Z);
+        bool fold = false;
+        float *Zo = orthonormalize(Z, m_, pick({Z}), u.panel_ends, u.plan.n_lock, &fold);
+        rayleigh_ritz(u, Zo, fold);
         judge(u);
         const bool crowded = m_ < live_ && eig_rules::reaches_guards(u.nw, m_, guard_);
         if (crowded) u.conv = false;
@@ -490,11 +536,16 @@
     st_.product_rows -= m_;
 }
 
-void EigTracker::rayleigh_ritz(UpdateState &u, float *Qo)
+void EigTracker::rayleigh_ritz(UpdateState &u, float *Qo, bool fold)
 {
     float *Yb = pick({Qo});
     product(Qo, m_, u.G, -1.0f, Yb, nullptr, 0.f, nullptr, 0.f, false);
-    gram_rect(Yb, m_, Qo, m_, Tm_.p);
+    if (fold) {
+        gram_pair(Qo, Yb, m_, Mt_.p);
+        ritz_prepare(Mt_.p, cap_, m_, 1e-5f, Sm_.p, cap_, Tm_.p, cap_, Cw_.p, cap_, dead_.p, s_);
+    } else {
+        gram_rect(Yb, m_, Qo, m_, Tm_.p);
+    }
     if (prof_) prof_->begin(PROF_JACOBI);
     const float lam_cut = eig_rules::jacobi_lam_cut(block_of(u), have_theta_ && u.n_ritz == m_);
     float *Qn = pick({Qo, Yb});
@@ -504,7 +555,8 @@
     for (int attempt = 0;; attempt++) {
         jacobi_eigh(Tm_.p, cap_, m_, evals_.p, Vm_.p, cap_, jwork_.p, sweeps_dev_, s_, lam_cut, attempt > 0);
         if (prof_) prof_->end(PROF_JACOBI);
-        rotate(Vm_.p, cap_, m_, m_, Qo, Qn, Yb, Yn);
+        if (fold) ritz_compose(Vm_.p, cap_, Sm_.p, cap_, m_, Cw_.p, cap_, s_);
+        rotate(fold ? Cw_.p : Vm_.p, cap_, m_, m_, Qo, Qn, Yb, Yn);
         Q_ = Qn; Y_ = Yn;
         y_ok_ = true;
         unsigned *flag = reinterpret_cast<unsigned *>(pin_ + pin_floats_ - 16);
diff --git a/opencv-dlco_amd/csrc/eig_tracker.hpp b/opencv-dlco_amd/csrc/eig_tracker.hpp
--- a/opencv-dlco_amd/csrc/eig_tracker.hpp
+++ b/opencv-dlco_amd/csrc/eig_tracker.hpp
@@ -41,6 +41,8 @@
     int update(const float *G, float mu, float cscale, float *W, double *trace, bool *converged);
 
     int block_rows() const { return m_; }
+    const float *block_q() const { return Q_; }
+    const float *block_y() const { return Y_; }
     void set_profiler(Profiler *p) { prof_ = p; }
     void set_shard(const ShardComm *sc) { shard_ = sc; }
     void set_readback_extra(const int *dev) { extra_dev_ = dev; }
@@ -65,17 +67,20 @@
     float *filter_locked(const UpdateState &u);
     float *filter_plain(const UpdateState &u);
     void check_first_term(const UpdateState &u, const float *cur);
-    void rayleigh_ritz(UpdateState &u, float *Qo);
+    void rayleigh_ritz(UpdateState &u, float *Qo, bool fold);
     void judge(UpdateState &u);
     void grow(UpdateState &u);
     double trim_and_emit(UpdateState &u);
 
     void product(const float *X, int rows, const float *G, float alpha, float *out, const float *E1, float b1,
                  const float *E2, float b2, bool approx, PlaneChain *chain = nullptr);
+    int gram_slices(int xrows, int yrows, int products) const;
     void gram_rect(const float *X, int xrows, const float *Y, int yrows, float *T);
+    void gram_pair(const float *X, const float *Y, int rows, float *MT);
+    bool exact_planes_fit(int rows) const;
     void project_out(float *Wp, int np, const float *Q, int kept);
     void rotate(const float *C, long ldc, int k_in, int k_out, const float *X, float *out, const float *X2 = nullptr, float *out2 = nullptr);
-    int orthonormalize(float *Z, int rows, float *scratch, const std::vector<int> &panel_ends, int skip = 0);
+    float *orthonormalize(float *Z, int rows, float *scratch, const std::vector<int> &panel_ends, int skip, bool *fold);
     int drop_dead_rows();
     void refresh_lower_bound(const float *G, int iters, float theta_top);
     void append_random(float *Q, int have, int add);
@@ -115,6 +120,9 @@
     float *all_[6] = {nullptr, nullptr, nullptr, nullptr, nullptr, nullptr};
     float *Q_ = nullptr, *Y_ = nullptr;
     DevBuf<float> Tm_, Vm_, Cw_, jwork_, slab_, pv_, pw_, scale_;
+    DevBuf<float> Mt_, Sm_;
+    const float *x3_of_ = nullptr;
+    int x3_rows_ = 0;
     struct FView { float *p = nullptr; };
     DevBuf<float> ritz_block_;
     FView evals_, res_;
diff --git a/opencv-dlco_amd/csrc/kernels_bf16x2.hip b/opencv-dlco_amd/csrc/kernels_bf16x2.hip
--- a/opencv-dlco_amd/csrc/kernels_bf16x2.hip
+++ b/opencv-dlco_amd/csrc/kernels_bf16x2.hip
@@ -499,13 +499,13 @@
 
 bool skinny_product_bf16x2(const float *X, long ldx, int M, const float *G, long ldg, int N, int K, float alpha, float *C,
                            long ldc, const float *E1, float b1, const float *E2, float b2, void *plane_hi, void *plane_lo,
-                           float *slab, hipStream_t s, int ksplit, void *plane_lo2, bool g_tiled)
+                           float *slab, hipStream_t s, int ksplit, void *plane_lo2, bool g_tiled, bool planes_ready)
 {
     const int mt = (M + 31) / 32;
     const int ks = ksplit > 0 ? ksplit : KS;
     if (M < 1 || mt > 5 || N % 128 != 0 || K % (16 * ks * 2 * 4) != 0) return false;
     if (ldx % 4 != 0 || (reinterpret_cast<uintptr_t>(X) & 15) != 0) return false;
-    split_planes_bf16(X, ldx, M, K, plane_hi, plane_lo, plane_lo2, s);
+    if (!planes_ready) split_planes_bf16(X, ldx, M, K, plane_hi, plane_lo, plane_lo2, s);
     Bf2Dev g;
     g.M = M; g.N = N; g.K = K;
     g.xhi = static_cast<const bf16x8 *>(plane_hi); g.xlo = static_cast<const bf16x8 *>(plane_lo);
@@ -536,7 +536,7 @@
     const int nt = F / 128;
     if (F % 128 != 0 || nt < 1 || nt > 64 || M < 1 || mt > 5 || (mt >= 4 && plane_lo2)) return false;
     if (ldx % 4 != 0 || (reinterpret_cast<uintptr_t>(X) & 15) != 0 || (reinterpret_cast<uintptr_t>(Gpacked) & 15) != 0) return false;
-    if ((planes_ready || emit_planes) && plane_lo2) return false;
+    if (emit_planes && plane_lo2) return false;
     if (!planes_ready) split_planes_bf16(X, ldx, M, F, plane_hi, plane_lo, plane_lo2, s);
     SymDev g;
     g.M = M; g.K = F;
diff --git a/opencv-dlco_amd/csrc/kernels_eig.hip b/opencv-dlco_amd/csrc/kernels_eig.hip
--- a/opencv-dlco_amd/csrc/kernels_eig.hip
+++ b/opencv-dlco_amd/csrc/kernels_eig.hip
@@ -7,6 +7,7 @@
 namespace {
 
 typedef float f32x4 __attribute__((ext_vector_type(4)));
+typedef float f32x16 __attribute__((ext_vector_type(16)));
 
 __device__ __forceinline__ float wsum(float v)
 {
@@ -88,10 +89,8 @@
 __device__ __forceinline__ float readlane_f(float v, int l) { return __int_as_float(__builtin_amdgcn_readlane(__float_as_int(v), l)); }
 
 template <int NBM>
-__global__ __launch_bounds__(C2_T) void chol_inv2_kernel(const float *M, long ldm, int n, float rel_thresh, float *Linv, long ldl,
-                                                         int *dead)
-{
-    extern __shared__ __attribute__((aligned(16))) float c2[];
+__device__ __forceinline__ void chol_inv2_body(const float *M, long ldm, int n, float rel_thresh, float *Linv, long ldl, int *dead, float *c2)
+{
     float (*Dblk)[33] = reinterpret_cast<float (*)[33]>(c2);
     float (*Tblk)[33] = reinterpret_cast<float (*)[33]>(c2 + 32 * 33);
     constexpr int C2_PLD = c2_pld(NBM), NR = 32 * NBM;
@@ -265,6 +264,119 @@
     if (t < n) dead[t] = deadf[t];
 }
 
+template <int NBM>
+__global__ __launch_bounds__(C2_T) void chol_inv2_kernel(const float *M, long ldm, int n, float rel_thresh, float *Linv, long ldl,
+                                                         int *dead)
+{
+    extern __shared__ __attribute__((aligned(16))) float c2[];
+    chol_inv2_body<NBM>(M, ldm, n, rel_thresh, Linv, ldl, dead, c2);
+}
+
+
+__host__ __device__ constexpr int sm_tpw(int nbm) { return (nbm * nbm + 15) / 16; }
+
+template <int NBM, bool BT>
+__device__ __forceinline__ void small_mm(const float *A, long lda, const float *B, long ldb, int n, f32x16 (&acc)[sm_tpw(NBM)], float *lds)
+{
+    constexpr int NR = 32 * NBM, TPW = sm_tpw(NBM);
+    float (*As)[33] = reinterpret_cast<float (*)[33]>(lds);
+    float (*Bs)[NR + 1] = reinterpret_cast<float (*)[NR + 1]>(lds + NR * 33);
+    const int t = threadIdx.x, lane = t & 63, wave = t >> 6, nb = (n + 31) >> 5;
+    const int lr = lane & 31, lk = lane >> 5;
+#pragma unroll
+    for (int u = 0; u < TPW; u++)
+#pragma unroll
+        for (int r = 0; r < 16; r++) acc[u][r] = 0.f;
+    for (int kb = 0; kb < nb; kb++) {
+        __syncthreads();
+        for (int idx = t; idx < NR * 32; idx += C2_T) {
+            const int i = idx >> 5, kk = idx & 31, k = 32 * kb + kk;
+            const bool in = i < n && k < n;
+            const float id = (i == k) ? 1.f : 0.f;
+            if (BT) {
+                As[i][kk] = in ? A[(long)i * lda + k] : 0.f;
+                Bs[kk][i] = in ? B[(long)i * ldb + k] - id : 0.f;
+            } else {
+                As[i][kk] = in ? A[(long)i * lda + k] - id : 0.f;
+                const int k2 = idx / NR, j = idx % NR;
+                Bs[k2][j] = (j < n && 32 * kb + k2 < n) ? B[(long)(32 * kb + k2) * ldb + j] : 0.f;
+            }
+        }
+        __syncthreads();
+#pragma unroll
+        for (int u = 0; u < TPW; u++) {
+            const int tile = wave + 16 * u;
+            if (tile < NBM * NBM) {
+                const int tr = tile / NBM, tc = tile % NBM;
+#pragma unroll
+                for (int kk = 0; kk < 16; kk++)
+                    acc[u] = __builtin_amdgcn_mfma_f32_32x32x2f32(As[32 * tr + lr][2 * kk + lk], Bs[2 * kk + lk][32 * tc + lr], acc[u], 0, 0, 0);
+            }
+        }
+    }
+    const float *X = BT ? A : B;
+    const long ldx = BT ? lda : ldb;
+#pragma unroll
+    for (int u = 0; u < TPW; u++) {
+        const int tile = wave + 16 * u;
+        if (tile < NBM * NBM) {
+#pragma unroll
+            for (int r = 0; r < 16; r++) {
+                const int i = 32 * (tile / NBM) + (r & 3) + 8 * (r >> 2) + 4 * lk, j = 32 * (tile % NBM) + lr;
+                if (i < n && j < n) acc[u][r] += X[(long)i * ldx + j];
+            }
+        }
+    }
+}
+
+template <int NBM>
+__device__ __forceinline__ void small_store(const f32x16 (&acc)[sm_tpw(NBM)], float *C, long ldc, int n)
+{
+    const int lane = threadIdx.x & 63, wave = threadIdx.x >> 6;
+#pragma unroll
+    for (int u = 0; u < sm_tpw(NBM); u++) {
+        const int tile = wave + 16 * u;
+        if (tile < NBM * NBM) {
+#pragma unroll
+            for (int r = 0; r < 16; r++) {
+                const int i = 32 * (tile / NBM) + (r & 3) + 8 * (r >> 2) + 4 * (lane >> 5), j = 32 * (tile % NBM) + (lane & 31);
+                if (i < n && j < n) C[(long)i * ldc + j] = acc[u][r];
+            }
+        }
+    }
+}
+
+template <int NBM>
+__global__ __launch_bounds__(C2_T) void ritz_prepare_kernel(const float *MT, long ldm, int n, float rel_thresh, float *S, long lds, float *T,
+                                                            long ldt, float *U, long ldu, int *dead)
+{
+    extern __shared__ __attribute__((aligned(16))) float c2[];
+    chol_inv2_body<NBM>(MT, ldm, n, rel_thresh, S, lds, dead, c2);
+    __syncthreads();
+    f32x16 acc[sm_tpw(NBM)];
+    small_mm<NBM, true>(MT + (long)n * ldm, ldm, S, lds, n, acc, c2);
+    small_store<NBM>(acc, U, ldu, n);
+    small_mm<NBM, false>(S, lds, U, ldu, n, acc, c2);
+    small_store<NBM>(acc, T, ldt, n);
+}
+
+__global__ __launch_bounds__(1024) void ritz_compose_kernel(const float *V, long ldv, const float *S, long lds, int n, float *C, long ldc)
+{
+    __shared__ float Vs[32][33], Ss[32][33];
+    const int tx = threadIdx.x & 31, ty = threadIdx.x >> 5;
+    const int i = 32 * blockIdx.y + ty, j = 32 * blockIdx.x + tx;
+    float acc = 0.f;
+    for (int k0 = 0; k0 < n; k0 += 32) {
+        Vs[ty][tx] = (i < n && k0 + tx < n) ? V[(long)i * ldv + k0 + tx] : 0.f;
+        Ss[ty][tx] = (k0 + ty < n && j < n) ? S[(long)(k0 + ty) * lds + j] - ((k0 + ty == j) ? 1.f : 0.f) : 0.f;
+        __syncthreads();
+#pragma unroll 8
+        for (int kk = 0; kk < 32; kk++) acc = fmaf(Vs[ty][kk], Ss[kk][tx], acc);
+        __syncthreads();
+    }
+    if (i < n && j < n) C[(long)i * ldc + j] = V[(long)i * ldv + j] + acc;
+}
+
 }
 
 template <int NBM>
@@ -280,6 +392,32 @@
     if (n <= 96) launch_chol_inv2<3>(M, ldm, n, rel_thresh, Linv, ldl, dead, s);
     else if (n <= 128) launch_chol_inv2<4>(M, ldm, n, rel_thresh, Linv, ldl, dead, s);
     else launch_chol_inv2<5>(M, ldm, n, rel_thresh, Linv, ldl, dead, s);
+    DLCO_HIP(hipGetLastError());
+}
+
+template <int NBM>
+static void launch_ritz_prepare(const float *MT, long ldm, int n, float rel_thresh, float *S, long lds, float *T, long ldt, float *U, long ldu,
+                                int *dead, hipStream_t s)
+{
+    ensure_dynamic_lds(reinterpret_cast<const void *>(ritz_prepare_kernel<NBM>), (int)(c2_lds_floats(NBM) * sizeof(float)));
+    hipLaunchKernelGGL(ritz_prepare_kernel<NBM>, dim3(1), dim3(C2_T), c2_lds_floats(NBM) * sizeof(float), s, MT, ldm, n, rel_thresh, S, lds, T,
+                       ldt, U, ldu, dead);
+}
+
+void ritz_prepare(const float *MT, long ldm, int n, float rel_thresh, float *S, long lds, float *T, long ldt, float *U, long ldu, int *dead,
+                  hipStream_t s)
+{
+    DLCO_CHECK(n >= 1 && n <= CHOL_INV_MAX_N, -2, "ritz_prepare: n out of range");
+    if (n <= 96) launch_ritz_prepare<3>(MT, ldm, n, rel_thresh, S, lds, T, ldt, U, ldu, dead, s);
+    else if (n <= 128) launch_ritz_prepare<4>(MT, ldm, n, rel_thresh, S, lds, T, ldt, U, ldu, dead, s);
+    else launch_ritz_prepare<5>(MT, ldm, n, rel_thresh, S, lds, T, ldt, U, ldu, dead, s);
+    DLCO_HIP(hipGetLastError());
+}
+
+void ritz_compose(const float *V, long ldv, const float *S, long lds, int n, float *C, long ldc, hipStream_t s)
+{
+    const unsigned nb = (unsigned)((n + 31) / 32);
+    hipLaunchKernelGGL(ritz_compose_kernel, dim3(nb, nb), dim3(1024), 0, s, V, ldv, S, lds, n, C, ldc);
     DLCO_HIP(hipGetLastError());
 }
 
diff --git a/opencv-dlco_amd/csrc/kernels_gemm.hip b/opencv-dlco_amd/csrc/kernels_gemm.hip
--- a/opencv-dlco_amd/csrc/kernels_gemm.hip
+++ b/opencv-dlco_amd/csrc/kernels_gemm.hip
@@ -1,9 +1,7 @@
 #include "dlco_internal.hpp"
+#include "split_bf16_dev.hpp"
 
 namespace dlco {
-
-typedef float f32x16 __attribute__((ext_vector_type(16)));
-typedef float f32x4 __attribute__((ext_vector_type(4)));
 
 namespace {
 
@@ -47,6 +45,9 @@
     int upper_only;
     const float *B2;
     float *C2;
+    const float *A2;
+    bf16x8 *plane_hi, *plane_lo, *plane_lo2;
+    int plane_mt;
 };
 
 template <int BT, bool KM>
@@ -103,12 +104,10 @@
     }
 }
 
-template <int WM, int WN, bool A_KM, bool B_KM>
-__global__ __launch_bounds__(NT) void gemm_kernel(GemmDev g)
+template <int WM, int WN, bool A_KM, bool B_KM, bool PLANES>
+__device__ __forceinline__ void gemm_body(GemmDev g, float (*As)[BK][64 * WM + PAD], float (*Bs)[BK][64 * WN + PAD])
 {
     constexpr int BM = 64 * WM, BN = 64 * WN;
-    __shared__ __attribute__((aligned(16))) float As[2][BK][BM + PAD];
-    __shared__ __attribute__((aligned(16))) float Bs[2][BK][BN + PAD];
 
     const int bi = blockIdx.y, bj = blockIdx.x;
     if (g.upper_only && bj * BN + BN <= bi * BM) return;
@@ -120,6 +119,10 @@
     if (g.B2) {
         if (kz == 1) { g.B.p = g.B2; g.C = g.C2; }
         kz = 0;
+    }
+    if (g.A2) {
+        if (kz & 1) g.A.p = g.A2;
+        kz >>= 1;
     }
     int kbeg = kz * g.k_chunk;
     int kend = min(g.K, kbeg + g.k_chunk);
@@ -192,6 +195,47 @@
                 g.C[idx] = o;
                 if (g.upper_only && j > i) g.C[(long)j * g.ldc + i] = o;
             }
+
+    if constexpr (PLANES) {
+        static_assert(WM == 1 && WN == 1, "plane emission is written for 64 x 64 tiles");
+        float (*stage)[64 + PAD] = reinterpret_cast<float (*)[64 + PAD]>(&As[0][0][0]);
+#pragma unroll
+        for (int r = 0; r < 16; r++) {
+            const int li = wm * 32 + (r & 3) + 8 * (r >> 2) + 4 * lh, lj = wn * 32 + lc;
+            stage[li][lj] = (i0 + li < g.M && j0 + lj < g.N) ? g.alpha * acc[0][0][r] : 0.f;
+        }
+        __syncthreads();
+#pragma unroll
+        for (int u = 0; u < 2; u++) {
+            const int e = threadIdx.x + NT * u;
+            const int lrow = ((e >> 6) & 1) * 32 + (e & 31), lc8 = 2 * (e >> 7) + ((e >> 5) & 1);
+            const int row = i0 + lrow;
+            if (row < 32 * g.plane_mt) {
+                const f32x4 g0 = *reinterpret_cast<const f32x4 *>(&stage[lrow][8 * lc8]);
+                const f32x4 g1 = *reinterpret_cast<const f32x4 *>(&stage[lrow][8 * lc8 + 4]);
+                bf16x8 h, l, l2;
+                split_frag<3>(g0, g1, h, l, l2);
+                const long t = plane_entry_at(g.plane_mt, row, (j0 >> 3) + lc8);
+                g.plane_hi[t] = h;
+                g.plane_lo[t] = l;
+                g.plane_lo2[t] = l2;
+            }
+        }
+    }
+}
+
+template <int WM, int WN, bool A_KM, bool B_KM>
+__global__ __launch_bounds__(NT) void gemm_kernel(GemmDev g)
+{
+    __shared__ __attribute__((aligned(16))) float As[2][BK][64 * WM + PAD];
+    __shared__ __attribute__((aligned(16))) float Bs[2][BK][64 * WN + PAD];
+    gemm_body<WM, WN, A_KM, B_KM, false>(g, As, Bs);
+}
+
+__global__ __launch_bounds__(NT) void gemm_planes_kernel(GemmDev g)
+{
+    __shared__ __attribute__((aligned(16))) float AB[4][BK][64 + PAD];
+    gemm_body<1, 1, false, true, true>(g, AB, AB + 2);
 }
 
 __global__ void splitk_reduce_kernel(const float *slab, int split, int M, int N, float *C, long ldc, float alpha,
@@ -297,6 +341,26 @@
         g.slab = a.slab;
     }
     g.B2 = a.B2; g.C2 = a.C2;
+    g.A2 = a.A2;
+    g.plane_hi = static_cast<bf16x8 *>(a.plane_hi); g.plane_lo = static_cast<bf16x8 *>(a.plane_lo); g.plane_lo2 = static_cast<bf16x8 *>(a.plane_lo2);
+    g.plane_mt = (a.M + 31) / 32;
+    if (a.A2) {
+        DLCO_CHECK(a.slab && !a.B2 && !a.upper_only && !a.plane_hi && !a.A.kmajor && !a.B.kmajor && !a.A.row_ids &&
+                   ((reinterpret_cast<uintptr_t>(a.A2) ^ reinterpret_cast<uintptr_t>(a.A.p)) & 15) == 0, -2,
+                   "gemm_f32: a twin A needs a slab, row-major operands and no other twin");
+        g.slab = a.slab;
+        hipLaunchKernelGGL((gemm_kernel<1, 1, false, false>), dim3((a.N + 63) / 64, (a.M + 63) / 64, 2 * split), dim3(NT), 0, s, g);
+        DLCO_HIP(hipGetLastError());
+        splitk_reduce_f32(a.slab, split, 2 * a.M, a.N, a.C, a.ldc, a.alpha, a.beta, a.E1, a.b1, a.E2, a.b2, s);
+        return;
+    }
+    if (a.plane_hi) {
+        DLCO_CHECK(a.plane_lo && a.plane_lo2 && !a.A.kmajor && a.B.kmajor && a.N % 64 == 0 && split == 1 && !a.B2 && !a.upper_only &&
+                   a.beta == 0.f && !a.E1 && !a.E2, -2, "gemm_f32: plane emission takes a plain C = alpha A B with N in whole 64-column tiles");
+        hipLaunchKernelGGL(gemm_planes_kernel, dim3(a.N / 64, (a.M + 63) / 64, 1), dim3(NT), 0, s, g);
+        DLCO_HIP(hipGetLastError());
+        return;
+    }
     if (a.B2) {
         DLCO_CHECK(a.C2 && split == 1 && !a.upper_only, -2, "gemm_f32: a twin product needs C2 and no K split");
         split = 2;
```
